# delldu/VSTNet

Hardware: AMD Instinct MI355X
Metric: stylized frames/sec at 1024x1024 (1/2/4/8 GPU) + % HBM roofline (higher is better)
Workload: dtype bf16x3

## Files before the change

include/vstnet.h:

```cpp
#ifndef VSTNET_H
#define VSTNET_H

#include <stddef.h>
#include <stdint.h>

#ifdef __cplusplus
extern "C" {
#endif
#pragma GCC visibility push(default)

#define VST_OK 0
#define VST_E_ARG (-1)
#define VST_E_SHAPE (-2)
#define VST_E_MODE (-3)
#define VST_E_WORKSPACE (-4)

#define VST_PREC_BF16X3 0
#define VST_PREC_FP32 1
#define VST_PREC_F16X2 2

#define VST_PREC_F16X2H 3

#define VST_NUM_BLOCKS 32

int vst_version(void);
const char* vst_error_string(int code);

#define VST_MAX_FRAME_PIXELS ((int64_t)1 << 26)
int64_t vst_max_frame_pixels(void);

size_t vst_conv_packed_bytes(int cout, int cin);
int vst_pack_conv(const float* w_oihw, int cout, int cin, void* packed, void* stream);

int vst_normalize_block(float* w1, float* b1, float* w4, float* b4, float* w7, int c_in1, int c_mid, int c_out,
                        float* scales, void* stream);

#define VST_RANGE_SATURATED 1u
#define VST_RANGE_WEIGHT 2u
int vst_range_flags(unsigned* flags_host, int reset);
int vst_range_flags_async(unsigned* flags4_dev, void* stream);

typedef struct vst_conv_weights {
    const void* packed;
    const float* bias;
} vst_conv_weights;

typedef struct vst_block_weights {
    vst_conv_weights conv[3];
} vst_block_weights;

typedef struct vst_net_weights {
    vst_block_weights blocks[VST_NUM_BLOCKS];
} vst_net_weights;

int vst_pack_input(const float* x, float* s1, float* s2, int B, int C, int H, int W, void* stream);
int vst_unpack_output(const float* s1, float* x, int B, int C, int H, int W, void* stream);
int vst_pack_input_u8(const uint8_t* frames_hwc, float* s1, float* s2, int B, int H, int W, void* stream);
int vst_unpack_output_u8(const float* s1, uint8_t* frames_hwc, int B, int H, int W, void* stream);
int vst_lab_luminance(const float* content, const float* stylized, float* out, int B, int H, int W, void* stream);
int vst_lab_luminance_u8(const uint8_t* content_hwc, const float* stylized, uint8_t* out_hwc, int B, int H, int W, void* stream);
int vst_lab_luminance_u8_f32(const uint8_t* content_hwc, const float* stylized, float* out, int B, int H, int W, void* stream);
int vst_spread(const float* s1, const float* s2, float* z, int B, int H, int W, int sp_steps, void* stream);
int vst_gather(const float* z, float* s1, float* s2, int B, int H, int W, int sp_steps, void* stream);

size_t vst_block_tmp_bytes(int B, int H, int W);
int vst_block_apply(const vst_block_weights* w, int channel, int stride, int direction, int precision,
                    float* dst, const float* src, void* tmp, int B, int H, int W, void* stream);

size_t vst_pass_workspace_bytes(int B, int H, int W);
int vst_pass_sub_batch(int B, int H, int W);
int vst_revnet_forward(const vst_net_weights* w, const float* x, float* z, void* workspace,
                       int B, int C_in, int H, int W, int sp_steps, int precision, void* stream);
int vst_revnet_inverse(const vst_net_weights* w, const float* z, float* x, void* workspace,
                       int B, int C_out, int H, int W, int sp_steps, int precision, void* stream);

int vst_revnet_forward_u8(const vst_net_weights* w, const uint8_t* frames_hwc, float* z, void* workspace,
                          int B, int H, int W, int sp_steps, int precision, void* stream);
int vst_revnet_inverse_u8(const vst_net_weights* w, const float* z, uint8_t* frames_hwc, void* workspace,
                          int B, int H, int W, int sp_steps, int precision, void* stream);

int vst_revnet_encode(const vst_net_weights* w, const float* x, float* code, void* workspace,
                      int B, int C_in, int H, int W, int precision, void* stream);
int vst_revnet_encode_u8(const vst_net_weights* w, const uint8_t* frames_hwc, float* code, void* workspace,
                         int B, int H, int W, int precision, void* stream);
int vst_revnet_decode(const vst_net_weights* w, const float* code, const float* affines, float* x, void* workspace,
                      int B, int C_out, int H, int W, int sp_steps, int precision, void* stream);
int vst_revnet_decode_u8(const vst_net_weights* w, const float* code, const float* affines, uint8_t* frames_hwc,
                         void* workspace, int B, int H, int W, int sp_steps, int precision, void* stream);
int vst_code_to_z(const float* code, float* z, int B, int H, int W, int sp_steps, void* stream);
int vst_z_to_code(const float* z, float* code, int B, int H, int W, int sp_steps, void* stream);
size_t vst_cwct_stats_code_workspace_bytes(int H, int W, int sp_steps);
int vst_cwct_stats_code(const float* code, int H, int W, int sp_steps, double* stats, void* workspace, void* stream);
int vst_cwct_apply_code(const float* code, float* out, int H, int W, int sp_steps, const float* affine, void* stream);
int vst_mask_to_code(const uint8_t* mask, uint8_t* mask_rows, int H, int W, void* stream);
size_t vst_cwct_stats_labels_code_workspace_bytes(int H, int W);
int vst_cwct_stats_labels_code(const float* code, int H, int W, const uint8_t* mask_rows, const void* plan, int max_slots,
                               double* stats, void* workspace, void* stream);
int vst_cwct_apply_labels_code(const float* code, float* out, int H, int W, const float* affines, const uint8_t* mask_rows,
                               const void* plan, int max_slots, void* stream);
int vst_cwct_stats_code_rect(const float* code, int H, int W, int sp_steps, int y0, int x0, int h, int w, double* stats,
                             void* workspace, void* stream);
int vst_cwct_stats_labels_code_rect(const float* code, int H, int W, int y0, int x0, int h, int w, const uint8_t* mask_rows,
                                    const void* plan, int max_slots, double* stats, void* workspace, void* stream);
int vst_revnet_decode_labels(const vst_net_weights* w, const float* code, const float* affines, const uint8_t* mask_rows,
                             const void* plan, int max_slots, float* x, void* workspace, int C_out, int H, int W,
                             int precision, void* stream);
int vst_revnet_decode_labels_u8(const vst_net_weights* w, const float* code, const float* affines, const uint8_t* mask_rows,
                                const void* plan, int max_slots, uint8_t* frame_hwc, void* workspace, int H, int W,
                                int precision, void* stream);
int vst_map_to_code(const float* map, float* rows, int H, int W, int sp_steps, void* stream);
int vst_cwct_apply_code_blend(const float* code, float* out, int H, int W, int sp_steps, const float* affine,
                              const float* strength_rows, void* stream);
int vst_cwct_apply_labels_code_blend(const float* code, float* out, int H, int W, const float* affines, const uint8_t* mask_rows,
                                     const void* plan, int max_slots, const float* strength_rows, void* stream);
int vst_revnet_decode_blend(const vst_net_weights* w, const float* code, const float* affines, const float* strength_rows,
                            float* x, void* workspace, int B, int C_out, int H, int W, int sp_steps, int precision, void* stream);
int vst_revnet_decode_blend_u8(const vst_net_weights* w, const float* code, const float* affines, const float* strength_rows,
                               uint8_t* frames_hwc, void* workspace, int B, int H, int W, int sp_steps, int precision,
                               void* stream);
int vst_revnet_decode_labels_blend(const vst_net_weights* w, const float* code, const float* affines, const uint8_t* mask_rows,
                                   const void* plan, int max_slots, const float* strength_rows, float* x, void* workspace,
                                   int C_out, int H, int W, int precision, void* stream);
int vst_revnet_decode_labels_blend_u8(const vst_net_weights* w, const float* code, const float* affines, const uint8_t* mask_rows,
                                      const void* plan, int max_slots, const float* strength_rows, uint8_t* frame_hwc,
                                      void* workspace, int H, int W, int precision, void* stream);
int vst_cwct_blend(const float* x, const float* y, const float* strength, float* out, int N, long L, void* stream);
int vst_cwct_apply_code_mix(const float* code, float* out, int H, int W, int sp_steps, const float* affines, int K,
                            const float* weight_rows, const float* strength_rows, void* stream);
int vst_revnet_decode_mix(const vst_net_weights* w, const float* code, const float* affines, int K, const float* weight_rows,
                          const float* strength_rows, float* x, void* workspace, int B, int C_out, int H, int W, int sp_steps,
                          int precision, void* stream);
int vst_revnet_decode_mix_u8(const vst_net_weights* w, const float* code, const float* affines, int K, const float* weight_rows,
                             const float* strength_rows, uint8_t* frames_hwc, void* workspace, int B, int H, int W, int sp_steps,
                             int precision, void* stream);
int vst_cwct_mix_acc(const float* a, const float* w, float* out, int N, long L, int first, void* stream);
int vst_strength_frame(const uint8_t* matte, const uint8_t* labels, const float* table, float* dense, float* rows, int H, int W,
                       int sp_steps, void* stream);
#define VST_STATS_POOL_MAX 8
int vst_cwct_stats_pool(const double* const* records_host_array, const double* weights_host, int n_ages, int n_records, int N,
                        double cut, double* out, int* used, void* stream);

size_t vst_cwct_stats_workspace_bytes(int N, long L);
int vst_cwct_stats(const float* x, int N, long L, const uint8_t* mask, int label,
                   double* stats, void* workspace, void* stream);
int vst_cwct_factor(const double* content_stats, const double* const* style_stats_host_array,
                    const float* alphas_host, int n_styles, float alpha_c, float eps, int N,
                    float* affine, int* info, void* stream);
int vst_cwct_apply(const float* x, float* y, int N, long L, const float* affine,
                   const uint8_t* mask, int label, void* stream);
int vst_cwct_apply_prec(const float* x, float* y, int N, long L, const float* affine,
                        const uint8_t* mask, int label, int precision, void* stream);
#define VST_LABEL_PLAN_BYTES 2344
int vst_label_plan(const uint8_t* cmask, long Lc, const uint8_t* smask, long Ls, void* plan, void* stream);
size_t vst_cwct_labels_workspace_bytes(int N, long L);
int vst_cwct_stats_labels(const float* x, int N, long L, const uint8_t* mask, const void* plan, int max_slots,
                          double* stats, void* workspace, void* stream);
int vst_cwct_factor_labels(const double* content_stats, const double* style_stats, const void* plan, int max_slots,
                           float eps, int N, float* affines, int* info, void* stream);
int vst_cwct_apply_labels(const float* x, float* y, int N, long L, const float* affines, const uint8_t* mask,
                          const void* plan, int max_slots, int precision, void* stream);

#define VST_MASK_OVERFLOW 1u
#define VST_MASK_OUT_OF_TABLE 2u
int vst_colors_to_labels(const uint8_t* rgb, uint8_t* labels, long n, void* stream);
int vst_label_hist(const uint8_t* labels, long n, int* hist, void* stream);
int vst_mask_prepare(const uint8_t* src, int colours, int H, int W, uint8_t* mask_rows, int* hist, void* stream);
int vst_remap_lut(const int* hist, const int* style_hist, const int16_t* table, int rows, int cols, int min_count,
                  uint8_t* lut, int* hist_out, unsigned* flags, void* stream);
int vst_apply_lut(const uint8_t* in, const uint8_t* lut, uint8_t* out, long n, void* stream);
int vst_label_plan_hist(const int* hist_c, const uint8_t* remap_lut, const int* hist_s, int max_slots, void* plan,
                        unsigned* flags, void* stream);
int vst_cwct_factor_labels_keyed(const double* content_stats, const double* style_stats, const void* plan,
                                 const void* style_plan, int max_slots, float eps, int N, float* affines, int* info,
                                 void* stream);
int vst_label_plan_hists(const int* hist_c, const uint8_t* remap_lut, const int* const* hist_s_host_array, int n_styles,
                         int max_slots, void* plan, unsigned* flags, void* stream);
int vst_cwct_factor_labels_mix(const double* content_stats, const double* const* style_stats_host_array,
                               const void* const* style_plans_host_array, const float* alphas_host, int n_styles,
                               float alpha_c, const void* plan, int max_slots, float eps, int N, float* affines, int* info,
                               void* stream);
int vst_cwct_prefactor_labels(const double* stats, const void* plan, int max_slots, int N, float eps, double* out, int* info,
                              void* stream);

int vst_cwct_prefactor(const double* stats, int N, float eps, double* out, int* info, void* stream);

int vst_generic_conv(const float* x, const float* w, const float* bias, const float* old, float sign, int relu, float* out, int B,
                     int Cin, int Cout, int H, int W, int K, int stride, void* stream);
int vst_generic_squeeze(const float* x, float* y, int B, int D, int H, int W, void* stream);
int vst_generic_unsqueeze(const float* y, float* x, int B, int D, int H, int W, void* stream);
int vst_generic_copy_channels(const float* src, float* dst, int B, int C_src, int c0, int n, long HW, int C_dst, int d0,
                              void* stream);
int vst_generic_zero(float* dst, size_t n_floats, void* stream);

size_t vst_cwct_stats_f64_workspace_bytes(int N, long L);
int vst_cwct_stats_f64(const float* x, int N, long L, const uint8_t* mask, int label, double* stats, void* workspace,
                       void* stream);
size_t vst_cwct_factor_f64_workspace_bytes(int N);
int vst_cwct_factor_f64(const double* content_stats, const double* const* style_stats_host_array, const float* alphas_host,
                        int n_styles, float alpha_c, float eps, int N, double* affine, int* info, void* workspace,
                        void* stream);
int vst_cwct_apply_f64(const float* x, float* y, int N, long L, const double* affine, const uint8_t* mask, int label,
                       void* stream);

size_t vst_cwct_stats_n_workspace_bytes(int N, long L);
int vst_cwct_stats_n(const float* x, int N, long L, const uint8_t* mask, int label, double* stats, void* workspace,
                     size_t workspace_bytes, void* stream);
size_t vst_cwct_factor_n_workspace_bytes(int N);
int vst_cwct_factor_n(const double* content_stats, const double* const* style_stats_host_array, const float* alphas_host,
                      int n_styles, float alpha_c, float eps, int N, float* affine, int* info, void* workspace,
                      size_t workspace_bytes, void* stream);
int vst_cwct_prefactor_n(const double* stats, int N, float eps, double* out, int* info, void* workspace, size_t workspace_bytes,
                         void* stream);
int vst_cwct_apply_n(const float* x, float* y, int N, long L, const float* affine, const uint8_t* mask, int label, void* stream);
size_t vst_cwct_stats_n_f64_workspace_bytes(int N, long L);
int vst_cwct_stats_n_f64(const float* x, int N, long L, const uint8_t* mask, int label, double* stats, void* workspace,
                         size_t workspace_bytes, void* stream);
size_t vst_cwct_factor_n_f64_workspace_bytes(int N);
int vst_cwct_factor_n_f64(const double* content_stats, const double* const* style_stats_host_array, const float* alphas_host,
                          int n_styles, float alpha_c, float eps, int N, double* affine, int* info, void* workspace,
                          size_t workspace_bytes, void* stream);
int vst_cwct_apply_n_f64(const float* x, float* y, int N, long L, const double* affine, const uint8_t* mask, int label,
                         void* stream);

#define VST_KERNEL_ID(cin, cout, stride) (((cin) << 16) | ((cout) << 4) | (stride))
#define VST_KERNEL_ALL (-1)
#define VST_KERNEL_PACK 1
#define VST_KERNEL_UNPACK 2
#define VST_KERNEL_SPREAD 3
#define VST_KERNEL_GATHER 4
#define VST_KERNEL_CWCT_STATS 5
#define VST_KERNEL_CWCT_FACTOR 6
#define VST_KERNEL_CWCT_APPLY 7
#define VST_KERNEL_PRESPLIT 8
#define VST_KERNEL_SEG_MIX 9
#define VST_KERNEL_CWCT_POOL 10
int vst_profile_begin(int kernel_id, int max_records);
int vst_profile_end(double* total_ms, int* launches);
int vst_profile_end_table(int* ids, double* ms, int* launches, int cap, int* n_ids);

#define VST_OPT_STAGE3_LEAN 1
#define VST_OPT_STAGE3_PINGPONG 2
#define VST_OPT_STAGE3_WIDE 3
#define VST_OPT_STAGE1_FOLD 4
#define VST_OPT_OUT_RGB 5
int vst_set_option(int option, int value);
int vst_get_option(int option);

#define VST_RESIZE_MAX_SHRINK 16
int vst_resize_coeffs_u8(int in_size, int out_size, int* ksize, int* bounds, int* kk);
int vst_resize_u8(const uint8_t* src_hwc, int Hs, int Ws, uint8_t* dst_hwc, int Hd, int Wd, const int* tables_dev,
                  uint8_t* tmp, void* stream);
int vst_resize_coeffs_u8_bilinear(int in_size, int out_size, int* ksize, int* bounds, int* kk);
int vst_resize_grey_u8(const uint8_t* src, int Hs, int Ws, uint8_t* dst, int Hd, int Wd, const int* tables_dev, uint8_t* tmp,
                       void* stream);
int vst_resize_coeffs_f32(int in_size, int out_size, int* ksize, int* xmin, float* w);
int vst_resize_f32(const float* x_planar, int B, int Hs, int Ws, float* dst_planar, int Hd, int Wd, const void* tables_dev,
                   float* tmp, void* stream);
int vst_resize_f32_to_u8(const float* x_planar, int B, int Hs, int Ws, uint8_t* dst_hwc, int Hd, int Wd,
                         const void* tables_dev, float* tmp, void* stream);

#define VST_SEG_CLASSES 150
#define VST_SEG_MAX_LABEL_PIXELS (1LL << 30)
#define VST_SEG_MIX_MAX 8
typedef struct vst_seg vst_seg;
int vst_seg_create(const int* depths, int embed_dim, vst_seg** plan);
int vst_seg_tensor_count(const vst_seg* plan);
int vst_seg_tensor_info(const vst_seg* plan, int index, const char** name, size_t* count);
int vst_seg_load_tensor(vst_seg* plan, const char* name, const float* data_host, size_t count);
int vst_seg_run_u8(vst_seg* plan, const uint8_t* frame_u8, int chw, int H, int W, uint8_t* labels_u8, void* stream);
int vst_seg_run_scaled_u8(vst_seg* plan, const uint8_t* work_u8, int chw, int Hw, int Ww, int H, int W, uint8_t* labels_u8,
                          void* stream);
int vst_seg_labels_from_logits(const float* logits, int Hq, int Wq, int H, int W, int kernel, uint8_t* labels, void* stream);
int vst_seg_logits(vst_seg* plan, const uint8_t* frame_u8, int chw, int H, int W, float* logits, float* x1, float* x2,
                   float* x3, float* x4, void* stream);
int vst_seg_shape(int H, int W, int* hw8);
int vst_seg_mix_logits(const float* const* logits_host_array, const float* weights_host, int n, size_t count, float* out,
                       void* stream);
int vst_seg_destroy(vst_seg* plan);
int vst_seg_gemm(const float* A, const float* W, const float* bias, const float* res, float* out, int M, int N, int K,
                 void* stream);
int vst_seg_layernorm(const float* x, const float* g, const float* b, float* out, int T, int C, float eps, void* stream);
int vst_seg_attention(const float* q, const float* kv, float* out, int N, int Nk, int C, float scale, void* stream);
int vst_seg_dwconv_gelu(const float* in, const float* w, const float* b, float* out, int H, int W, int C, void* stream);
int vst_seg_im2col(const float* in, int Hi, int Wi, int C, int k, int stride, int pad, float* col, void* stream);
int vst_seg_gather_rgb(const uint8_t* frame_u8, int chw, int H, int W, float* col, void* stream);
int vst_seg_head_sum(const float* y0, const float* y1, const float* y2, const float* y3, const int* hw8, int E, float* out,
                     void* stream);

#pragma GCC visibility pop
#ifdef __cplusplus
}
#endif
#endif
```

vstnet_amd/_lib.py:

```python
from __future__ import annotations

import ctypes as C
import glob
import os
import subprocess

PKG_DIR = os.path.dirname(os.path.abspath(__file__))
REPO_DIR = os.path.dirname(PKG_DIR)
LIB_PATH = os.environ.get("VSTNET_HIP_LIB") or os.path.join(PKG_DIR, "libvstnet_hip.so")
RESOURCES_PATH = os.path.join(PKG_DIR, "libvstnet_hip.resources.txt")
SOURCES = sorted(glob.glob(os.path.join(PKG_DIR, "csrc", "*.hip")))
HEADERS = sorted(glob.glob(os.path.join(PKG_DIR, "csrc", "*.h"))) + [os.path.join(REPO_DIR, "include", "vstnet.h")]

NUM_BLOCKS = 32
PREC_BF16X3 = 0
PREC_FP32 = 1
PREC_F16X2 = 2
PREC_F16X2H = 3

EXPORTS = [
    "vst_version", "vst_error_string", "vst_conv_packed_bytes", "vst_pack_conv", "vst_pack_input",
    "vst_unpack_output", "vst_pack_input_u8", "vst_unpack_output_u8", "vst_revnet_forward_u8", "vst_revnet_inverse_u8",
    "vst_spread", "vst_gather", "vst_block_tmp_bytes", "vst_block_apply",
    "vst_pass_workspace_bytes", "vst_revnet_forward", "vst_revnet_inverse",
    "vst_cwct_stats_workspace_bytes", "vst_cwct_stats", "vst_cwct_factor", "vst_cwct_apply", "vst_cwct_apply_prec",
    "vst_cwct_prefactor", "vst_label_plan", "vst_cwct_labels_workspace_bytes", "vst_cwct_stats_labels",
    "vst_cwct_factor_labels", "vst_cwct_apply_labels", "vst_profile_begin", "vst_profile_end", "vst_profile_end_table", "vst_lab_luminance",
    "vst_revnet_encode", "vst_revnet_encode_u8", "vst_revnet_decode", "vst_revnet_decode_u8", "vst_code_to_z", "vst_z_to_code",
    "vst_cwct_stats_code_workspace_bytes", "vst_cwct_stats_code", "vst_cwct_apply_code",
    "vst_mask_to_code", "vst_cwct_stats_labels_code_workspace_bytes", "vst_cwct_stats_labels_code", "vst_cwct_apply_labels_code",
    "vst_revnet_decode_labels", "vst_revnet_decode_labels_u8", "vst_pass_sub_batch",
    "vst_normalize_block", "vst_range_flags", "vst_range_flags_async",
    "vst_cwct_stats_f64_workspace_bytes", "vst_cwct_stats_f64", "vst_cwct_factor_f64_workspace_bytes", "vst_cwct_factor_f64",
    "vst_cwct_apply_f64",
    "vst_generic_conv", "vst_generic_squeeze", "vst_generic_unsqueeze", "vst_generic_copy_channels", "vst_generic_zero",
    "vst_set_option", "vst_get_option",
    "vst_cwct_stats_n_workspace_bytes", "vst_cwct_stats_n", "vst_cwct_factor_n_workspace_bytes", "vst_cwct_factor_n",
    "vst_cwct_prefactor_n", "vst_cwct_apply_n", "vst_cwct_stats_n_f64_workspace_bytes", "vst_cwct_stats_n_f64",
    "vst_cwct_factor_n_f64_workspace_bytes", "vst_cwct_factor_n_f64", "vst_cwct_apply_n_f64",
    "vst_max_frame_pixels", "vst_cwct_stats_code_rect", "vst_cwct_stats_labels_code_rect",
    "vst_colors_to_labels", "vst_label_hist", "vst_mask_prepare", "vst_remap_lut", "vst_apply_lut", "vst_label_plan_hist",
    "vst_cwct_factor_labels_keyed",
    "vst_label_plan_hists", "vst_cwct_factor_labels_mix", "vst_cwct_prefactor_labels",
    "vst_resize_coeffs_u8", "vst_resize_u8", "vst_resize_coeffs_f32", "vst_resize_f32", "vst_resize_f32_to_u8",
    "vst_lab_luminance_u8", "vst_lab_luminance_u8_f32",
    "vst_seg_create", "vst_seg_tensor_count", "vst_seg_tensor_info", "vst_seg_load_tensor", "vst_seg_run_u8", "vst_seg_logits",
    "vst_seg_shape", "vst_seg_destroy", "vst_seg_run_scaled_u8", "vst_seg_labels_from_logits",
    "vst_seg_mix_logits",
    "vst_seg_gemm", "vst_seg_layernorm", "vst_seg_attention", "vst_seg_dwconv_gelu", "vst_seg_im2col", "vst_seg_gather_rgb",
    "vst_seg_head_sum",
    "vst_map_to_code", "vst_cwct_apply_code_blend", "vst_cwct_apply_labels_code_blend", "vst_revnet_decode_blend",
    "vst_revnet_decode_blend_u8", "vst_revnet_decode_labels_blend", "vst_revnet_decode_labels_blend_u8", "vst_cwct_blend",
    "vst_strength_frame", "vst_resize_coeffs_u8_bilinear", "vst_resize_grey_u8",
    "vst_cwct_apply_code_mix", "vst_revnet_decode_mix", "vst_revnet_decode_mix_u8", "vst_cwct_mix_acc",
    "vst_cwct_stats_pool",
]
MAX_STYLES = 8
SEG_MIX_MAX = 8
KERNEL_SEG_MIX = 9
STATS_POOL_MAX = 8
KERNEL_CWCT_POOL = 10
MASK_OVERFLOW = 1
MASK_OUT_OF_TABLE = 2
LABEL_PLAN_BYTES = 2344
OPT_STAGE3_LEAN = 1
OPT_STAGE3_WIDE = 3
OPT_STAGE1_FOLD = 4
OPT_OUT_RGB = 5
RANGE_SATURATED = 1
RANGE_WEIGHT = 2


PRECISIONS = {"bf16x3": PREC_BF16X3, "fp32": PREC_FP32, "f16x2": PREC_F16X2, "f16x2h": PREC_F16X2H}


def default_precision() -> str:
    p = os.environ.get("VST_PRECISION", "bf16x3")
    if p not in PRECISIONS:
        raise ValueError(f"VST_PRECISION must be one of {sorted(PRECISIONS)}")
    return p


class VstError(RuntimeError):
    pass


class ConvWeights(C.Structure):
    _fields_ = [("packed", C.c_void_p), ("bias", C.c_void_p)]


class BlockWeights(C.Structure):
    _fields_ = [("conv", ConvWeights * 3)]


class NetWeights(C.Structure):
    _fields_ = [("blocks", BlockWeights * NUM_BLOCKS)]


def build(force: bool = False, verbose: bool = False) -> str:
    newest_src = max(os.path.getmtime(p) for p in SOURCES + HEADERS)
    if not force and os.path.exists(LIB_PATH) and os.path.getmtime(LIB_PATH) >= newest_src:
        return LIB_PATH
    hipcc = os.environ.get("HIPCC", "/opt/rocm/bin/hipcc")
    cmd = [hipcc, "-O3", "--offload-arch=gfx950", "-fPIC", "-shared", "-std=c++17", "-Xarch_host", "-fvisibility=hidden",
           "-I", os.path.join(REPO_DIR, "include"), "-o", LIB_PATH] + SOURCES
    cmd[1:1] = ["-Rpass-analysis=kernel-resource-usage", "-fno-caret-diagnostics"]
    if verbose:
        print(" ".join(cmd))
    p = subprocess.run(cmd, stderr=subprocess.PIPE, text=True)
    remarks = [ln.split("remark:", 1)[1].split("[-Rpass")[0].strip() for ln in p.stderr.splitlines() if "remark:" in ln]
    other = "\n".join(ln for ln in p.stderr.splitlines() if "remark:" not in ln and "kernel-resource-usage" not in ln)
    if p.returncode != 0:
        raise subprocess.CalledProcessError(p.returncode, cmd, stderr=other)
    if other.strip():
        print(other)
    table, name = [], None
    for r in remarks:
        if r.startswith("Function Name:"):
            name = r.split(":", 1)[1].strip()
        elif name and (r.startswith("VGPRs:") or r.startswith("ScratchSize") or r.startswith("LDS Size") or r.startswith("Occupancy")):
            table.append(f"{name}\t{r}")
    with open(RESOURCES_PATH, "w") as f:
        f.write("\n".join(table) + "\n")
    spills = [t for t in table if "ScratchSize" in t and not t.rstrip().endswith(": 0")]
    if spills:
        os.remove(LIB_PATH)
        raise RuntimeError("kernels with a private segment (register spills):\n" + "\n".join(spills))
    return LIB_PATH


RUNNER_SRC = os.path.join(REPO_DIR, "tools", "vst_run.cpp")
RUNNER_BIN = os.path.join(REPO_DIR, "tools", "vst_run")


def build_runner(force: bool = False) -> str:
    if not force and os.path.exists(RUNNER_BIN) and os.path.getmtime(RUNNER_BIN) >= max(os.path.getmtime(RUNNER_SRC),
                                                                                       os.path.getmtime(LIB_PATH)):
        return RUNNER_BIN
    hipcc = os.environ.get("HIPCC", "/opt/rocm/bin/hipcc")
    cmd = [hipcc, "-O2", "--offload-arch=gfx950", "-std=c++17", "-I", os.path.join(REPO_DIR, "include"), RUNNER_SRC,
           "-L", PKG_DIR, "-lvstnet_hip", "-Wl,-rpath," + PKG_DIR, "-Wl,-rpath,$ORIGIN/../vstnet_amd", "-o", RUNNER_BIN]
    subprocess.run(cmd, check=True)
    return RUNNER_BIN


_lib = None


def lib() -> C.CDLL:
    global _lib
    if _lib is not None:
        return _lib
    if not os.path.exists(LIB_PATH):
        raise VstError(f"{LIB_PATH} is missing: run `python -c 'import __graft_entry__ as g; g.build()'` "
                       "(there is no CPU fallback for the HIP path)")
    L = C.CDLL(LIB_PATH)
    vp, i, f, sz, lg = C.c_void_p, C.c_int, C.c_float, C.c_size_t, C.c_long
    sig = {
        "vst_version": (i, []),
        "vst_error_string": (C.c_char_p, [i]),
        "vst_conv_packed_bytes": (sz, [i, i]),
        "vst_pack_conv": (i, [vp, i, i, vp, vp]),
        "vst_normalize_block": (i, [vp, vp, vp, vp, vp, i, i, i, vp, vp]),
        "vst_range_flags": (i, [C.POINTER(C.c_uint), i]),
        "vst_range_flags_async": (i, [vp, vp]),
        "vst_pack_input": (i, [vp, vp, vp, i, i, i, i, vp]),
        "vst_unpack_output": (i, [vp, vp, i, i, i, i, vp]),
        "vst_pack_input_u8": (i, [vp, vp, vp, i, i, i, vp]),
        "vst_unpack_output_u8": (i, [vp, vp, i, i, i, vp]),
        "vst_lab_luminance": (i, [vp, vp, vp, i, i, i, vp]),
        "vst_lab_luminance_u8": (i, [vp, vp, vp, i, i, i, vp]),
        "vst_lab_luminance_u8_f32": (i, [vp, vp, vp, i, i, i, vp]),
        "vst_revnet_forward_u8": (i, [C.POINTER(NetWeights), vp, vp, vp, i, i, i, i, i, vp]),
        "vst_revnet_inverse_u8": (i, [C.POINTER(NetWeights), vp, vp, vp, i, i, i, i, i, vp]),
        "vst_spread": (i, [vp, vp, vp, i, i, i, i, vp]),
        "vst_gather": (i, [vp, vp, vp, i, i, i, i, vp]),
        "vst_block_tmp_bytes": (sz, [i, i, i]),
        "vst_block_apply": (i, [C.POINTER(BlockWeights), i, i, i, i, vp, vp, vp, i, i, i, vp]),
        "vst_pass_workspace_bytes": (sz, [i, i, i]),
        "vst_pass_sub_batch": (i, [i, i, i]),
        "vst_revnet_forward": (i, [C.POINTER(NetWeights), vp, vp, vp, i, i, i, i, i, i, vp]),
        "vst_revnet_inverse": (i, [C.POINTER(NetWeights), vp, vp, vp, i, i, i, i, i, i, vp]),
        "vst_cwct_stats_workspace_bytes": (sz, [i, lg]),
        "vst_cwct_stats": (i, [vp, i, lg, vp, i, vp, vp, vp]),
        "vst_cwct_factor": (i, [vp, C.POINTER(vp), C.POINTER(f), i, f, f, i, vp, vp, vp]),
        "vst_cwct_apply": (i, [vp, vp, i, lg, vp, vp, i, vp]),
        "vst_cwct_apply_prec": (i, [vp, vp, i, lg, vp, vp, i, i, vp]),
        "vst_cwct_prefactor": (i, [vp, i, f, vp, vp, vp]),
        "vst_cwct_stats_f64_workspace_bytes": (sz, [i, lg]),
        "vst_cwct_stats_f64": (i, [vp, i, lg, vp, i, vp, vp, vp]),
        "vst_cwct_factor_f64_workspace_bytes": (sz, [i]),
        "vst_cwct_factor_f64": (i, [vp, C.POINTER(vp), C.POINTER(f), i, f, f, i, vp, vp, vp, vp]),
        "vst_cwct_apply_f64": (i, [vp, vp, i, lg, vp, vp, i, vp]),
        "vst_cwct_stats_n_workspace_bytes": (sz, [i, lg]),
        "vst_cwct_stats_n": (i, [vp, i, lg, vp, i, vp, vp, sz, vp]),
        "vst_cwct_factor_n_workspace_bytes": (sz, [i]),
        "vst_cwct_factor_n": (i, [vp, C.POINTER(vp), C.POINTER(f), i, f, f, i, vp, vp, vp, sz, vp]),
        "vst_cwct_prefactor_n": (i, [vp, i, f, vp, vp, vp, sz, vp]),
        "vst_cwct_apply_n": (i, [vp, vp, i, lg, vp, vp, i, vp]),
        "vst_cwct_stats_n_f64_workspace_bytes": (sz, [i, lg]),
        "vst_cwct_stats_n_f64": (i, [vp, i, lg, vp, i, vp, vp, sz, vp]),
        "vst_cwct_factor_n_f64_workspace_bytes": (sz, [i]),
        "vst_cwct_factor_n_f64": (i, [vp, C.POINTER(vp), C.POINTER(f), i, f, f, i, vp, vp, vp, sz, vp]),
        "vst_cwct_apply_n_f64": (i, [vp, vp, i, lg, vp, vp, i, vp]),
        "vst_generic_conv": (i, [vp, vp, vp, vp, f, i, vp, i, i, i, i, i, i, i, vp]),
        "vst_generic_squeeze": (i, [vp, vp, i, i, i, i, vp]),
        "vst_generic_unsqueeze": (i, [vp, vp, i, i, i, i, vp]),
        "vst_generic_copy_channels": (i, [vp, vp, i, i, i, i, lg, i, i, vp]),
        "vst_generic_zero": (i, [vp, sz, vp]),
        "vst_label_plan": (i, [vp, lg, vp, lg, vp, vp]),
        "vst_cwct_labels_workspace_bytes": (sz, [i, lg]),
        "vst_cwct_stats_labels": (i, [vp, i, lg, vp, vp, i, vp, vp, vp]),
        "vst_cwct_factor_labels": (i, [vp, vp, vp, i, f, i, vp, vp, vp]),
        "vst_cwct_apply_labels": (i, [vp, vp, i, lg, vp, vp, vp, i, i, vp]),
        "vst_revnet_encode": (i, [C.POINTER(NetWeights), vp, vp, vp, i, i, i, i, i, vp]),
        "vst_revnet_encode_u8": (i, [C.POINTER(NetWeights), vp, vp, vp, i, i, i, i, vp]),
        "vst_revnet_decode": (i, [C.POINTER(NetWeights), vp, vp, vp, vp, i, i, i, i, i, i, vp]),
        "vst_revnet_decode_u8": (i, [C.POINTER(NetWeights), vp, vp, vp, vp, i, i, i, i, i, vp]),
        "vst_code_to_z": (i, [vp, vp, i, i, i, i, vp]),
        "vst_z_to_code": (i, [vp, vp, i, i, i, i, vp]),
        "vst_cwct_stats_code_workspace_bytes": (sz, [i, i, i]),
        "vst_cwct_stats_code": (i, [vp, i, i, i, vp, vp, vp]),
        "vst_cwct_apply_code": (i, [vp, vp, i, i, i, vp, vp]),
        "vst_mask_to_code": (i, [vp, vp, i, i, vp]),
        "vst_cwct_stats_labels_code_workspace_bytes": (sz, [i, i]),
        "vst_cwct_stats_labels_code": (i, [vp, i, i, vp, vp, i, vp, vp, vp]),
        "vst_cwct_apply_labels_code": (i, [vp, vp, i, i, vp, vp, vp, i, vp]),
        "vst_revnet_decode_labels": (i, [C.POINTER(NetWeights), vp, vp, vp, vp, i, vp, vp, i, i, i, i, vp]),
        "vst_revnet_decode_labels_u8": (i, [C.POINTER(NetWeights), vp, vp, vp, vp, i, vp, vp, i, i, i, vp]),
        "vst_map_to_code": (i, [vp, vp, i, i, i, vp]),
        "vst_cwct_apply_code_blend": (i, [vp, vp, i, i, i, vp, vp, vp]),
        "vst_cwct_apply_labels_code_blend": (i, [vp, vp, i, i, vp, vp, vp, i, vp, vp]),
        "vst_revnet_decode_blend": (i, [C.POINTER(NetWeights), vp, vp, vp, vp, vp, i, i, i, i, i, i, vp]),
        "vst_revnet_decode_blend_u8": (i, [C.POINTER(NetWeights), vp, vp, vp, vp, vp, i, i, i, i, i, vp]),
        "vst_revnet_decode_labels_blend": (i, [C.POINTER(NetWeights), vp, vp, vp, vp, i, vp, vp, vp, i, i, i, i, vp]),
        "vst_revnet_decode_labels_blend_u8": (i, [C.POINTER(NetWeights), vp, vp, vp, vp, i, vp, vp, vp, i, i, i, vp]),
        "vst_cwct_blend": (i, [vp, vp, vp, vp, i, lg, vp]),
        "vst_strength_frame": (i, [vp, vp, vp, vp, vp, i, i, i, vp]),
        "vst_cwct_apply_code_mix": (i, [vp, vp, i, i, i, vp, i, vp, vp, vp]),
        "vst_revnet_decode_mix": (i, [C.POINTER(NetWeights), vp, vp, i, vp, vp, vp, vp, i, i, i, i, i, i, vp]),
        "vst_revnet_decode_mix_u8": (i, [C.POINTER(NetWeights), vp, vp, i, vp, vp, vp, vp, i, i, i, i, i, vp]),
        "vst_cwct_mix_acc": (i, [vp, vp, vp, i, lg, i, vp]),
        "vst_resize_coeffs_u8_bilinear": (i, [i, i, C.POINTER(i), vp, vp]),
        "vst_resize_grey_u8": (i, [vp, i, i, vp, i, i, vp, vp, vp]),
        "vst_max_frame_pixels": (C.c_int64, []),
        "vst_cwct_stats_code_rect": (i, [vp, i, i, i, i, i, i, i, vp, vp, vp]),
        "vst_cwct_stats_labels_code_rect": (i, [vp, i, i, i, i, i, i, vp, vp, i, vp, vp, vp]),
        "vst_colors_to_labels": (i, [vp, vp, lg, vp]),
        "vst_label_hist": (i, [vp, lg, vp, vp]),
        "vst_mask_prepare": (i, [vp, i, i, i, vp, vp, vp]),
        "vst_remap_lut": (i, [vp, vp, vp, i, i, i, vp, vp, vp, vp]),
        "vst_apply_lut": (i, [vp, vp, vp, lg, vp]),
        "vst_label_plan_hist": (i, [vp, vp, vp, i, vp, vp, vp]),
        "vst_cwct_factor_labels_keyed": (i, [vp, vp, vp, vp, i, f, i, vp, vp, vp]),
        "vst_label_plan_hists": (i, [vp, vp, C.POINTER(vp), i, i, vp, vp, vp]),
        "vst_cwct_factor_labels_mix": (i, [vp, C.POINTER(vp), C.POINTER(vp), C.POINTER(f), i, f, vp, i, f, i, vp, vp, vp]),
        "vst_cwct_prefactor_labels": (i, [vp, vp, i, i, f, vp, vp, vp]),
        "vst_resize_coeffs_u8": (i, [i, i, C.POINTER(i), vp, vp]),
        "vst_resize_u8": (i, [vp, i, i, vp, i, i, vp, vp, vp]),
        "vst_resize_coeffs_f32": (i, [i, i, C.POINTER(i), vp, vp]),
        "vst_resize_f32": (i, [vp, i, i, i, vp, i, i, vp, vp, vp]),
        "vst_resize_f32_to_u8": (i, [vp, i, i, i, vp, i, i, vp, vp, vp]),
        "vst_seg_create": (i, [C.POINTER(i), i, C.POINTER(vp)]),
        "vst_seg_tensor_count": (i, [vp]),
        "vst_seg_tensor_info": (i, [vp, i, C.POINTER(C.c_char_p), C.POINTER(sz)]),
        "vst_seg_load_tensor": (i, [vp, C.c_char_p, vp, sz]),
        "vst_seg_run_u8": (i, [vp, vp, i, i, i, vp, vp]),
        "vst_seg_run_scaled_u8": (i, [vp, vp, i, i, i, i, i, vp, vp]),
        "vst_seg_labels_from_logits": (i, [vp, i, i, i, i, i, vp, vp]),
        "vst_seg_logits": (i, [vp, vp, i, i, i, vp, vp, vp, vp, vp, vp]),
        "vst_seg_shape": (i, [i, i, C.POINTER(i)]),
        "vst_seg_mix_logits": (i, [C.POINTER(vp), C.POINTER(f), i, sz, vp, vp]),
        "vst_cwct_stats_pool": (i, [C.POINTER(vp), C.POINTER(C.c_double), i, i, i, C.c_double, vp, vp, vp]),
        "vst_seg_destroy": (i, [vp]),
        "vst_seg_gemm": (i, [vp, vp, vp, vp, vp, i, i, i, vp]),
        "vst_seg_layernorm": (i, [vp, vp, vp, vp, i, i, f, vp]),
        "vst_seg_attention": (i, [vp, vp, vp, i, i, i, f, vp]),
        "vst_seg_dwconv_gelu": (i, [vp, vp, vp, vp, i, i, i, vp]),
        "vst_seg_im2col": (i, [vp, i, i, i, i, i, i, vp, vp]),
        "vst_seg_gather_rgb": (i, [vp, i, i, i, vp, vp]),
        "vst_seg_head_sum": (i, [vp, vp, vp, vp, C.POINTER(i), i, vp, vp]),
        "vst_set_option": (i, [i, i]),
        "vst_get_option": (i, [i]),
        "vst_profile_begin": (i, [i, i]),
        "vst_profile_end": (i, [C.POINTER(C.c_double), C.POINTER(i)]),
        "vst_profile_end_table": (i, [C.POINTER(i), C.POINTER(C.c_double), C.POINTER(i), i, C.POINTER(i)]),
    }
    for name, (res, args) in sig.items():
        fn = getattr(L, name)
        fn.restype = res
        fn.argtypes = args
    _lib = L
    return L


KERNEL_ALL = -1
MISC_KERNELS = {1: "pack_input", 2: "unpack_output", 3: "spread", 4: "gather", 5: "cwct_stats", 6: "cwct_factor",
                7: "cwct_apply", 8: "presplit", 9: "seg_mix", 10: "cwct_pool"}


def profile_table(run, max_records: int = 4096):
    L = lib()
    check(L.vst_profile_begin(KERNEL_ALL, max_records), "vst_profile_begin")
    try:
        run()
    finally:
        ids, ms, cnt, n = (C.c_int * 64)(), (C.c_double * 64)(), (C.c_int * 64)(), C.c_int(0)
        check(L.vst_profile_end_table(ids, ms, cnt, 64, C.byref(n)), "vst_profile_end_table")
    return {ids[k]: (ms[k], cnt[k]) for k in range(n.value)}


def set_option(option: int, value: int) -> None:
    check(lib().vst_set_option(option, int(value)), "vst_set_option")


def get_option(option: int) -> int:
    v = lib().vst_get_option(option)
    if v < 0:
        check(v, "vst_get_option")
    return v


def kernel_id(cin: int, cout: int, stride: int) -> int:
    return (cin << 16) | (cout << 4) | stride


def range_flags(reset: bool = False) -> int:
    v = C.c_uint(0)
    check(lib().vst_range_flags(C.byref(v), 1 if reset else 0), "vst_range_flags")
    return int(v.value)


def check(rc: int, what: str) -> None:
    if rc != 0:
        msg = lib().vst_error_string(rc).decode()
        raise VstError(f"{what} failed with status {rc}: {msg}")
```

vstnet_amd/csrc/common.h:

```cpp
#pragma once
#include <hip/hip_runtime.h>
#include <stdint.h>
#include <atomic>
#include "vstnet.h"

#define VST_RETURN_IF_LAUNCH_FAILED()                      \
    do {                                                   \
        hipError_t e__ = hipGetLastError();                \
        if (e__ != hipSuccess) return (int)e__;            \
    } while (0)

typedef __attribute__((ext_vector_type(8))) __bf16 bf16x8;
typedef __attribute__((ext_vector_type(8))) _Float16 f16x8;
typedef __attribute__((ext_vector_type(4))) unsigned u32x4;
typedef __attribute__((ext_vector_type(4))) __bf16 bf16x4;
typedef __attribute__((ext_vector_type(4))) float f32x4;
typedef __attribute__((ext_vector_type(16))) float f32x16;

__host__ __device__ __forceinline__ int vst_level_of_channels(int c) { return c == 16 ? 0 : (c == 64 ? 1 : 2); }

__device__ __forceinline__ size_t zc_offset(int level, int y, int x, int Wq) {
    if (level == 0) {
        const int cell = (y >> 2) * Wq + (x >> 2);
        const int sub = ((((y >> 1) & 1) * 2 + ((x >> 1) & 1)) << 6) + (((y & 1) * 2 + (x & 1)) << 4);
        return (size_t)cell * 256 + sub;
    } else if (level == 1) {
        const int cell = (y >> 1) * Wq + (x >> 1);
        return (size_t)cell * 256 + (((y & 1) * 2 + (x & 1)) << 6);
    }
    return (size_t)(y * Wq + x) * 256;
}

__device__ __forceinline__ int reflect_clamp(int v, int n) {
    if (v < 0) v = -v;
    if (v >= n) v = 2 * n - 2 - v;
    v = v < 0 ? 0 : v;
    return v >= n ? n - 1 : v;
}

#ifdef __HIPCC__
static __device__ unsigned vst_tu_range_flags;
__device__ __forceinline__ void vst_note_range(float amax) {
#ifndef VST_NO_RANGE_CHECK
    if (amax > 65504.f) atomicOr(&vst_tu_range_flags, VST_RANGE_SATURATED);
#endif
}
#define VST_DEFINE_TU_RANGE(name)                                                                                    \
    __attribute__((visibility("hidden"))) int name(unsigned* acc, int reset) {                                       \
        unsigned v = 0;                                                                                              \
        hipError_t e = hipMemcpyFromSymbol(&v, HIP_SYMBOL(vst_tu_range_flags), sizeof(v));                           \
        if (e != hipSuccess) return (int)e;                                                                          \
        *acc |= v;                                                                                                   \
        if (reset && v) {                                                                                            \
            const unsigned zero = 0;                                                                                 \
            e = hipMemcpyToSymbol(HIP_SYMBOL(vst_tu_range_flags), &zero, sizeof(zero));                              \
            if (e != hipSuccess) return (int)e;                                                                      \
        }                                                                                                            \
        return VST_OK;                                                                                               \
    }                                                                                                                \
    __attribute__((visibility("hidden"))) int name##_async(unsigned* dst_dev, hipStream_t st) {                      \
        return (int)hipMemcpyFromSymbolAsync(dst_dev, HIP_SYMBOL(vst_tu_range_flags), sizeof(unsigned), 0,           \
                                             hipMemcpyDeviceToDevice, st);                                           \
    }

__device__ __forceinline__ void split8_sp(const float (&f)[8], u32x4& hi, u32x4& lo, float& amax) {
    f16x8 h, l;
#ifndef VST_NO_RANGE_CHECK
    amax = fmaxf(fmaxf(fmaxf(amax, fabsf(f[0])), fmaxf(fabsf(f[1]), fabsf(f[2]))),
                 fmaxf(fmaxf(fabsf(f[3]), fabsf(f[4])), fmaxf(fmaxf(fabsf(f[5]), fabsf(f[6])), fabsf(f[7]))));
#endif
#pragma unroll
    for (int i = 0; i < 8; ++i) {
        h[i] = (_Float16)__builtin_amdgcn_fmed3f(f[i], -65504.f, 65504.f);
        l[i] = (_Float16)(f[i] - (float)h[i]);
    }
    hi = __builtin_bit_cast(u32x4, h);
    lo = __builtin_bit_cast(u32x4, l);
}
__device__ __forceinline__ void split8_sp(const float (&f)[8], u32x4& hi, u32x4& lo) {
    float amax = 0.f;
    split8_sp(f, hi, lo, amax);
    vst_note_range(amax);
}

__device__ __forceinline__ unsigned sp_offset(int cig, int plane, int y, int x, int H, int W) {
    return ((((unsigned)cig * 2 + plane) * H + y) * W + x) * 16u;
}
__device__ __forceinline__ unsigned sp_offset1(int cig, int y, int x, int H, int W) {
    return (((unsigned)cig * H + y) * W + x) * 16u;
}
#endif

static inline int vst_ensure_dynamic_lds(const void* kernel, int bytes, std::atomic<unsigned>* done_mask) {
    int dev = 0;
    hipError_t e = hipGetDevice(&dev);
    if (e != hipSuccess) return (int)e;
    if (dev < 32 && (done_mask->load(std::memory_order_acquire) >> dev) & 1u) return VST_OK;
    e = hipFuncSetAttribute(kernel, hipFuncAttributeMaxDynamicSharedMemorySize, bytes);
    if (e != hipSuccess) return (int)e;
    if (dev < 32) done_mask->fetch_or(1u << dev, std::memory_order_release);
    return VST_OK;
}

static inline bool vst_shape_ok(int B, int H, int W) {
    return B > 0 && H >= 8 && W >= 8 && (H % 4) == 0 && (W % 4) == 0 && (int64_t)H * W <= VST_MAX_FRAME_PIXELS;
}

struct PackedConvLayout {
    int ksteps;
    int coutp;
    size_t f32_bytes;
    size_t frag_bytes;
    int sp_sections;
    size_t f16_offset;
};

__host__ __device__ inline PackedConvLayout packed_conv_layout(int cout, int cin) {
    PackedConvLayout p;
    p.ksteps = cin >= 32 ? 9 * (cin / 32) : (cin == 16 ? 5 : 2);
    p.coutp = (cout + 15) / 16 * 16;
    p.f32_bytes = ((size_t)9 * cin * cout * 4 + 255) / 256 * 256;
    p.frag_bytes = (size_t)p.ksteps * 4 * p.coutp * 16;
    p.sp_sections = (cin >= 64 && cout >= 64) ? 1 : 0;
    p.f16_offset = p.f32_bytes + (size_t)(2 + p.sp_sections) * p.frag_bytes;
    return p;
}

#define CWCT_MAX_SLOTS 32
#define CWCT_MAX_STYLES 8
struct LabelPlan {
    int n_slots, overflow;
    int hist_c[256], hist_s[256];
    unsigned char lut[256];
    unsigned char slot_label[CWCT_MAX_SLOTS];
};
static_assert(sizeof(LabelPlan) == VST_LABEL_PLAN_BYTES, "vstnet.h: VST_LABEL_PLAN_BYTES");

int vst_prof_open(int kernel_id, hipStream_t st);
void vst_prof_close(int rec, hipStream_t st);
struct vst_prof_scope {
    int rec;
    hipStream_t st;
    vst_prof_scope(int kernel_id, hipStream_t s) : rec(vst_prof_open(kernel_id, s)), st(s) {}
    ~vst_prof_scope() { if (rec >= 0) vst_prof_close(rec, st); }
};
int vst_option(int option);

int vst3_block256(const vst_block_weights* w, int direction, int precision, float* dst, const float* src, void* tmp,
                  int pos, int src_planes_ready, int B, int H, int W, void* stream);
int vst3_conv_mid(const vst_conv_weights* c, const void* in_sp, void* out_sp, int out_single, int B, int H, int W, void* stream);
int vst3_conv_out(const vst_conv_weights* c, const void* in_sp, int in_single, float* state, void* out_sp, float sign, int B,
                  int H, int W, void* stream);
static inline bool vst_is_f16(int precision) { return precision == VST_PREC_F16X2 || precision == VST_PREC_F16X2H; }
int vst_block0_to_image(const vst_block_weights* w0, int precision, float* dst, const float* src, float* tmp, int B, int H,
                        int W, float* rgb, uint8_t* rgb_u8, int rgb_c, void* stream);

unsigned char* vst3_plane_buffer(void* tmp, int idx, int B, int H, int W);
extern "C" __attribute__((visibility("hidden"))) int vst3_gather_planes(const float* z, unsigned char* s1_planes, float* s2, int B, int H, int W, int sp_steps,
                                  void* stream);

int vst3_presplit(const float* state, unsigned char* planes, int B, int H, int W, void* stream);
int vst3_apply_code(const float* code, float* out0, float* out1, unsigned char* planes0, int H, int W, int sp_steps,
                    const float* affine, const float* strength_rows, void* stream);

int vst3_apply_code_mix(const float* code, float* out0, float* out1, unsigned char* planes0, int H, int W, int sp_steps,
                        const float* affines, int K, const float* weight_rows, const float* strength_rows, void* stream);

int vst3_apply_labels_code(const float* code, float* out0, float* out1, unsigned char* planes0, int H, int W,
                           const float* affines, const uint8_t* mask_rows, const void* plan, int max_slots,
                           const float* strength_rows, void* stream);

#define VST_INTERNAL __attribute__((visibility("hidden")))
int vst_range_tu_conv(unsigned* acc, int reset);
int vst_range_tu_conv3(unsigned* acc, int reset);
int vst_range_tu_layout(unsigned* acc, int reset);
int vst_range_tu_cwct(unsigned* acc, int reset);
int vst_range_tu_conv_async(unsigned* dst_dev, hipStream_t st);
int vst_range_tu_conv3_async(unsigned* dst_dev, hipStream_t st);
int vst_range_tu_layout_async(unsigned* dst_dev, hipStream_t st);
int vst_range_tu_cwct_async(unsigned* dst_dev, hipStream_t st);
extern "C" VST_INTERNAL int vst_pack_input_k(const float* x, const uint8_t* x_u8, float* s1, float* s2, int B, int C, int H, int W,
                                const float* addk, void* stream);
extern "C" VST_INTERNAL int vst_block0_const(const vst_block_weights* w0, float* k16, void* stream);
```

vstnet_amd/csrc/conv.hip:

```cpp
#include "common.h"

struct ConvArgs {
    const float* in;
    float* out;
    const unsigned char* packed;
    const float* bias;
    int Hin, Win, Hout, Wout;
    int Wq;
    size_t in_img_stride;
    size_t out_img_stride;
    float sign;
    int tiles_x, tiles_y, tiles_total;
    const unsigned char* packed1;
    const float* bias1;
    unsigned char* out_sp;
    size_t out_sp_img_bytes;
    unsigned trace_base;
    float* rgb;
    unsigned char* rgb_u8;
    int rgb_c;
};

#ifdef VST_TRACE
__device__ unsigned long long vst_trace_buf[4 * 16384];
__device__ unsigned long long* vst_trace_ptr;
__device__ unsigned vst_trace_cap;
static std::atomic<unsigned> vst_trace_host_n{0};
#define VST_TRACE_RESERVE(t_, grid_) (t_).trace_base = vst_trace_host_n.fetch_add((unsigned)(grid_));
#define VST_TRACE_BEGIN(which)                                                                                  \
    const unsigned long long trace_t0 = __builtin_amdgcn_s_memrealtime();
#define VST_TRACE_END_(which, cin_, cout_)                                                                      \
    if (VST_TRACE == (which) || VST_TRACE == 3) {                                                               \
        __builtin_amdgcn_s_waitcnt(0);                                                                          \
        asm volatile("s_waitcnt vmcnt(0)" ::: "memory");                                                       \
        if (threadIdx.x == 0 && (VST_TRACE == 3 || blockIdx.x < 16384)) {                                       \
            unsigned hw, xcc;                                                                                   \
            asm volatile("s_getreg_b32 %0, hwreg(HW_REG_HW_ID)" : "=s"(hw));                                    \
            asm volatile("s_getreg_b32 %0, hwreg(HW_REG_XCC_ID)" : "=s"(xcc));                                  \
            if (VST_TRACE == 3) {                                                                               \
                const unsigned i_ = a.trace_base + blockIdx.x;                                                  \
                if (vst_trace_ptr && i_ < vst_trace_cap) {                                                      \
                    unsigned long long* r_ = vst_trace_ptr + 4 * (size_t)i_;                                    \
                    r_[0] = trace_t0;                                                                           \
                    r_[1] = __builtin_amdgcn_s_memrealtime();                                                   \
                    r_[2] = hw | ((unsigned long long)xcc << 32);                                               \
                    r_[3] = (which) | ((cin_) << 8) | ((cout_) << 20) | ((unsigned long long)blockIdx.x << 32); \
                }                                                                                               \
            } else {                                                                                            \
                vst_trace_buf[4 * blockIdx.x + 0] = trace_t0;                                                   \
                vst_trace_buf[4 * blockIdx.x + 1] = __builtin_amdgcn_s_memrealtime();                           \
                vst_trace_buf[4 * blockIdx.x + 2] = hw;                                                         \
                vst_trace_buf[4 * blockIdx.x + 3] = xcc;                                                        \
            }                                                                                                   \
        }                                                                                                       \
    }
#define VST_TRACE_END(which) VST_TRACE_END_(which, 0, 0)
extern "C" __attribute__((visibility("default"))) int vst_trace_dump(unsigned long long* host, int n_wg) {
    return (int)hipMemcpyFromSymbol(host, HIP_SYMBOL(vst_trace_buf), sizeof(unsigned long long) * 4 * (size_t)n_wg);
}
extern "C" __attribute__((visibility("default"))) int vst_trace_set(unsigned long long* dev_buf, unsigned cap) {
    const unsigned zero = 0;
    hipError_t e = hipMemcpyToSymbol(HIP_SYMBOL(vst_trace_ptr), &dev_buf, sizeof(dev_buf));
    if (e == hipSuccess) e = hipMemcpyToSymbol(HIP_SYMBOL(vst_trace_cap), &cap, sizeof(cap));
    (void)zero;
    vst_trace_host_n.store(0);
    return (int)e;
}
extern "C" __attribute__((visibility("default"))) int vst_trace_count(unsigned* n) { *n = vst_trace_host_n.load(); return 0; }
#else
#define VST_TRACE_BEGIN(which)
#define VST_TRACE_END(which)
#define VST_TRACE_END_(which, cin_, cout_)
#define VST_TRACE_RESERVE(t_, grid_)
#endif

__device__ __forceinline__ bool xcd_tile(const ConvArgs& a, int& bx, int& by, int& bz) {
    const int g = blockIdx.x, per = gridDim.x >> 3;
    const int n = (g & 7) * per + (g >> 3);
    if (n >= a.tiles_total) return false;
    bx = n % a.tiles_x;
    const int r = n / a.tiles_x;
    by = r % a.tiles_y;
    bz = r / a.tiles_y;
    return true;
}

template <int CIN, int COUT, int STRIDE, int MRO = 0, int KSO = 0>
struct ConvCfg {
    static constexpr int NT = COUT >= 64 ? 64 : 16;
    static constexpr int NB = NT / 16;
    static constexpr int COUTP = (COUT + 15) / 16 * 16;
    static constexpr int NCOT = COUTP / NT;
    static constexpr int MR = MRO ? MRO : (STRIDE == 2 ? 2 : 4);
    static constexpr int TH = 4 * MR, TW = 16;
    static constexpr int IH = (TH - 1) * STRIDE + 3, IW = (TW - 1) * STRIDE + 3;
    static constexpr int NSLOT = (IH * IW + 15) / 16 * 16;
    static constexpr int CC = CIN >= 32 ? 32 : CIN;
    static constexpr int NCHUNK = CIN / CC;
    static constexpr int CIG = CC >= 8 ? CC / 8 : 1;
    static constexpr int KS = KSO ? KSO : (CIN >= 32 ? 9 : (CIN == 16 ? 5 : 2));
    static constexpr int A_PLANE = CIN == 4 ? NSLOT * 8 : CIG * NSLOT * 16;
    static constexpr int B_PLANE = KS * 4 * NT * 16;
    static constexpr int LDS_BYTES = 2 * A_PLANE + 2 * B_PLANE;
    static constexpr int LDS_BYTES_T2 = 2 * A_PLANE + B_PLANE;
    static_assert(LDS_BYTES <= 160 * 1024, "LDS budget");
};

__device__ __forceinline__ void split8_f16(const float4 v0, const float4 v1, uint4& hi, uint4& lo, float& amax) {
    const float f[8] = {v0.x, v0.y, v0.z, v0.w, v1.x, v1.y, v1.z, v1.w};
    u32x4 h, l;
    split8_sp(f, h, l, amax);
    hi = __builtin_bit_cast(uint4, h);
    lo = __builtin_bit_cast(uint4, l);
}

__device__ __forceinline__ void split4_f16(const float4 v, uint2& hi, uint2& lo, float& amax) {
    const float f[4] = {v.x, v.y, v.z, v.w};
    typedef __attribute__((ext_vector_type(4))) _Float16 f16x4;
    f16x4 h, l;
#ifndef VST_NO_RANGE_CHECK
    amax = fmaxf(fmaxf(amax, fabsf(f[0])), fmaxf(fmaxf(fabsf(f[1]), fabsf(f[2])), fabsf(f[3])));
#endif
#pragma unroll
    for (int i = 0; i < 4; ++i) {
        const float c = __builtin_amdgcn_fmed3f(f[i], -65504.f, 65504.f);
        h[i] = (_Float16)c;
        l[i] = (_Float16)(f[i] - (float)h[i]);
    }
    hi = __builtin_bit_cast(uint2, h);
    lo = __builtin_bit_cast(uint2, l);
}

__device__ __forceinline__ void split8(const float4 v0, const float4 v1, uint4& hi, uint4& lo) {
    const float f[8] = {v0.x, v0.y, v0.z, v0.w, v1.x, v1.y, v1.z, v1.w};
    bf16x8 h, l;
#pragma unroll
    for (int i = 0; i < 8; ++i) {
        h[i] = (__bf16)f[i];
        l[i] = (__bf16)(f[i] - (float)h[i]);
    }
    hi = __builtin_bit_cast(uint4, h);
    lo = __builtin_bit_cast(uint4, l);
}

__device__ __forceinline__ void split4(const float4 v, uint2& hi, uint2& lo) {
    const float f[4] = {v.x, v.y, v.z, v.w};
    bf16x4 h, l;
#pragma unroll
    for (int i = 0; i < 4; ++i) {
        h[i] = (__bf16)f[i];
        l[i] = (__bf16)(f[i] - (float)h[i]);
    }
    hi = __builtin_bit_cast(uint2, h);
    lo = __builtin_bit_cast(uint2, l);
}

template <int COUT, int NB>
__device__ __forceinline__ void load_bias(const ConvArgs& a, int co_lane, float4 (&bias)[NB]) {
#pragma unroll
    for (int n = 0; n < NB; ++n)
        bias[n] = co_lane + n * 16 < COUT ? *(const float4*)(a.bias + co_lane + n * 16) : make_float4(0.f, 0.f, 0.f, 0.f);
}

template <int COUT, bool OUT_STATE, bool FULL = false>
__device__ __forceinline__ float4* out_ptr(const ConvArgs& a, float* out_img, int oy, int ox, int co) {
    if (!FULL && (oy >= a.Hout || ox >= a.Wout || co >= COUT)) return nullptr;
    if (OUT_STATE) return (float4*)(out_img + zc_offset(vst_level_of_channels(COUT), oy, ox, a.Wq) + co);
    return (float4*)(out_img + ((size_t)oy * a.Wout + ox) * COUT + co);
}

template <int COUT, int MR, int NB, bool FULL = false>
__device__ __forceinline__ void load_old(const ConvArgs& a, float* out_img, int oy0, int ox, int co_lane,
                                         float4 (&old)[MR][NB]) {
#pragma unroll
    for (int m = 0; m < MR; ++m)
#pragma unroll
        for (int n = 0; n < NB; ++n) {
            const float4* p = out_ptr<COUT, true, FULL>(a, out_img, oy0 + m, ox, co_lane + n * 16);
            old[m][n] = (FULL || p) ? *p : make_float4(0.f, 0.f, 0.f, 0.f);
        }
}

template <int COUT, bool OUT_STATE, int MR, int NB, bool FULL = false>
__device__ __forceinline__ void store_tile(const ConvArgs& a, float* out_img, int oy0, int ox, int co_lane,
                                           const f32x4 (&acc)[MR][NB], const float4 (&bias)[NB],
                                           const float4 (&old)[MR][NB]) {
#pragma unroll
    for (int m = 0; m < MR; ++m)
#pragma unroll
        for (int n = 0; n < NB; ++n) {
            float4* p = out_ptr<COUT, OUT_STATE, FULL>(a, out_img, oy0 + m, ox, co_lane + n * 16);
            if (!FULL && !p) continue;
            float4 r = make_float4(acc[m][n][0] + bias[n].x, acc[m][n][1] + bias[n].y, acc[m][n][2] + bias[n].z,
                                   acc[m][n][3] + bias[n].w);
            if (OUT_STATE) {
                const float4 o = old[m][n];
                r = make_float4(o.x + a.sign * r.x, o.y + a.sign * r.y, o.z + a.sign * r.z, o.w + a.sign * r.w);
            } else {
                r.x = r.x > 0.f ? r.x : 0.f; r.y = r.y > 0.f ? r.y : 0.f;
                r.z = r.z > 0.f ? r.z : 0.f; r.w = r.w > 0.f ? r.w : 0.f;
            }
            *p = r;
        }
}

#define MFMA3(acc, wh, wl, xh, xl)                                              \
    acc = __builtin_amdgcn_mfma_f32_16x16x32_bf16(wh, xl, acc, 0, 0, 0);        \
    acc = __builtin_amdgcn_mfma_f32_16x16x32_bf16(wl, xh, acc, 0, 0, 0);        \
    acc = __builtin_amdgcn_mfma_f32_16x16x32_bf16(wh, xh, acc, 0, 0, 0)

#define MFMA_T(acc, wh, wl, xh, xl)                                                                                          \
    if constexpr (TERMS == 3) {                                                                                               \
        MFMA3(acc, wh, wl, xh, xl);                                                                                           \
    } else {                                                                                                                  \
        acc = __builtin_amdgcn_mfma_f32_16x16x32_f16(__builtin_bit_cast(f16x8, wh), __builtin_bit_cast(f16x8, xl), acc, 0, 0, 0); \
        acc = __builtin_amdgcn_mfma_f32_16x16x32_f16(__builtin_bit_cast(f16x8, wh), __builtin_bit_cast(f16x8, xh), acc, 0, 0, 0); \
    }
#define SPLIT8_T(v0_, v1_, h_, l_) { if constexpr (TERMS == 3) split8(v0_, v1_, h_, l_); else split8_f16(v0_, v1_, h_, l_, range_amax); }
#define SPLIT4_T(v_, h_, l_) { if constexpr (TERMS == 3) split4(v_, h_, l_); else split4_f16(v_, h_, l_, range_amax); }

template <int CIN, int COUT, int STRIDE, bool IN_STATE, bool OUT_STATE, bool OUT_SP = false, int TERMS = 3, bool OUT_H16 = false,
          bool FOLD = false>
__global__ __launch_bounds__(256) void conv_mfma_kernel(const ConvArgs a) {
    static_assert(!FOLD || (CIN == 16 && COUT == 4 && STRIDE == 1 && TERMS == 3 && !OUT_STATE && !OUT_SP && !OUT_H16),
                  "tap-folded form: conv.1 of the 16-channel blocks, bf16x3");
    using C = ConvCfg<CIN, COUT, STRIDE, 0, FOLD ? 2 : 0>;
    extern __shared__ __attribute__((aligned(16))) unsigned char smem[];
    unsigned char* const a_hi = smem;
    unsigned char* const a_lo = smem + C::A_PLANE;
    unsigned char* const b_hi = smem + 2 * C::A_PLANE;
    unsigned char* const b_lo = TERMS == 3 ? b_hi + C::B_PLANE : b_hi;

    const int tid = threadIdx.x, lane = tid & 63, wave = tid >> 6;
    const int lrow = lane & 15, kg = lane >> 4;
    int bx, by, bz;
    if (!xcd_tile(a, bx, by, bz)) return;
    float range_amax = 0.f;
    VST_TRACE_BEGIN(2)
    const int tx0 = bx * C::TW, ty0 = by * C::TH;
    const int b = bz / C::NCOT, co0 = (bz % C::NCOT) * C::NT;

    const float* const in_img = a.in + (size_t)b * a.in_img_stride;
    const PackedConvLayout PL = packed_conv_layout(COUT, CIN);
    const unsigned char* const w_hi = a.packed + (TERMS == 3 ? PL.f32_bytes : PL.f16_offset);
    const unsigned char* const w_lo = w_hi + PL.frag_bytes;

    f32x4 acc[C::MR][C::NB];
#pragma unroll
    for (int m = 0; m < C::MR; ++m)
#pragma unroll
        for (int n = 0; n < C::NB; ++n) acc[m][n] = f32x4{0.f, 0.f, 0.f, 0.f};

    const int slot_base = (wave * C::MR * STRIDE) * C::IW + lrow * STRIDE;

    constexpr int A_ITEMS_T = CIN == 4 ? C::IH * C::IW : C::IH * C::IW * C::CIG;
    constexpr int AIT = (A_ITEMS_T + 255) / 256, NV = CIN == 4 ? 1 : 2;
    constexpr int W_ITEMS_T = C::KS * 4 * C::NT, WIT = (W_ITEMS_T + 255) / 256;
    typedef __attribute__((ext_vector_type(4))) unsigned u32x4;
    f32x4 areg[AIT][NV];
    u32x4 wreg[WIT][2];
#define F4(v_) make_float4((v_)[0], (v_)[1], (v_)[2], (v_)[3])
#define GEN_FETCH(chunk_)                                                                           \
    _Pragma("unroll") for (int it = 0; it < WIT; ++it) {                                           \
        int idx = it * 256 + tid;                                                                  \
        idx = idx < W_ITEMS_T ? idx : W_ITEMS_T - 1;                                               \
        const int co = idx % C::NT, r = idx / C::NT;                                               \
        if constexpr (FOLD) {                                                                      \
            const int ty = 2 * (r >> 2) + ((r >> 1) & 1), tx = co >> 2;           \
            const bool live = ty < 3 && tx < 3;                                                    \
            const int tap = live ? 3 * ty + tx : 0;                                                \
            const size_t src = ((size_t)((tap >> 1) * 4 + (tap & 1) * 2 + (r & 1)) * 16 + (co & 3)) * 16; \
            const u32x4 h_ = *(const u32x4*)(w_hi + src), l_ = *(const u32x4*)(w_lo + src);        \
            wreg[it][0] = live ? h_ : u32x4{0u, 0u, 0u, 0u};                                       \
            wreg[it][1] = live ? l_ : u32x4{0u, 0u, 0u, 0u};                                       \
        } else {                                                                                   \
            const size_t src = ((size_t)((chunk_) * C::KS * 4 + r) * C::COUTP + co0 + co) * 16;    \
            wreg[it][0] = *(const u32x4*)(w_hi + src);                                             \
            if (TERMS == 3) wreg[it][1] = *(const u32x4*)(w_lo + src);                             \
        }                                                                                          \
    }                                                                                              \
    _Pragma("unroll") for (int it = 0; it < AIT; ++it) {                                           \
        int idx = it * 256 + tid;                                                                  \
        idx = idx < A_ITEMS_T ? idx : A_ITEMS_T - 1;                                               \
        const int cig = CIN == 4 ? 0 : idx % C::CIG, slot = CIN == 4 ? idx : idx / C::CIG;         \
        const int iy = slot / C::IW, ix = slot - iy * C::IW;                                       \
        const int gy = reflect_clamp(ty0 * STRIDE - 1 + iy, a.Hin);                                \
        const int gx = reflect_clamp(tx0 * STRIDE - 1 + ix, a.Win);                                \
        const size_t off = IN_STATE ? zc_offset(vst_level_of_channels(CIN), gy, gx, a.Wq)          \
                                    : ((size_t)gy * a.Win + gx) * CIN;                             \
        const float* p = in_img + off + (chunk_) * C::CC + cig * 8;                                \
        areg[it][0] = *(const f32x4*)p;                                                            \
        if (NV == 2) areg[it][NV - 1] = *(const f32x4*)(p + 4);                                    \
    }
#define GEN_LAND()                                                                                 \
    _Pragma("unroll") for (int it = 0; it < AIT; ++it) {                                           \
        int idx = it * 256 + tid;                                                                  \
        idx = idx < A_ITEMS_T ? idx : A_ITEMS_T - 1;                                               \
        if (CIN == 4) {                                                                            \
            uint2 h, l;                                                                            \
            SPLIT4_T(F4(areg[it][0]), h, l);                                                       \
            *(uint2*)(a_hi + idx * 8) = h;                                                         \
            *(uint2*)(a_lo + idx * 8) = l;                                                         \
        } else {                                                                                   \
            const int cig = idx % C::CIG, slot = idx / C::CIG;                                     \
            uint4 h, l;                                                                            \
            SPLIT8_T(F4(areg[it][0]), F4(areg[it][NV - 1]), h, l);                                 \
            *(uint4*)(a_hi + (cig * C::NSLOT + slot) * 16) = h;                                    \
            *(uint4*)(a_lo + (cig * C::NSLOT + slot) * 16) = l;                                    \
        }                                                                                          \
    }                                                                                              \
    _Pragma("unroll") for (int it = 0; it < WIT; ++it) {                                           \
        int idx = it * 256 + tid;                                                                  \
        idx = idx < W_ITEMS_T ? idx : W_ITEMS_T - 1;                                               \
        *(u32x4*)(b_hi + idx * 16) = wreg[it][0];                                                  \
        if (TERMS == 3) *(u32x4*)(b_lo + idx * 16) = wreg[it][1];                                  \
    }

    float* const out_img = a.out + (size_t)b * a.out_img_stride;
    float4 bias[C::NB], old[C::MR][C::NB];
    const bool interior = COUT % 16 == 0 && ty0 + C::TH <= a.Hout && tx0 + C::TW <= a.Wout;
    constexpr bool EARLY_OLD = OUT_STATE && C::MR * C::NB >= 16;
    auto fetch_old = [&]() __attribute__((always_inline)) {
        if (interior) load_old<COUT, C::MR, C::NB, true>(a, out_img, ty0 + wave * C::MR, tx0 + lrow, co0 + 4 * kg, old);
        else load_old<COUT, C::MR, C::NB>(a, out_img, ty0 + wave * C::MR, tx0 + lrow, co0 + 4 * kg, old);
    };

    GEN_FETCH(0);
    GEN_LAND();
    if constexpr (FOLD) {
        constexpr int NPX = C::MR * C::IW, NBLK = (NPX + 15) / 16;
        static_assert(4 * NBLK * 16 * 12 * 4 <= 2 * C::A_PLANE, "the transposed accumulators fit the image region");
        __syncthreads();
        f32x4 facc[NBLK];
#pragma unroll
        for (int j = 0; j < NBLK; ++j) facc[j] = f32x4{0.f, 0.f, 0.f, 0.f};
#pragma unroll
        for (int ks = 0; ks < C::KS; ++ks) {
            const int boff = ((ks * 4 + kg) * 16 + lrow) * 16;
            const bf16x8 wh = __builtin_bit_cast(bf16x8, *(const uint4*)(b_hi + boff));
            const bf16x8 wl = __builtin_bit_cast(bf16x8, *(const uint4*)(b_lo + boff));
            int ty = 2 * ks + (kg >> 1);
            ty = ty > 2 ? 2 : ty;
#pragma unroll
            for (int j = 0; j < NBLK; ++j) {
                int q = j * 16 + lrow;
                q = q < NPX ? q : NPX - 1;
                const int aoff = ((kg & 1) * C::NSLOT + (wave * C::MR + ty) * C::IW + q) * 16;
                const bf16x8 xh = __builtin_bit_cast(bf16x8, *(const uint4*)(a_hi + aoff));
                const bf16x8 xl = __builtin_bit_cast(bf16x8, *(const uint4*)(a_lo + aoff));
                MFMA3(facc[j], wh, wl, xh, xl);
            }
        }
        __syncthreads();
        float* const sc = (float*)smem + wave * (NBLK * 16 * 12);
        if (kg < 3) {
#pragma unroll
            for (int j = 0; j < NBLK; ++j) *(f32x4*)(sc + ((j * 16 + lrow) * 3 + kg) * 4) = facc[j];
        }
        __syncthreads();
        const int q0 = kg * C::IW + lrow;
        const f32x4 d0 = *(const f32x4*)(sc + ((q0 + 0) * 3 + 0) * 4);
        const f32x4 d1 = *(const f32x4*)(sc + ((q0 + 1) * 3 + 1) * 4);
        const f32x4 d2 = *(const f32x4*)(sc + ((q0 + 2) * 3 + 2) * 4);
        const float4 bs = *(const float4*)a.bias;
        const int oy = ty0 + wave * C::MR + kg, ox = tx0 + lrow;
        if (oy < a.Hout && ox < a.Wout) {
            float4 r = make_float4((d0[0] + d1[0]) + d2[0] + bs.x, (d0[1] + d1[1]) + d2[1] + bs.y,
                                   (d0[2] + d1[2]) + d2[2] + bs.z, (d0[3] + d1[3]) + d2[3] + bs.w);
            r.x = r.x > 0.f ? r.x : 0.f; r.y = r.y > 0.f ? r.y : 0.f;
            r.z = r.z > 0.f ? r.z : 0.f; r.w = r.w > 0.f ? r.w : 0.f;
            *(float4*)(a.out + (size_t)b * a.out_img_stride + ((size_t)oy * a.Wout + ox) * COUT) = r;
        }
        VST_TRACE_END_(2, CIN, COUT)
        return;
    }
#pragma unroll
    for (int chunk = 0; chunk < C::NCHUNK; ++chunk) {
        __syncthreads();
        if (chunk + 1 < C::NCHUNK) { GEN_FETCH(chunk + 1); }
        if (EARLY_OLD && chunk == C::NCHUNK - 1) fetch_old();

#pragma unroll
        for (int ks = 0; ks < C::KS; ++ks) {
            bf16x8 wh[C::NB], wl[C::NB];
#pragma unroll
            for (int n = 0; n < C::NB; ++n) {
                const int boff = ((ks * 4 + kg) * C::NT + n * 16 + lrow) * 16;
                wh[n] = __builtin_bit_cast(bf16x8, *(const uint4*)(b_hi + boff));
                if (TERMS == 3) wl[n] = __builtin_bit_cast(bf16x8, *(const uint4*)(b_lo + boff)); else wl[n] = wh[n];
            }
#pragma unroll
            for (int m = 0; m < C::MR; ++m) {
                bf16x8 xh, xl;
                if (CIN >= 32) {
                    const int dy = ks / 3, dx = ks - dy * 3;
                    const int slot = slot_base + (m * STRIDE + dy) * C::IW + dx;
                    const int aoff = (kg * C::NSLOT + slot) * 16;
                    xh = __builtin_bit_cast(bf16x8, *(const uint4*)(a_hi + aoff));
                    xl = __builtin_bit_cast(bf16x8, *(const uint4*)(a_lo + aoff));
                } else if (CIN == 16) {
                    int tap = 2 * ks + (kg >> 1);
                    tap = tap > 8 ? 8 : tap;
                    const int dy = tap / 3, dx = tap - dy * 3;
                    const int slot = slot_base + (m * STRIDE + dy) * C::IW + dx;
                    const int aoff = ((kg & 1) * C::NSLOT + slot) * 16;
                    xh = __builtin_bit_cast(bf16x8, *(const uint4*)(a_hi + aoff));
                    xl = __builtin_bit_cast(bf16x8, *(const uint4*)(a_lo + aoff));
                } else {
                    int t0 = 8 * ks + 2 * kg;
                    t0 = t0 > 8 ? 8 : t0;
                    const int t1 = t0 + 1 > 8 ? 8 : t0 + 1;
                    const int s0 = slot_base + (m * STRIDE + t0 / 3) * C::IW + t0 % 3;
                    const int s1 = slot_base + (m * STRIDE + t1 / 3) * C::IW + t1 % 3;
                    const uint2 h0 = *(const uint2*)(a_hi + s0 * 8), h1 = *(const uint2*)(a_hi + s1 * 8);
                    const uint2 l0 = *(const uint2*)(a_lo + s0 * 8), l1 = *(const uint2*)(a_lo + s1 * 8);
                    xh = __builtin_bit_cast(bf16x8, make_uint4(h0.x, h0.y, h1.x, h1.y));
                    xl = __builtin_bit_cast(bf16x8, make_uint4(l0.x, l0.y, l1.x, l1.y));
                }
#pragma unroll
                for (int n = 0; n < C::NB; ++n) { MFMA_T(acc[m][n], wh[n], wl[n], xh, xl); }
            }
        }
        if (chunk + 1 < C::NCHUNK) {
            __syncthreads();
            GEN_LAND();
        }
    }
#undef GEN_FETCH
#undef GEN_LAND
#undef F4

    load_bias<COUT, C::NB>(a, co0 + 4 * kg, bias);
    if constexpr (OUT_SP) {
        static_assert(COUT == 64 && C::NB == 4 && !OUT_STATE, "plane output: the 64-channel intermediates only");
        unsigned char* const sp_img = a.out_sp + (size_t)b * a.out_sp_img_bytes;
#pragma unroll
        for (int m = 0; m < C::MR; ++m) {
            const int oy = ty0 + wave * C::MR + m, ox = tx0 + lrow;
            if (oy >= a.Hout || ox >= a.Wout) continue;
#pragma unroll
            for (int j = 0; j < 2; ++j) {
                float f8[8];
#pragma unroll
                for (int e = 0; e < 8; ++e) {
                    const int n = 2 * j + (e >> 2);
                    const float bb = e & 2 ? (e & 1 ? bias[n].w : bias[n].z) : (e & 1 ? bias[n].y : bias[n].x);
                    const float v = acc[m][n][e & 3] + bb;
                    f8[e] = v > 0.f ? v : 0.f;
                }
                u32x4 hi, lo;
                split8_sp(f8, hi, lo, range_amax);
                *(u32x4*)(sp_img + sp_offset(j * 4 + kg, 0, oy, ox, a.Hout, a.Wout)) = hi;
                *(u32x4*)(sp_img + sp_offset(j * 4 + kg, 1, oy, ox, a.Hout, a.Wout)) = lo;
            }
        }
        vst_note_range(range_amax);
        return;
    }
    if constexpr (OUT_H16) {
        static_assert(!OUT_STATE && !OUT_SP, "fp16 output: the h1 intermediates only");
        _Float16* const o16 = (_Float16*)a.out + (size_t)b * a.out_img_stride;
#pragma unroll
        for (int m = 0; m < C::MR; ++m)
#pragma unroll
            for (int n = 0; n < C::NB; ++n) {
                const int oy = ty0 + wave * C::MR + m, ox = tx0 + lrow, co = co0 + 4 * kg + n * 16;
                if (oy >= a.Hout || ox >= a.Wout || co >= COUT) continue;
                const float r[4] = {acc[m][n][0] + bias[n].x, acc[m][n][1] + bias[n].y, acc[m][n][2] + bias[n].z, acc[m][n][3] + bias[n].w};
                typedef __attribute__((ext_vector_type(4))) _Float16 f16x4;
                f16x4 h;
                range_amax = fmaxf(fmaxf(range_amax, r[0]), fmaxf(fmaxf(r[1], r[2]), r[3]));
#pragma unroll
                for (int e = 0; e < 4; ++e) h[e] = (_Float16)__builtin_amdgcn_fmed3f(r[e], 0.f, 65504.f);
                *(f16x4*)(o16 + ((size_t)oy * a.Wout + ox) * COUT + co) = h;
            }
        vst_note_range(range_amax);
        VST_TRACE_END_(2, CIN, COUT)
        return;
    }
    if constexpr (TERMS == 2) vst_note_range(range_amax);
    if (OUT_STATE && !EARLY_OLD) fetch_old();
    if (interior) store_tile<COUT, OUT_STATE, C::MR, C::NB, true>(a, out_img, ty0 + wave * C::MR, tx0 + lrow, co0 + 4 * kg, acc, bias, old);
    else store_tile<COUT, OUT_STATE, C::MR, C::NB>(a, out_img, ty0 + wave * C::MR, tx0 + lrow, co0 + 4 * kg, acc, bias, old);
    VST_TRACE_END_(2, CIN, COUT)
}

template <int CIN, bool NO_LO = false>
__device__ __forceinline__ void read_x_small(const unsigned char* img_hi, const unsigned char* img_lo, int nslot,
                                             int slot00, int iw, int ks, int kg, bf16x8& xh, bf16x8& xl) {
    if (CIN == 16) {
        int tap = 2 * ks + (kg >> 1);
        tap = tap > 8 ? 8 : tap;
        const int slot = slot00 + (tap / 3) * iw + tap % 3;
        const int aoff = ((kg & 1) * nslot + slot) * 16;
        xh = __builtin_bit_cast(bf16x8, *(const uint4*)(img_hi + aoff));
        if (!NO_LO) xl = __builtin_bit_cast(bf16x8, *(const uint4*)(img_lo + aoff)); else xl = xh;
    } else {
        int t0 = 8 * ks + 2 * kg;
        t0 = t0 > 8 ? 8 : t0;
        const int t1 = t0 + 1 > 8 ? 8 : t0 + 1;
        const int s0 = slot00 + (t0 / 3) * iw + t0 % 3, s1 = slot00 + (t1 / 3) * iw + t1 % 3;
        const uint2 h0 = *(const uint2*)(img_hi + s0 * 8), h1 = *(const uint2*)(img_hi + s1 * 8);
        xh = __builtin_bit_cast(bf16x8, make_uint4(h0.x, h0.y, h1.x, h1.y));
        if (!NO_LO) {
            const uint2 l0 = *(const uint2*)(img_lo + s0 * 8), l1 = *(const uint2*)(img_lo + s1 * 8);
            xl = __builtin_bit_cast(bf16x8, make_uint4(l0.x, l0.y, l1.x, l1.y));
        } else {
            xl = xh;
        }
    }
}

template <int MID, int CH, int TERMS = 3, int MR = 4, bool H16 = false>
struct PairCfg {
    using C7 = ConvCfg<MID, CH, 1, MR>;
    static constexpr int R1 = 20, N1SLOT = (4 * MR + 4) * R1, RW = 18, RH = 4 * MR + 2, NPX = RH * RW, NBLK = (NPX + 15) / 16;
    static constexpr int H1_PLANE = MID == 4 ? N1SLOT * 8 : C7::CIG * N1SLOT * 16;
    static constexpr int W4_PLANE = C7::KS * 4 * 16 * 16;
    static constexpr bool ALIAS = MID == 16;
    static constexpr int WPL = TERMS == 3 ? 2 : 1;
    static constexpr int H1W4 = (H16 ? 1 : 2) * H1_PLANE + WPL * W4_PLANE;
    static constexpr int U_BYTES = ALIAS ? (H1W4 > WPL * C7::B_PLANE ? H1W4 : WPL * C7::B_PLANE) : H1W4 + WPL * C7::B_PLANE;
    static constexpr int LDS_BYTES = 2 * C7::A_PLANE + U_BYTES;
};

template <int MID, int CH, int TERMS = 3, int MR = 4, bool H16 = false, bool OUT_RGB = false>
__global__ __launch_bounds__(256, (MID == 16 && TERMS == 2) ? 3 : 1) void conv_pair_kernel(const ConvArgs a) {
    static_assert(!H16 || TERMS == 2, "fp16 h1: the 2-term kernels only");
    static_assert(!OUT_RGB || (MID == 4 && CH == 16), "image output: the 16-channel blocks only");
    using P = PairCfg<MID, CH, TERMS, MR, H16>;
    using C = typename P::C7;
    static_assert(C::NCHUNK == 1 && C::NCOT == 1, "single-chunk shapes");
    extern __shared__ __attribute__((aligned(16))) unsigned char smem[];
    unsigned char* const a_hi = smem;
    unsigned char* const a_lo = smem + C::A_PLANE;
    unsigned char* const u0 = smem + 2 * C::A_PLANE;
    unsigned char* const b_hi = P::ALIAS ? u0 : u0 + P::H1W4;
    unsigned char* const b_lo = TERMS == 3 ? b_hi + C::B_PLANE : b_hi;
    unsigned char* const h1_hi = u0;
    unsigned char* const h1_lo = H16 ? u0 : u0 + P::H1_PLANE;
    unsigned char* const w4s_hi = u0 + (H16 ? 1 : 2) * P::H1_PLANE;
    unsigned char* const w4s_lo = TERMS == 3 ? w4s_hi + P::W4_PLANE : w4s_hi;

    const int tid = threadIdx.x, lane = tid & 63, wave = tid >> 6;
    const int lrow = lane & 15, kg = lane >> 4;
    int bx, by, b;
    if (!xcd_tile(a, bx, by, b)) return;
    float range_amax = 0.f;
    VST_TRACE_BEGIN(1)
    const int tx0 = bx * C::TW, ty0 = by * C::TH;
    const int H = a.Hout, W = a.Wout;
    const float* const in_img = a.in + (size_t)b * a.in_img_stride;
    float* const out_img = a.out + (size_t)b * a.out_img_stride;
    const PackedConvLayout PL7 = packed_conv_layout(CH, MID), PL4 = packed_conv_layout(MID, MID);
    const unsigned char* const w7_hi = a.packed + (TERMS == 3 ? PL7.f32_bytes : PL7.f16_offset);
    const unsigned char* const w7_lo = w7_hi + PL7.frag_bytes;
    const unsigned char* const w4_hi = a.packed1 + (TERMS == 3 ? PL4.f32_bytes : PL4.f16_offset);
    const unsigned char* const w4_lo = w4_hi + PL4.frag_bytes;

    typedef __attribute__((ext_vector_type(4))) unsigned u32x4;
    constexpr int H1_ITEMS = MID == 4 ? P::N1SLOT : P::N1SLOT * C::CIG, H1IT = (H1_ITEMS + 255) / 256, NV = MID == 4 ? 1 : 2;
    constexpr int W4_ITEMS = C::KS * 4 * 16, W4IT = (W4_ITEMS + 255) / 256;
    constexpr int W7_ITEMS = C::KS * 4 * C::NT, W7IT = (W7_ITEMS + 255) / 256;
    f32x4 hreg[H1IT][NV];
    u32x4 h16reg[H16 ? H1IT : 1];
    u32x4 w4reg[W4IT][2], w7reg[W7IT][2];
#pragma unroll
    for (int it = 0; it < W4IT; ++it) {
        int idx = it * 256 + tid;
        idx = idx < W4_ITEMS ? idx : W4_ITEMS - 1;
        w4reg[it][0] = *(const u32x4*)(w4_hi + (size_t)idx * 16);
        if (TERMS == 3) w4reg[it][1] = *(const u32x4*)(w4_lo + (size_t)idx * 16);
    }
#pragma unroll
    for (int it = 0; it < H1IT; ++it) {
        int idx = it * 256 + tid;
        idx = idx < H1_ITEMS ? idx : H1_ITEMS - 1;
        const int cig = MID == 4 ? 0 : idx % C::CIG, slot = MID == 4 ? idx : idx / C::CIG;
        const int iy = slot / P::R1, ix = slot - iy * P::R1;
        const int gy = reflect_clamp(ty0 - 2 + iy, H), gx = reflect_clamp(tx0 - 2 + ix, W);
        if constexpr (H16) {
            const _Float16* p16 = (const _Float16*)a.in + (size_t)b * a.in_img_stride + ((size_t)gy * W + gx) * MID + cig * 8;
            if (MID == 4) { const uint2 v = *(const uint2*)p16; h16reg[it] = u32x4{v.x, v.y, 0u, 0u}; }
            else h16reg[it] = *(const u32x4*)p16;
        } else {
            const float* p = in_img + ((size_t)gy * W + gx) * MID + cig * 8;
            hreg[it][0] = *(const f32x4*)p;
            if (NV == 2) hreg[it][NV - 1] = *(const f32x4*)(p + 4);
        }
    }
#pragma unroll
    for (int it = 0; it < W7IT; ++it) {
        int idx = it * 256 + tid;
        idx = idx < W7_ITEMS ? idx : W7_ITEMS - 1;
        const int co = idx % C::NT, r = idx / C::NT;
        const size_t src = ((size_t)r * C::COUTP + co) * 16;
        w7reg[it][0] = *(const u32x4*)(w7_hi + src);
        if (TERMS == 3) w7reg[it][1] = *(const u32x4*)(w7_lo + src);
    }
    float4 bias[C::NB], old[C::MR][C::NB];
    const bool interior = ty0 + C::TH <= H && tx0 + C::TW <= W;
    constexpr bool EARLY_OLD = C::MR * C::NB >= 16 && TERMS == 3 && !OUT_RGB;
#define PAIR_FETCH_OLD()                                                                                         \
    if (interior) load_old<CH, C::MR, C::NB, true>(a, out_img, ty0 + wave * C::MR, tx0 + lrow, 4 * kg, old);   \
    else load_old<CH, C::MR, C::NB>(a, out_img, ty0 + wave * C::MR, tx0 + lrow, 4 * kg, old);
    if (EARLY_OLD) { PAIR_FETCH_OLD(); }

#define F4(v_) make_float4((v_)[0], (v_)[1], (v_)[2], (v_)[3])
#pragma unroll
    for (int it = 0; it < H1IT; ++it) {
        int idx = it * 256 + tid;
        idx = idx < H1_ITEMS ? idx : H1_ITEMS - 1;
        if constexpr (H16) {
            if (MID == 4) {
                *(uint2*)(h1_hi + idx * 8) = make_uint2(h16reg[it][0], h16reg[it][1]);
            } else {
                const int cig = idx % C::CIG, slot = idx / C::CIG;
                *(u32x4*)(h1_hi + (cig * P::N1SLOT + slot) * 16) = h16reg[it];
            }
        } else if (MID == 4) {
            uint2 h, l;
            SPLIT4_T(F4(hreg[it][0]), h, l);
            *(uint2*)(h1_hi + idx * 8) = h;
            *(uint2*)(h1_lo + idx * 8) = l;
        } else {
            const int cig = idx % C::CIG, slot = idx / C::CIG;
            uint4 h, l;
            SPLIT8_T(F4(hreg[it][0]), F4(hreg[it][NV - 1]), h, l);
            *(uint4*)(h1_hi + (cig * P::N1SLOT + slot) * 16) = h;
            *(uint4*)(h1_lo + (cig * P::N1SLOT + slot) * 16) = l;
        }
    }
#undef F4
#pragma unroll
    for (int it = 0; it < W4IT; ++it) {
        int idx = it * 256 + tid;
        idx = idx < W4_ITEMS ? idx : W4_ITEMS - 1;
        *(u32x4*)(w4s_hi + idx * 16) = w4reg[it][0];
        if (TERMS == 3) *(u32x4*)(w4s_lo + idx * 16) = w4reg[it][1];
    }
#define LAND_W7()                                                                                  \
    _Pragma("unroll") for (int it = 0; it < W7IT; ++it) {                                          \
        int idx = it * 256 + tid;                                                                  \
        idx = idx < W7_ITEMS ? idx : W7_ITEMS - 1;                                                 \
        *(u32x4*)(b_hi + idx * 16) = w7reg[it][0];                                                 \
        if (TERMS == 3) *(u32x4*)(b_lo + idx * 16) = w7reg[it][1];                                 \
    }
    if (!P::ALIAS) { LAND_W7(); }
    __syncthreads();

    {
        float4 b4 = make_float4(0.f, 0.f, 0.f, 0.f);
        if (4 * kg < MID) b4 = *(const float4*)(a.bias1 + 4 * kg);
        const bool ring_inside = ty0 >= 1 && tx0 >= 1 && ty0 + C::TH + 1 <= H && tx0 + 17 <= W;
        constexpr bool HOIST = MID == 4;
        bf16x8 w4h[HOIST ? C::KS : 1], w4l[HOIST ? C::KS : 1];
        if (HOIST) {
#pragma unroll
            for (int ks = 0; ks < C::KS; ++ks) {
                const int boff = ((ks * 4 + kg) * 16 + lrow) * 16;
                w4h[HOIST ? ks : 0] = __builtin_bit_cast(bf16x8, *(const uint4*)(w4s_hi + boff));
                w4l[HOIST ? ks : 0] = __builtin_bit_cast(bf16x8, *(const uint4*)(w4s_lo + boff));
            }
        }
        for (int blk0 = wave; blk0 < P::NBLK; blk0 += 8) {
            f32x4 acc4[2];
            int ryv[2], rxv[2];
            bool okv[2];
#pragma unroll
            for (int u = 0; u < 2; ++u) {
                int p = (blk0 + 4 * u) * 16 + lrow;
                okv[u] = p < P::NPX;
                p = okv[u] ? p : P::NPX - 1;
                ryv[u] = p / P::RW; rxv[u] = p - ryv[u] * P::RW;
                acc4[u] = f32x4{0.f, 0.f, 0.f, 0.f};
            }
#pragma unroll
            for (int ks = 0; ks < C::KS; ++ks) {
                bf16x8 wh, wl;
                if (HOIST) {
                    wh = w4h[HOIST ? ks : 0]; wl = w4l[HOIST ? ks : 0];
                } else {
                    const int boff = ((ks * 4 + kg) * 16 + lrow) * 16;
                    wh = __builtin_bit_cast(bf16x8, *(const uint4*)(w4s_hi + boff));
                    wl = __builtin_bit_cast(bf16x8, *(const uint4*)(w4s_lo + boff));
                }
#pragma unroll
                for (int u = 0; u < 2; ++u) {
                    bf16x8 xh, xl;
                    read_x_small<MID, H16>(h1_hi, h1_lo, P::N1SLOT, ryv[u] * P::R1 + rxv[u], P::R1, ks, kg, xh, xl);
                    if constexpr (H16) {
                        acc4[u] = __builtin_amdgcn_mfma_f32_16x16x32_f16(__builtin_bit_cast(f16x8, wh), __builtin_bit_cast(f16x8, xh), acc4[u], 0, 0, 0);
                    } else {
                        MFMA_T(acc4[u], wh, wl, xh, xl);
                    }
                }
            }
#pragma unroll
            for (int u = 0; u < 2; ++u) {
                const int ry = ryv[u], rx = rxv[u];
                float4 v = make_float4(acc4[u][0] + b4.x, acc4[u][1] + b4.y, acc4[u][2] + b4.z, acc4[u][3] + b4.w);
                v.x = v.x > 0.f ? v.x : 0.f; v.y = v.y > 0.f ? v.y : 0.f;
                v.z = v.z > 0.f ? v.z : 0.f; v.w = v.w > 0.f ? v.w : 0.f;
                uint2 h, l;
                SPLIT4_T(v, h, l);
#define PAIR_PUT(slot_)                                                                            \
                if (MID == 4) {                                                                    \
                    *(uint2*)(a_hi + (slot_) * 8) = h;                                             \
                    *(uint2*)(a_lo + (slot_) * 8) = l;                                             \
                } else {                                                                           \
                    const int off_ = ((kg >> 1) * C::NSLOT + (slot_)) * 16 + (kg & 1) * 8;         \
                    *(uint2*)(a_hi + off_) = h;                                                    \
                    *(uint2*)(a_lo + off_) = l;                                                    \
                }
                if (ring_inside) {
                    if (okv[u] && 4 * kg < MID) { PAIR_PUT(ry * C::IW + rx); }
                } else {
                    const int gy = ty0 - 1 + ry, gx = tx0 - 1 + rx;
                    if (okv[u] && 4 * kg < MID && gy >= 0 && gy < H && gx >= 0 && gx < W) {
                        const int my = gy == 1 ? -2 : (gy == H - 2 ? 2 : 0), mx = gx == 1 ? -2 : (gx == W - 2 ? 2 : 0);
                        int sy = ry + my, sx = rx + mx;
                        sy = (sy < 0 || sy >= P::RH) ? ry : sy;
                        sx = (sx < 0 || sx >= P::RW) ? rx : sx;
                        PAIR_PUT(ry * C::IW + rx);
                        PAIR_PUT(sy * C::IW + rx);
                        PAIR_PUT(ry * C::IW + sx);
                        PAIR_PUT(sy * C::IW + sx);
                    }
                }
#undef PAIR_PUT
            }
        }
    }
    __syncthreads();
    if (P::ALIAS) {
        LAND_W7();
        __syncthreads();
    }
#undef LAND_W7

    f32x4 acc[C::MR][C::NB];
#pragma unroll
    for (int m = 0; m < C::MR; ++m)
#pragma unroll
        for (int n = 0; n < C::NB; ++n) acc[m][n] = f32x4{0.f, 0.f, 0.f, 0.f};
    const int slot_base = (wave * C::MR) * C::IW + lrow;
#pragma unroll
    for (int ks = 0; ks < C::KS; ++ks) {
        bf16x8 wh[C::NB], wl[C::NB];
#pragma unroll
        for (int n = 0; n < C::NB; ++n) {
            const int boff = ((ks * 4 + kg) * C::NT + n * 16 + lrow) * 16;
            wh[n] = __builtin_bit_cast(bf16x8, *(const uint4*)(b_hi + boff));
            wl[n] = __builtin_bit_cast(bf16x8, *(const uint4*)(b_lo + boff));
        }
#pragma unroll
        for (int m = 0; m < C::MR; ++m) {
            bf16x8 xh, xl;
            read_x_small<MID>(a_hi, a_lo, C::NSLOT, slot_base + m * C::IW, C::IW, ks, kg, xh, xl);
#pragma unroll
            for (int n = 0; n < C::NB; ++n) { MFMA_T(acc[m][n], wh[n], wl[n], xh, xl); }
        }
    }
    load_bias<CH, C::NB>(a, 4 * kg, bias);
    if constexpr (TERMS == 2) vst_note_range(range_amax);
    if constexpr (OUT_RGB) {
        const int ox = tx0 + lrow, nc = a.rgb_u8 ? 3 : a.rgb_c;
        const size_t plane = (size_t)H * W;
#pragma unroll
        for (int m = 0; m < C::MR; ++m) {
            const int oy = ty0 + wave * C::MR + m;
            if (oy >= H || ox >= W || 4 * kg >= nc) continue;
            const float4 o = *(const float4*)(out_img + zc_offset(0, oy, ox, a.Wq) + 4 * kg);
            float4 r = make_float4(acc[m][0][0] + bias[0].x, acc[m][0][1] + bias[0].y, acc[m][0][2] + bias[0].z,
                                   acc[m][0][3] + bias[0].w);
            r = make_float4(o.x + a.sign * r.x, o.y + a.sign * r.y, o.z + a.sign * r.z, o.w + a.sign * r.w);
            const float c[4] = {r.x, r.y, r.z, r.w};
            if (a.rgb_u8) {
                unsigned char* dst = a.rgb_u8 + ((size_t)b * plane + (size_t)oy * W + ox) * 3;
#pragma unroll
                for (int k = 0; k < 3; ++k) {
                    float t = c[k] * 255.f;
                    t = t < 0.f ? 0.f : (t > 255.f ? 255.f : t);
                    dst[k] = (unsigned char)t;
                }
            } else {
                float* dst = a.rgb + ((size_t)b * a.rgb_c + 4 * kg) * plane + (size_t)oy * W + ox;
#pragma unroll
                for (int k = 0; k < 4; ++k)
                    if (4 * kg + k < nc) dst[k * plane] = c[k];
            }
        }
        VST_TRACE_END_(1, MID, CH)
        return;
    }
    if (!EARLY_OLD) { PAIR_FETCH_OLD(); }
#undef PAIR_FETCH_OLD
    if (interior) store_tile<CH, true, C::MR, C::NB, true>(a, out_img, ty0 + wave * C::MR, tx0 + lrow, 4 * kg, acc, bias, old);
    else store_tile<CH, true, C::MR, C::NB>(a, out_img, ty0 + wave * C::MR, tx0 + lrow, 4 * kg, acc, bias, old);
    VST_TRACE_END_(1, MID, CH)
}

template <int CIN, int COUT, int NW_ = 8, int MR_ = 2>
struct PipeCfg {
    static constexpr int NW = NW_, NTHR = 64 * NW, MR = MR_;
    static constexpr int NT = 64, NB = 4, TH = MR * NW, IW = 18, NPIX = (TH + 2) * IW, NSLOT = (NPIX + 15) / 16 * 16;
    static constexpr int NCHUNK = CIN / 32, NCOT = COUT / 64;
    static constexpr int A_PLANE = 4 * NSLOT * 16, A_BUF = 2 * A_PLANE;
    static constexpr int B_PLANE = 3 * 4 * 64 * 16, B_BUF = 2 * B_PLANE;
    static constexpr int LDS_BYTES = 2 * A_BUF + 2 * B_BUF;
    static constexpr int A_PART = NPIX * 4 / 3;
    static constexpr int A_ITEMS = ((A_PART / 4 + 15) / 16 * 64 + NTHR - 1) / NTHR;
    static constexpr int B_ITEMS = 2 * 768 / NTHR;
    static_assert(NPIX % 3 == 0, "three equal parts");
    static_assert(LDS_BYTES <= 160 * 1024, "LDS budget");
};

template <int NDSR, int NVM, int NDW>
__device__ __forceinline__ void wide_interleave() {
#pragma unroll
    for (int i = 0; i < 48; ++i) {
        __builtin_amdgcn_sched_group_barrier(0x008, 1, 0);
        if (i % 2 == 0 && i / 2 < NDSR) __builtin_amdgcn_sched_group_barrier(0x100, 1, 0);
        if (i % 2 == 1 && i / 2 < NVM) __builtin_amdgcn_sched_group_barrier(0x020, 1, 0);
        if (i % 2 == 1 && i / 2 < NDW) __builtin_amdgcn_sched_group_barrier(0x200, 1, 0);
    }
}

template <int CIN, int COUT, bool IN_STATE, bool OUT_STATE, int NW = 8, int MR = 2>
__global__ __launch_bounds__(64 * NW, (NW == 4 && MR == 2) ? 2 : 1) void conv_pipe_kernel(const ConvArgs a) {
    using C = PipeCfg<CIN, COUT, NW, MR>;
    constexpr bool WIDE = NW == 4 && MR == 4;
    constexpr bool PEEL = WIDE && COUT == 64;
    extern __shared__ __attribute__((aligned(16))) unsigned char smem[];
    unsigned char* const Abuf = smem;
    unsigned char* const Bbuf = smem + 2 * C::A_BUF;

    const int tid = threadIdx.x, lane = tid & 63, wave = tid >> 6;
    const int lrow = lane & 15, kg = lane >> 4;
    int bx, by, b;
    if (!xcd_tile(a, bx, by, b)) return;
    VST_TRACE_BEGIN(4)
    const int tx0 = bx * 16, ty0 = by * C::TH;
    const float* const in_img = a.in + (size_t)b * a.in_img_stride;
    float* const out_img = a.out + (size_t)b * a.out_img_stride;
    const PackedConvLayout PL = packed_conv_layout(COUT, CIN);
    const unsigned char* const w_plane0 = a.packed + PL.f32_bytes;

    unsigned a_src[3][C::A_ITEMS], a_dst[3][C::A_ITEMS];
#define A_TABLE(part)                                                                   \
    _Pragma("unroll") for (int it = 0; it < C::A_ITEMS; ++it) {                         \
         \
            \
        const int j = it * C::NTHR + tid;                                               \
        int sl = (j >> 6) * 16 + (j & 15);                            \
        sl = sl < C::A_PART / 4 ? sl : C::A_PART / 4 - 1;                               \
        const int cig = (j >> 4) & 3, slot = (part) * (C::A_PART / 4) + sl;             \
        const int iy = slot / C::IW, ix = slot - iy * C::IW;                            \
        const int gy = reflect_clamp(ty0 - 1 + iy, a.Hin), gx = reflect_clamp(tx0 - 1 + ix, a.Win); \
        const size_t off = IN_STATE ? zc_offset(vst_level_of_channels(CIN), gy, gx, a.Wq) \
                                    : ((size_t)gy * a.Win + gx) * CIN;                  \
        a_src[part][it] = (unsigned)(off + cig * 8);                                    \
        a_dst[part][it] = (cig * C::NSLOT + slot) * 16;                                 \
    }
    if constexpr (!PEEL) {
#pragma unroll
        for (int part = 0; part < 3; ++part) { A_TABLE(part); }
    }
    typedef f32x4 APart[C::A_ITEMS][2];
    typedef u32x4 BStage[C::B_ITEMS];
#define LOAD_A(r, chunk, part)                                                          \
    _Pragma("unroll") for (int it_ = 0; it_ < C::A_ITEMS; ++it_) {                      \
        const float* p_ = in_img + a_src[part][it_] + (chunk) * 32;                     \
        r[it_][0] = *(const f32x4*)p_; r[it_][1] = *(const f32x4*)(p_ + 4);             \
    }
#define F4_(v_) make_float4((v_)[0], (v_)[1], (v_)[2], (v_)[3])
#define STORE_A(buf, part, r)                                                           \
    _Pragma("unroll") for (int it_ = 0; it_ < C::A_ITEMS; ++it_) {                      \
        unsigned char* base_ = Abuf + (buf) * C::A_BUF;                                 \
        uint4 h_, l_;                                                                   \
        split8(F4_(r[it_][0]), F4_(r[it_][1]), h_, l_);                                 \
        *(uint4*)(base_ + a_dst[part][it_]) = h_;                                       \
        *(uint4*)(base_ + C::A_PLANE + a_dst[part][it_]) = l_;                          \
    }
    int b_off[C::B_ITEMS], b_dst[C::B_ITEMS];
#pragma unroll
    for (int it = 0; it < C::B_ITEMS; ++it) {
        if constexpr (NW == 4) {
            const int plane = it / 3, k3 = it % 3, kgi = tid >> 6, co = tid & 63;
            b_off[it] = ((kgi * COUT + co) * 16) + (int)(plane * PL.frag_bytes) + k3 * 4 * COUT * 16;
            b_dst[it] = tid * 16 + plane * C::B_PLANE + k3 * 256 * 16;
        } else {
            const int idx = it * C::NTHR + tid;
            const int plane = idx >= 768, r = idx - plane * 768;
            const int k3 = r >> 8, kgi = (r >> 6) & 3, co = r & 63;
            b_off[it] = (int)(plane * PL.frag_bytes) + ((k3 * 4 + kgi) * COUT + co) * 16;
            b_dst[it] = plane * C::B_PLANE + r * 16;
        }
    }
#define LOAD_B(r, q_, dy_)                                                              \
    {                                                                                   \
        const int cot_ = (q_) / C::NCHUNK, chunk_ = (q_) - cot_ * C::NCHUNK;            \
        const unsigned char* src_ = w_plane0 + ((size_t)(chunk_ * 9 + (dy_) * 3) * 4 * COUT + cot_ * 64) * 16;   \
        _Pragma("unroll") for (int it_ = 0; it_ < C::B_ITEMS; ++it_) r[it_] = *(const u32x4*)(src_ + b_off[it_]); \
    }
#define STORE_B(buf, r)                                                                 \
    { _Pragma("unroll") for (int it_ = 0; it_ < C::B_ITEMS; ++it_) *(u32x4*)(Bbuf + (buf) * C::B_BUF + b_dst[it_]) = r[it_]; }
    struct Frags { bf16x8 wh[4], wl[4], xh[C::MR], xl[C::MR]; };
    auto read_frags = [&](Frags& f, const unsigned char* Ab, const unsigned char* Bb, int k3) {
#pragma unroll
        for (int n = 0; n < 4; ++n) {
            f.wh[n] = __builtin_bit_cast(bf16x8, *(const uint4*)(Bb + (k3 * 256 + n * 16) * 16));
            f.wl[n] = __builtin_bit_cast(bf16x8, *(const uint4*)(Bb + C::B_PLANE + (k3 * 256 + n * 16) * 16));
        }
#pragma unroll
        for (int m = 0; m < C::MR; ++m) {
            f.xh[m] = __builtin_bit_cast(bf16x8, *(const uint4*)(Ab + (m * C::IW + k3) * 16));
            f.xl[m] = __builtin_bit_cast(bf16x8, *(const uint4*)(Ab + C::A_PLANE + (m * C::IW + k3) * 16));
        }
    };

    constexpr int Q = C::NCOT * C::NCHUNK;
    static_assert(Q % 2 == 0, "stage parity is static only for an even number of (slice, chunk) pairs");
    constexpr bool ONE_SET = NW == 4 && !WIDE;
#define RS(i_) (ONE_SET ? 0 : (i_))
    BStage rb[ONE_SET ? 1 : 2];
    APart ra[ONE_SET ? 1 : 2];
    if constexpr (PEEL) {
        BStage rb0;
        LOAD_B(rb0, 0, 0);
        APart r0, r1, r2;
        A_TABLE(0); LOAD_A(r0, 0, 0);
        __builtin_amdgcn_sched_barrier(0);
        A_TABLE(1); LOAD_A(r1, 0, 1);
        __builtin_amdgcn_sched_barrier(0);
        A_TABLE(2); LOAD_A(r2, 0, 2);
        __builtin_amdgcn_sched_barrier(0);
        LOAD_B(rb[1], 0, 1);
        if (C::NCHUNK > 1) LOAD_A(ra[1], 1, 0);
        STORE_B(0, rb0);
        STORE_A(0, 0, r0); STORE_A(0, 1, r1); STORE_A(0, 2, r2);
    } else {
        BStage rb0;
        LOAD_B(rb0, 0, 0);
        APart r0, r1, r2;
        LOAD_A(r0, 0, 0); LOAD_A(r1, 0, 1); LOAD_A(r2, 0, 2);
        LOAD_B(rb[RS(1)], 0, 1);
        if (C::NCHUNK > 1) LOAD_A(ra[RS(1)], 1, 0);
        STORE_A(0, 0, r0); STORE_A(0, 1, r1); STORE_A(0, 2, r2);
        STORE_B(0, rb0);
    }
    __syncthreads();

    f32x4 acc[C::MR][4];
#pragma unroll
    for (int m = 0; m < C::MR; ++m)
#pragma unroll
        for (int n = 0; n < 4; ++n) acc[m][n] = f32x4{0.f, 0.f, 0.f, 0.f};
    const int slot_base = (wave * C::MR) * C::IW + lrow;
    const int oy0 = ty0 + wave * C::MR;
    float4 bias[4], old[C::MR][4];
    const bool full_tile = ty0 + C::TH <= a.Hout && tx0 + 16 <= a.Wout;
    constexpr bool DEFER = OUT_STATE && C::NCOT > 1 && C::NCHUNK == 2;
    bool pending = false;
    int pend_cot = 0;
#define DEFER_UNIT(unit_)                                                                                                             \
    {                                                                                                                                 \
        const int m_ = (unit_) >> 2, n_ = (unit_) & 3;                                                                                \
        if (pending) {                                                             \
            float4* p_ = full_tile ? out_ptr<COUT, OUT_STATE, true>(a, out_img, oy0 + m_, tx0 + lrow, pend_cot * 64 + 4 * kg + n_ * 16) \
                                   : out_ptr<COUT, OUT_STATE, false>(a, out_img, oy0 + m_, tx0 + lrow, pend_cot * 64 + 4 * kg + n_ * 16); \
            if (full_tile || p_) *p_ = old[m_][n_];                                                                                   \
        }                                                                                                                             \
        {                                                                      \
            const float4* q_ = full_tile ? out_ptr<COUT, OUT_STATE, true>(a, out_img, oy0 + m_, tx0 + lrow, cot * 64 + 4 * kg + n_ * 16) \
                                         : out_ptr<COUT, OUT_STATE, false>(a, out_img, oy0 + m_, tx0 + lrow, cot * 64 + 4 * kg + n_ * 16); \
            old[m_][n_] = (full_tile || q_) ? *q_ : make_float4(0.f, 0.f, 0.f, 0.f);                                                  \
        }                                                                                                                             \
    }

    constexpr int NPASS = PEEL ? 2 : 1;
#pragma unroll
    for (int pass = 0; pass < NPASS; ++pass) {
    const bool tail = PEEL && pass == 1;
    const int q0_begin = tail ? Q - 2 : 0, q0_end = (PEEL && !tail) ? Q - 2 : Q;
#pragma unroll 1
    for (int q0v = q0_begin; q0v < q0_end; q0v += 2) {
      const int q0 = tail ? Q - 2 : q0v;
#pragma unroll
      for (int qq = 0; qq < 2; ++qq) {
        const int q = q0 + qq;
        const int cot = q / C::NCHUNK, chunk = q - cot * C::NCHUNK;
        const bool last_chunk = (!PEEL || tail) && chunk == C::NCHUNK - 1;
        const bool first_chunk = PEEL ? tail && qq == 0 : chunk == 0;
#pragma unroll
        for (int dy = 0; dy < 3; ++dy) {
            const int s = q * 3 + dy;
            const int cur = (qq * 3 + dy) & 1;
            if constexpr (WIDE) {
                constexpr bool A_ALWAYS = C::NCOT == 1;
                const int q2 = dy == 0 ? q : q + 1, dy2 = (dy + 2) % 3;
                const int qn = dy == 2 ? q + 1 : q, dyn = (dy + 1) % 3;
                const bool ld_b = !tail || q2 < Q, st_b = !tail || s + 1 < 3 * Q;
                const bool ld_a = A_ALWAYS && (!tail || qn + 1 < C::NCHUNK), st_a = A_ALWAYS && (!tail || q + 1 < C::NCHUNK);
                if (DEFER ? (dy == 2 && last_chunk) : (dy == 0 && first_chunk)) load_bias<COUT, 4>(a, cot * 64 + 4 * kg, bias);
                if (!A_ALWAYS && q < C::NCHUNK - 1) STORE_A((chunk + 1) & 1, dy, ra[cur ^ 1]);
                if (!A_ALWAYS && qn < C::NCHUNK - 1) LOAD_A(ra[cur], qn + 1, dyn);
                if (OUT_STATE && !DEFER && dy == 2 && last_chunk) {
                    if (full_tile) load_old<COUT, C::MR, 4, true>(a, out_img, oy0, tx0 + lrow, cot * 64 + 4 * kg, old);
                    else load_old<COUT, C::MR, 4, false>(a, out_img, oy0, tx0 + lrow, cot * 64 + 4 * kg, old);
                }
                const unsigned char* Ab = Abuf + (chunk & 1) * C::A_BUF + (kg * C::NSLOT + slot_base + dy * C::IW) * 16;
                const unsigned char* Bb = Bbuf + (s & 1) * C::B_BUF + (kg * 64 + lrow) * 16;
                Frags fr[2];
#pragma unroll
                for (int k3 = 0; k3 < 3; ++k3) {
                    if constexpr (DEFER) {
                        if (qq == 0 && dy * 3 + k3 < C::MR * 2) { DEFER_UNIT(2 * (dy * 3 + k3)); DEFER_UNIT(2 * (dy * 3 + k3) + 1); }
                    }
                    if (k3 == 0) read_frags(fr[0], Ab, Bb, 0);
                    __builtin_amdgcn_sched_barrier(0);
                    if (k3 == 0) {
                        if (ld_b) LOAD_B(rb[cur], (PEEL || q2 < Q) ? q2 : Q - 1, dy2);
                        if (ld_a) LOAD_A(ra[cur], qn + 1, dyn);
                    }
                    if (k3 < 2) read_frags(fr[(k3 + 1) & 1], Ab, Bb, k3 + 1);
                    if (k3 == 2) {
                        if (st_b) STORE_B((s + 1) & 1, rb[cur ^ 1]);
                        if (st_a) STORE_A((chunk + 1) & 1, dy, ra[cur ^ 1]);
                    }
                    const Frags& f = fr[k3 & 1];
#pragma unroll
                    for (int m = 0; m < C::MR; ++m)
#pragma unroll
                        for (int n = 0; n < 4; ++n) { MFMA3(acc[m][n], f.wh[n], f.wl[n], f.xh[m], f.xl[m]); }
                    constexpr int NSTB = C::B_ITEMS, NSTG = C::B_ITEMS + 2 * C::A_ITEMS;
                    if (k3 == 0) {
                        if (ld_a) wide_interleave<16, NSTG, 0>();
                        else if (ld_b) wide_interleave<16, NSTB, 0>();
                        else wide_interleave<16, 0, 0>();
                    } else if (k3 == 1) {
                        wide_interleave<16, 0, 0>();
                    } else {
                        if (st_a) wide_interleave<0, 0, NSTG>();
                        else if (st_b) wide_interleave<0, 0, NSTB>();
                        else wide_interleave<0, 0, 0>();
                    }
                    __builtin_amdgcn_sched_barrier(0);
                }
            } else {
#define PIPE_LAND()                                                                                 \
            {                                                                                       \
                if (s + 1 < 3 * Q) STORE_B((s + 1) & 1, rb[RS(cur ^ 1)]);                            \
                if (q < C::NCHUNK - 1) STORE_A((chunk + 1) & 1, dy, ra[RS(cur ^ 1)]);                \
            }
            if constexpr (ONE_SET) { PIPE_LAND(); }
            {
                const int q2 = dy == 0 ? q : q + 1, dy2 = (dy + 2) % 3;
                if (q2 < Q) LOAD_B(rb[RS(cur)], q2, dy2);
                const int qn = dy == 2 ? q + 1 : q, dyn = (dy + 1) % 3;
                if (qn < C::NCHUNK - 1) LOAD_A(ra[RS(cur)], qn + 1, dyn);
            }
            if (DEFER ? (dy == 2 && last_chunk) : (dy == 0 && chunk == 0)) load_bias<COUT, 4>(a, cot * 64 + 4 * kg, bias);
            if (OUT_STATE && !DEFER && dy == 2 && last_chunk) {
                if (full_tile) load_old<COUT, C::MR, 4, true>(a, out_img, oy0, tx0 + lrow, cot * 64 + 4 * kg, old);
                else load_old<COUT, C::MR, 4, false>(a, out_img, oy0, tx0 + lrow, cot * 64 + 4 * kg, old);
            }

            if constexpr (!ONE_SET) { PIPE_LAND(); }
#undef PIPE_LAND

            const unsigned char* Ab = Abuf + (chunk & 1) * C::A_BUF + (kg * C::NSLOT + slot_base + dy * C::IW) * 16;
            const unsigned char* Bb = Bbuf + (s & 1) * C::B_BUF + (kg * 64 + lrow) * 16;
            Frags fr[2];
            read_frags(fr[0], Ab, Bb, 0);
#pragma unroll
            for (int k3 = 0; k3 < 3; ++k3) {
                __builtin_amdgcn_sched_barrier(0);
                if (k3 < 2) read_frags(fr[(k3 + 1) & 1], Ab, Bb, k3 + 1);
                if constexpr (DEFER) {
                    if (qq == 0 && dy * 3 + k3 < C::MR * 4) DEFER_UNIT(dy * 3 + k3);
                }
                __builtin_amdgcn_sched_barrier(0);
                const Frags& f = fr[k3 & 1];
#pragma unroll
                for (int m = 0; m < C::MR; ++m)
#pragma unroll
                    for (int n = 0; n < 4; ++n) { MFMA3(acc[m][n], f.wh[n], f.wl[n], f.xh[m], f.xl[m]); }
            }
            }

            if (DEFER && dy == 2 && last_chunk && cot != C::NCOT - 1) {
#pragma unroll
                for (int m = 0; m < C::MR; ++m)
#pragma unroll
                    for (int n = 0; n < 4; ++n) {
                        const float4 o = old[m][n];
                        old[m][n] = make_float4(o.x + a.sign * (acc[m][n][0] + bias[n].x), o.y + a.sign * (acc[m][n][1] + bias[n].y),
                                                o.z + a.sign * (acc[m][n][2] + bias[n].z), o.w + a.sign * (acc[m][n][3] + bias[n].w));
                        acc[m][n] = f32x4{0.f, 0.f, 0.f, 0.f};
                    }
                pending = true;
                pend_cot = cot;
            } else if (dy == 2 && last_chunk) {
                if (full_tile) store_tile<COUT, OUT_STATE, C::MR, 4, true>(a, out_img, oy0, tx0 + lrow, cot * 64 + 4 * kg, acc, bias, old);
                else store_tile<COUT, OUT_STATE, C::MR, 4, false>(a, out_img, oy0, tx0 + lrow, cot * 64 + 4 * kg, acc, bias, old);
#pragma unroll
                for (int m = 0; m < C::MR; ++m)
#pragma unroll
                    for (int n = 0; n < 4; ++n) acc[m][n] = f32x4{0.f, 0.f, 0.f, 0.f};
            }
            if (DEFER && qq == 0 && dy == 2) pending = false;
            __syncthreads();
        }
      }
    }
    }
#undef A_TABLE
#undef LOAD_A
#undef STORE_A
#undef LOAD_B
#undef STORE_B
#undef F4_
#undef RS
#undef DEFER_UNIT
    VST_TRACE_END_(4, CIN, COUT)
}

template <bool IN_STATE, bool OUT_STATE>
__global__ __launch_bounds__(256) void conv_fp32_kernel(const ConvArgs a, int CIN, int COUT, int STRIDE, int B) {
    const size_t total = (size_t)B * a.Hout * a.Wout * COUT;
    const float* wf = (const float*)a.packed;
    for (size_t idx = (size_t)blockIdx.x * blockDim.x + threadIdx.x; idx < total; idx += (size_t)gridDim.x * blockDim.x) {
        const int co = idx % COUT;
        size_t rest = idx / COUT;
        const int ox = rest % a.Wout; rest /= a.Wout;
        const int oy = rest % a.Hout;
        const int b = rest / a.Hout;
        const float* in_img = a.in + (size_t)b * a.in_img_stride;
        float acc = a.bias[co];
        for (int tap = 0; tap < 9; ++tap) {
            const int gy = reflect_clamp(oy * STRIDE - 1 + tap / 3, a.Hin);
            const int gx = reflect_clamp(ox * STRIDE - 1 + tap % 3, a.Win);
            const float* p = in_img + (IN_STATE ? zc_offset(vst_level_of_channels(CIN), gy, gx, a.Wq)
                                                : ((size_t)gy * a.Win + gx) * CIN);
            const float* w = wf + (size_t)tap * CIN * COUT + co;
            for (int ci = 0; ci < CIN; ++ci) acc = fmaf(p[ci], w[(size_t)ci * COUT], acc);
        }
        float* out_img = a.out + (size_t)b * a.out_img_stride;
        if (OUT_STATE) {
            float* p = out_img + zc_offset(vst_level_of_channels(COUT), oy, ox, a.Wq) + co;
            *p = *p + a.sign * acc;
        } else {
            out_img[((size_t)oy * a.Wout + ox) * COUT + co] = acc > 0.f ? acc : 0.f;
        }
    }
}
template <void (*KERN)(const ConvArgs)>
static int launch_tiles(int threads, int lds_bytes, int tw, int th, int ncot, int B, const ConvArgs& a, hipStream_t st) {
    static std::atomic<unsigned> attr_done{0};
    if (int rc = vst_ensure_dynamic_lds((const void*)KERN, lds_bytes, &attr_done)) return rc;
    ConvArgs t = a;
    t.tiles_x = (a.Wout + tw - 1) / tw; t.tiles_y = (a.Hout + th - 1) / th;
    t.tiles_total = t.tiles_x * t.tiles_y * B * ncot;
    const int grid = (t.tiles_total + 7) / 8 * 8;
    VST_TRACE_RESERVE(t, grid)
    KERN<<<dim3(grid), threads, lds_bytes, st>>>(t);
    VST_RETURN_IF_LAUNCH_FAILED();
    return VST_OK;
}

template <int CIN, int COUT, bool IN_STATE, bool OUT_STATE, int NW, int MR>
static int launch_pipe(const ConvArgs& a, int B, hipStream_t st) {
    using C = PipeCfg<CIN, COUT, NW, MR>;
    return launch_tiles<conv_pipe_kernel<CIN, COUT, IN_STATE, OUT_STATE, NW, MR>>(C::NTHR, C::LDS_BYTES, 16, C::TH, 1, B, a, st);
}

template <int CIN, int COUT, int STRIDE, bool IN_STATE, bool OUT_STATE>
static int launch_conv(const ConvArgs& a, int B, int precision, hipStream_t st, bool out_h16 = false) {
    if (precision == VST_PREC_FP32) {
        const size_t total = (size_t)B * a.Hout * a.Wout * COUT;
        size_t blocks = (total + 255) / 256;
        if (blocks > 65536) blocks = 65536;
        conv_fp32_kernel<IN_STATE, OUT_STATE><<<dim3((unsigned)blocks), 256, 0, st>>>(a, CIN, COUT, STRIDE, B);
        VST_RETURN_IF_LAUNCH_FAILED();
        return VST_OK;
    }
    if (precision != VST_PREC_BF16X3 && !vst_is_f16(precision)) return VST_E_MODE;
    vst_prof_scope prof(VST_KERNEL_ID(CIN, COUT, STRIDE), st);
    if constexpr (CIN >= 64 && COUT >= 64 && STRIDE == 1) {
        if (vst_option(VST_OPT_STAGE3_LEAN)) return launch_pipe<CIN, COUT, IN_STATE, OUT_STATE, 4, 2>(a, B, st);
        if (vst_option(VST_OPT_STAGE3_WIDE)) return launch_pipe<CIN, COUT, IN_STATE, OUT_STATE, 4, 4>(a, B, st);
        return launch_pipe<CIN, COUT, IN_STATE, OUT_STATE, 8, 2>(a, B, st);
    } else {
        using C = ConvCfg<CIN, COUT, STRIDE>;
        constexpr bool T2_SHAPE = (CIN == 64 && COUT == 16) || (CIN == 16 && COUT == 16 && STRIDE == 2) || (CIN == 16 && COUT == 4);
        if constexpr (T2_SHAPE) {
            if (vst_is_f16(precision)) {
                if constexpr (!OUT_STATE) {
                    if (out_h16)
                        return launch_tiles<conv_mfma_kernel<CIN, COUT, STRIDE, IN_STATE, OUT_STATE, false, 2, true>>(
                            256, C::LDS_BYTES_T2, C::TW, C::TH, C::NCOT, B, a, st);
                }
                return launch_tiles<conv_mfma_kernel<CIN, COUT, STRIDE, IN_STATE, OUT_STATE, false, 2>>(
                    256, C::LDS_BYTES_T2, C::TW, C::TH, C::NCOT, B, a, st);
            }
        }
        if constexpr (CIN == 16 && COUT == 4 && STRIDE == 1 && !OUT_STATE) {
            if (vst_option(VST_OPT_STAGE1_FOLD))
                return launch_tiles<conv_mfma_kernel<CIN, COUT, STRIDE, IN_STATE, OUT_STATE, false, 3, false, true>>(
                    256, ConvCfg<CIN, COUT, STRIDE, 0, 2>::LDS_BYTES, C::TW, C::TH, C::NCOT, B, a, st);
        }
        return launch_tiles<conv_mfma_kernel<CIN, COUT, STRIDE, IN_STATE, OUT_STATE, false, 3>>(
            256, C::LDS_BYTES, C::TW, C::TH, C::NCOT, B, a, st);
    }
}

static int launch_conv_s2_planes(const ConvArgs& a, int B, hipStream_t st) {
    using C = ConvCfg<64, 64, 2>;
    vst_prof_scope prof(VST_KERNEL_ID(64, 64, 2), st);
    return launch_tiles<conv_mfma_kernel<64, 64, 2, true, false, true, 2>>(256, C::LDS_BYTES_T2, C::TW, C::TH, C::NCOT, B, a, st);
}

template <int MID, int CH>
static int launch_pair(const ConvArgs& a, int B, int precision, hipStream_t st) {
    const bool t2 = vst_is_f16(precision), h16 = precision == VST_PREC_F16X2H;
    vst_prof_scope prof(VST_KERNEL_ID(MID, CH, 1), st);
    if constexpr (MID == 4) {
        if (a.rgb || a.rgb_u8) {
            constexpr int LDS = PairCfg<MID, CH, 3>::LDS_BYTES;
            static_assert(LDS >= PairCfg<MID, CH, 2>::LDS_BYTES && LDS >= PairCfg<MID, CH, 2, 4, true>::LDS_BYTES, "");
            if (h16) return launch_tiles<conv_pair_kernel<MID, CH, 2, 4, true, true>>(256, LDS, 16, 16, 1, B, a, st);
            if (t2) return launch_tiles<conv_pair_kernel<MID, CH, 2, 4, false, true>>(256, LDS, 16, 16, 1, B, a, st);
            return launch_tiles<conv_pair_kernel<MID, CH, 3, 4, false, true>>(256, LDS, 16, 16, 1, B, a, st);
        }
    }
    if (h16) return launch_tiles<conv_pair_kernel<MID, CH, 2, 4, true>>(256, PairCfg<MID, CH, 2, 4, true>::LDS_BYTES, 16, 16, 1, B, a, st);
    if (t2) return launch_tiles<conv_pair_kernel<MID, CH, 2>>(256, PairCfg<MID, CH, 2>::LDS_BYTES, 16, 16, 1, B, a, st);
    return launch_tiles<conv_pair_kernel<MID, CH, 3>>(256, PairCfg<MID, CH, 3>::LDS_BYTES, 16, 16, 1, B, a, st);
}

template <int CH, int STRIDE>
static int run_block(const vst_block_weights* w, int direction, int precision, float* dst, const float* src,
                     float* tmp, int B, int H, int W, hipStream_t st, float* rgb = nullptr, uint8_t* rgb_u8 = nullptr,
                     int rgb_c = 0) {
    constexpr int LV = CH == 16 ? 0 : (CH == 64 ? 1 : 2);
    constexpr int MID = CH / 4;
    constexpr int IN_CH = STRIDE == 1 ? CH : CH / 4;
    const int Ho = H >> LV, Wo = W >> LV;
    const size_t state_img = (size_t)H * W * 16;
    const size_t mid_img = (size_t)Ho * Wo * MID;
    float* h1 = tmp;
    float* h2 = tmp + (size_t)B * mid_img;
    ConvArgs a{};
    a.Wq = W >> 2;
    a.in = src; a.out = h1; a.packed = (const unsigned char*)w->conv[0].packed; a.bias = w->conv[0].bias;
    a.Hin = Ho * STRIDE; a.Win = Wo * STRIDE; a.Hout = Ho; a.Wout = Wo;
    a.in_img_stride = state_img; a.out_img_stride = mid_img; a.sign = 0.f;
    if constexpr (CH == 256 && STRIDE == 2) {
        if (vst_is_f16(precision)) {
            const size_t mid_bytes = (size_t)Ho * Wo * 64 * 4;
            unsigned char* const h1p = (unsigned char*)tmp;
            unsigned char* const h2p = h1p + (size_t)B * mid_bytes;
            unsigned char* const planes_a = h2p + (size_t)B * mid_bytes;
            a.out_sp = h1p; a.out_sp_img_bytes = mid_bytes;
            int rc2 = launch_conv_s2_planes(a, B, st);
            if (rc2) return rc2;
            const int h2_single = precision == VST_PREC_F16X2H;
            rc2 = vst3_conv_mid(&w->conv[1], h1p, h2p, h2_single, B, H, W, st);
            if (rc2) return rc2;
            return vst3_conv_out(&w->conv[2], h2p, h2_single, dst, direction > 0 ? planes_a : nullptr, direction > 0 ? 1.f : -1.f,
                                 B, H, W, st);
        }
    }
    const bool h16 = CH <= 64 && precision == VST_PREC_F16X2H;
    int rc = launch_conv<IN_CH, MID, STRIDE, true, false>(a, B, precision, st, h16);
    if (rc) return rc;
    if constexpr (CH <= 64) {
        if (precision != VST_PREC_FP32) {
            a.in = h1; a.out = dst; a.Hin = Ho; a.Win = Wo; a.in_img_stride = mid_img; a.out_img_stride = state_img;
            a.packed = (const unsigned char*)w->conv[2].packed; a.bias = w->conv[2].bias;
            a.packed1 = (const unsigned char*)w->conv[1].packed; a.bias1 = w->conv[1].bias;
            a.sign = direction > 0 ? 1.f : -1.f;
            a.rgb = rgb; a.rgb_u8 = rgb_u8; a.rgb_c = rgb_c;
            return launch_pair<MID, CH>(a, B, precision, st);
        }
    }
    a.in = h1; a.out = h2; a.packed = (const unsigned char*)w->conv[1].packed; a.bias = w->conv[1].bias;
    a.Hin = Ho; a.Win = Wo; a.in_img_stride = mid_img;
    rc = launch_conv<MID, MID, 1, false, false>(a, B, precision, st);
    if (rc) return rc;
    a.in = h2; a.out = dst; a.packed = (const unsigned char*)w->conv[2].packed; a.bias = w->conv[2].bias;
    a.out_img_stride = state_img; a.sign = direction > 0 ? 1.f : -1.f;
    return launch_conv<MID, CH, 1, false, true>(a, B, precision, st);
}

VST_DEFINE_TU_RANGE(vst_range_tu_conv)

int vst_block0_to_image(const vst_block_weights* w0, int precision, float* dst, const float* src, float* tmp, int B, int H,
                        int W, float* rgb, uint8_t* rgb_u8, int rgb_c, void* stream) {
    return run_block<16, 1>(w0, -1, precision, dst, src, tmp, B, H, W, (hipStream_t)stream, rgb, rgb_u8, rgb_c);
}

extern "C" {

size_t vst_block_tmp_bytes(int B, int H, int W) { return (size_t)B * H * W * 40 * sizeof(float); }

int vst_block_apply(const vst_block_weights* w, int channel, int stride, int direction, int precision,
                    float* dst, const float* src, void* tmp, int B, int H, int W, void* stream) {
    if (!w || !dst || !src || !tmp) return VST_E_ARG;
    if (!vst_shape_ok(B, H, W)) return VST_E_SHAPE;
    if (direction != 1 && direction != -1) return VST_E_MODE;
    for (int i = 0; i < 3; ++i)
        if (!w->conv[i].packed || !w->conv[i].bias) return VST_E_ARG;
    hipStream_t st = (hipStream_t)stream;
    float* t = (float*)tmp;
    if (channel == 16 && stride == 1) return run_block<16, 1>(w, direction, precision, dst, src, t, B, H, W, st);
    if (channel == 64 && stride == 1) return run_block<64, 1>(w, direction, precision, dst, src, t, B, H, W, st);
    if (channel == 64 && stride == 2) return run_block<64, 2>(w, direction, precision, dst, src, t, B, H, W, st);
    if (channel == 256 && stride == 1) {
        if (vst_is_f16(precision)) return vst3_block256(w, direction, precision, dst, src, tmp, -1, 0, B, H, W, stream);
        return run_block<256, 1>(w, direction, precision, dst, src, t, B, H, W, st);
    }
    if (channel == 256 && stride == 2) return run_block<256, 2>(w, direction, precision, dst, src, t, B, H, W, st);
    return VST_E_SHAPE;
}

}
```

vstnet_amd/csrc/layout.hip:

```cpp
#include "common.h"

__global__ __launch_bounds__(256) void pack_input_kernel(const float* __restrict__ x, float* __restrict__ s1,
                                                         int C, int H, int W, const float* __restrict__ addk) {
    const int xg = blockIdx.x * 64 + (threadIdx.x & 63);
    const int yg = blockIdx.y * 4 + (threadIdx.x >> 6);
    const int b = blockIdx.z;
    if (xg >= W || yg >= H) return;
    const size_t plane = (size_t)H * W;
    const float* src = x + (size_t)b * C * plane + (size_t)yg * W + xg;
    float v[16];
#pragma unroll
    for (int c = 0; c < 16; ++c) v[c] = (c < C ? src[c * plane] : 0.f) + (addk ? addk[c] : 0.f);
    float* dst = s1 + (size_t)b * plane * 16 + zc_offset(0, yg, xg, W >> 2);
#pragma unroll
    for (int c = 0; c < 16; c += 4) *(float4*)(dst + c) = make_float4(v[c], v[c + 1], v[c + 2], v[c + 3]);
}

__global__ __launch_bounds__(256) void unpack_output_kernel(const float* __restrict__ s1, float* __restrict__ x,
                                                            int C, int H, int W) {
    const int xg = blockIdx.x * 64 + (threadIdx.x & 63);
    const int yg = blockIdx.y * 4 + (threadIdx.x >> 6);
    const int b = blockIdx.z;
    if (xg >= W || yg >= H) return;
    const size_t plane = (size_t)H * W;
    const float* src = s1 + (size_t)b * plane * 16 + zc_offset(0, yg, xg, W >> 2);
    float* dst = x + (size_t)b * C * plane + (size_t)yg * W + xg;
    for (int c = 0; c < C; ++c) dst[c * plane] = src[c];
}

__global__ __launch_bounds__(256) void pack_input_u8_kernel(const uint8_t* __restrict__ img, float* __restrict__ s1,
                                                            int H, int W, const float* __restrict__ addk) {
    const int xg = blockIdx.x * 64 + (threadIdx.x & 63);
    const int yg = blockIdx.y * 4 + (threadIdx.x >> 6);
    const int b = blockIdx.z;
    if (xg >= W || yg >= H) return;
    const uint8_t* src = img + ((size_t)b * H * W + (size_t)yg * W + xg) * 3;
    float* dst = s1 + (size_t)b * H * W * 16 + zc_offset(0, yg, xg, W >> 2);
    float k[16];
#pragma unroll
    for (int c = 0; c < 16; ++c) k[c] = addk ? addk[c] : 0.f;
    *(float4*)(dst) = make_float4((float)src[0] / 255.f + k[0], (float)src[1] / 255.f + k[1], (float)src[2] / 255.f + k[2], k[3]);
    *(float4*)(dst + 4) = make_float4(k[4], k[5], k[6], k[7]);
    *(float4*)(dst + 8) = make_float4(k[8], k[9], k[10], k[11]);
    *(float4*)(dst + 12) = make_float4(k[12], k[13], k[14], k[15]);
}

__global__ __launch_bounds__(256) void unpack_output_u8_kernel(const float* __restrict__ s1, uint8_t* __restrict__ img,
                                                               int H, int W) {
    const int xg = blockIdx.x * 64 + (threadIdx.x & 63);
    const int yg = blockIdx.y * 4 + (threadIdx.x >> 6);
    const int b = blockIdx.z;
    if (xg >= W || yg >= H) return;
    const float4 v = *(const float4*)(s1 + (size_t)b * H * W * 16 + zc_offset(0, yg, xg, W >> 2));
    uint8_t* dst = img + ((size_t)b * H * W + (size_t)yg * W + xg) * 3;
    const float c[3] = {v.x, v.y, v.z};
#pragma unroll
    for (int k = 0; k < 3; ++k) {
        float t = c[k] * 255.f;
        t = t < 0.f ? 0.f : (t > 255.f ? 255.f : t);
        dst[k] = (uint8_t)t;
    }
}

__global__ void block0_const_kernel(const float* __restrict__ w2, const float* __restrict__ w3,
                                    const float* __restrict__ b1, const float* __restrict__ b2,
                                    const float* __restrict__ b3, float* __restrict__ k) {
    __shared__ float h1[4], h2[4];
    const int t = threadIdx.x;
    if (t < 4) h1[t] = b1[t] > 0.f ? b1[t] : 0.f;
    __syncthreads();
    if (t < 4) {
        float acc = b2[t];
        for (int tap = 0; tap < 9; ++tap)
            for (int ci = 0; ci < 4; ++ci) acc = fmaf(w2[(tap * 4 + ci) * 4 + t], h1[ci], acc);
        h2[t] = acc > 0.f ? acc : 0.f;
    }
    __syncthreads();
    if (t < 16) {
        float acc = b3[t];
        for (int tap = 0; tap < 9; ++tap)
            for (int ci = 0; ci < 4; ++ci) acc = fmaf(w3[(tap * 4 + ci) * 16 + t], h2[ci], acc);
        k[t] = acc;
    }
}

template <int SP>
struct SpreadGeom {
    static constexpr int CELL_STRIDE = SP == 2 ? 324 : 258;
    __device__ static __forceinline__ int lds_index(int slot, int c) {
        if (SP == 2) {
            const int g = c >> 5, d = c & 31;
            return slot * 324 + (g >> 2) * 162 + ((g >> 1) & 1) * 66 + (g & 1) * 33 + d;
        } else {
            return slot * 258 + (c >> 7) * 129 + (c & 127);
        }
    }
};

template <int SP, bool TO_Z, bool PLANES = false>
__global__ __launch_bounds__(256) void spread_gather_kernel(float* __restrict__ s1, float* __restrict__ s2,
                                                            float* __restrict__ z, int H, int W,
                                                            unsigned char* __restrict__ sp1 = nullptr) {
    __shared__ float lds[32 * SpreadGeom<SP>::CELL_STRIDE];
    const int Hq = H >> 2, Wq = W >> 2;
    const int w0 = blockIdx.x * 16, h = blockIdx.y, b = blockIdx.z;
    const int t = threadIdx.x;
    const size_t img = (size_t)Hq * Wq * 256;
    float* half[2] = {s1 + (size_t)b * img, s2 + (size_t)b * img};

    auto state_phase = [&]() {
        if (PLANES) {
            unsigned char* const sp_img = sp1 + (size_t)b * img * 4;
#pragma unroll
            for (int it = 0; it < 2; ++it) {
                const int idx = it * 256 + t;
                const int cell = idx & 15, cig = idx >> 4;
                const int w = w0 + cell;
                if (w >= Wq) continue;
                const int cot = cig >> 3, j = (cig >> 2) & 1, kg = cig & 3;
                const int li = SpreadGeom<SP>::lds_index(cell, cot * 64 + j * 32 + kg * 4);
                const float f8[8] = {lds[li], lds[li + 1], lds[li + 2], lds[li + 3], lds[li + 16], lds[li + 17], lds[li + 18], lds[li + 19]};
                u32x4 hi, lo;
                split8_sp(f8, hi, lo);
                *(u32x4*)(sp_img + sp_offset(cig, 0, h, w, Hq, Wq)) = hi;
                *(u32x4*)(sp_img + sp_offset(cig, 1, h, w, Hq, Wq)) = lo;
            }
        }
#pragma unroll
        for (int it = PLANES ? 4 : 0; it < 8; ++it) {
            const int idx = it * 256 + t;
            const int slot = idx >> 6, q = idx & 63;
            const int w = w0 + (slot & 15);
            if (w >= Wq) continue;
            float* p = half[slot >> 4] + ((size_t)h * Wq + w) * 256 + q * 4;
            const int li = SpreadGeom<SP>::lds_index(slot, q * 4);
            if (TO_Z) {
                const float4 v = *(const float4*)p;
                lds[li] = v.x; lds[li + 1] = v.y; lds[li + 2] = v.z; lds[li + 3] = v.w;
            } else {
                *(float4*)p = make_float4(lds[li], lds[li + 1], lds[li + 2], lds[li + 3]);
            }
        }
    };
    auto z_phase = [&]() {
        if (SP == 2) {
            const int X = t & 63, wave = t >> 6;
            const int wl = X >> 2, j = (X >> 1) & 1, jp = X & 1;
            const int xg = w0 * 4 + X;
#pragma unroll 8
            for (int it = 0; it < 32; ++it) {
                const int combo = it * 4 + wave;
                const int d = combo >> 2, Yl = combo & 3;
                const int i = Yl >> 1, ip = Yl & 1;
                if (xg >= W) continue;
                float* p = z + (((size_t)b * 32 + d) * H + (4 * h + Yl)) * W + xg;
                const int li = (i * 16 + wl) * 324 + j * 162 + ip * 66 + jp * 33 + d;
                if (TO_Z) *p = lds[li]; else lds[li] = *p;
            }
        } else {
            const int H2 = H >> 1, W2 = W >> 1;
            const int X = t & 31, dsel = (t >> 5) & 1, wave = t >> 6;
            const int wl = X >> 1, j = X & 1;
            const int xg = w0 * 2 + X;
#pragma unroll 8
            for (int it = 0; it < 32; ++it) {
                const int combo = (it * 4 + wave) * 2 + dsel;
                const int d = combo >> 1, i = combo & 1;
                if (xg >= W2) continue;
                float* p = z + (((size_t)b * 128 + d) * H2 + (2 * h + i)) * W2 + xg;
                const int li = (i * 16 + wl) * 258 + j * 129 + d;
                if (TO_Z) *p = lds[li]; else lds[li] = *p;
            }
        }
    };
    if (TO_Z) { state_phase(); __syncthreads(); z_phase(); }
    else      { z_phase(); __syncthreads(); state_phase(); }
}

__global__ void pack_conv_kernel(const float* __restrict__ w, int cout, int cin, unsigned char* __restrict__ packed) {
    const PackedConvLayout L = packed_conv_layout(cout, cin);
    const size_t n_f32 = (size_t)9 * cin * cout;
    const size_t n_frag = (size_t)L.ksteps * 4 * L.coutp * 8;
    const size_t idx = (size_t)blockIdx.x * blockDim.x + threadIdx.x;
    if (idx < n_f32) {
        const int co = idx % cout;
        const int ci = (idx / cout) % cin;
        const int tap = idx / ((size_t)cout * cin);
        ((float*)packed)[idx] = w[((size_t)co * cin + ci) * 9 + tap];
    }
    if (idx < n_frag) {
        const int j = idx & 7;
        const int co = (idx >> 3) % L.coutp;
        const int kg = (idx >> 3) / L.coutp % 4;
        const int ks = (idx >> 3) / L.coutp / 4;
        int tap, ci;
        if (cin >= 32) { tap = ks % 9; ci = (ks / 9) * 32 + kg * 8 + j; }
        else if (cin == 16) { tap = 2 * ks + (kg >> 1); ci = (kg & 1) * 8 + j; }
        else { tap = 8 * ks + 2 * kg + (j >> 2); ci = j & 3; }
        float v = 0.f;
        if (tap < 9 && co < cout && ci < cin) v = w[((size_t)co * cin + ci) * 9 + tap];
        const __bf16 hi = (__bf16)v;
        const __bf16 lo = (__bf16)(v - (float)hi);
        ((__bf16*)(packed + L.f32_bytes))[idx] = hi;
        ((__bf16*)(packed + L.f32_bytes + L.frag_bytes))[idx] = lo;
        ((_Float16*)(packed + L.f16_offset))[idx] = (_Float16)v;
        if (fabsf(v) > 65504.f) atomicOr(&vst_tu_range_flags, VST_RANGE_WEIGHT);
        if (L.sp_sections) {
            const int cip = (ks / 9) * 32 + (j >> 2) * 16 + kg * 4 + (j & 3);
            const float vp = co < cout ? w[((size_t)co * cin + cip) * 9 + tap] : 0.f;
            unsigned char* sp = packed + L.f32_bytes + 2 * L.frag_bytes;
            ((_Float16*)sp)[idx] = (_Float16)vp;
        }
    }
}

__device__ __forceinline__ float pow2_scale_of_norm(float sumsq) {
    const float nrm = sqrtf(sumsq);
    if (!(nrm > 0.f) || !(nrm < 3.0e38f)) return 1.f;
    int e;
    const float m = frexpf(nrm, &e);
    int r = m >= 0.70710678f ? e : e - 1;
    r = r > 40 ? 40 : (r < -40 ? -40 : r);
    return ldexpf(1.f, -r);
}

__global__ __launch_bounds__(256) void normalize_block_kernel(float* __restrict__ w1, float* __restrict__ b1, float* __restrict__ w4,
                                                              float* __restrict__ b4, float* __restrict__ w7, int cin1, int mid,
                                                              int cout, float* __restrict__ scales) {
    __shared__ float sc[64];
    const int tid = threadIdx.x, lane = tid & 63, wave = tid >> 6;
    auto row_scales = [&](const float* w, int K) {
        for (int r = wave; r < mid; r += 4) {
            float acc = 0.f;
            for (int k = lane; k < K; k += 64) { const float v = w[(size_t)r * K + k]; acc += v * v; }
#pragma unroll
            for (int o = 32; o >= 1; o >>= 1) acc += __shfl_xor(acc, o, 64);
            if (lane == 0) sc[r] = pow2_scale_of_norm(acc);
        }
        __syncthreads();
    };
    const int K1 = cin1 * 9, K4 = mid * 9;
    row_scales(w1, K1);
    for (int i = tid; i < mid * K1; i += 256) w1[i] *= sc[i / K1];
    for (int i = tid; i < mid; i += 256) { b1[i] *= sc[i]; if (scales) scales[i] = sc[i]; }
    for (int i = tid; i < mid * K4; i += 256) w4[i] /= sc[(i / 9) % mid];
    __syncthreads();
    row_scales(w4, K4);
    for (int i = tid; i < mid * K4; i += 256) w4[i] *= sc[i / K4];
    for (int i = tid; i < mid; i += 256) { b4[i] *= sc[i]; if (scales) scales[mid + i] = sc[i]; }
    for (int i = tid; i < cout * K4; i += 256) w7[i] /= sc[(i / 9) % mid];
}

VST_DEFINE_TU_RANGE(vst_range_tu_layout)

extern "C" {

int vst_version(void) { return 113; }
int64_t vst_max_frame_pixels(void) { return VST_MAX_FRAME_PIXELS; }

int vst_normalize_block(float* w1, float* b1, float* w4, float* b4, float* w7, int c_in1, int c_mid, int c_out, float* scales,
                        void* stream) {
    if (!w1 || !b1 || !w4 || !b4 || !w7) return VST_E_ARG;
    if (c_in1 <= 0 || c_mid <= 0 || c_mid > 64 || c_out <= 0) return VST_E_SHAPE;
    normalize_block_kernel<<<dim3(1), 256, 0, (hipStream_t)stream>>>(w1, b1, w4, b4, w7, c_in1, c_mid, c_out, scales);
    VST_RETURN_IF_LAUNCH_FAILED();
    return VST_OK;
}

const char* vst_error_string(int code) {
    switch (code) {
        case VST_OK: return "ok";
        case VST_E_ARG: return "invalid argument (null pointer or non-positive size)";
        case VST_E_SHAPE: return "unsupported shape (H, W must be multiples of 4 and >= 8, H * W <= VST_MAX_FRAME_PIXELS; channels in the documented sets)";
        case VST_E_MODE: return "unknown mode (precision / sp_steps / direction)";
        case VST_E_WORKSPACE: return "workspace too small or null";
        default: return code > 0 ? hipGetErrorString((hipError_t)code) : "unknown vstnet error";
    }
}

size_t vst_conv_packed_bytes(int cout, int cin) {
    const PackedConvLayout L = packed_conv_layout(cout, cin);
    return L.f16_offset + L.frag_bytes;
}

int vst_pack_conv(const float* w, int cout, int cin, void* packed, void* stream) {
    if (!w || !packed || cout <= 0) return VST_E_ARG;
    if (!(cin == 4 || cin == 16 || (cin >= 32 && cin % 32 == 0))) return VST_E_SHAPE;
    const PackedConvLayout L = packed_conv_layout(cout, cin);
    size_t n = (size_t)9 * cin * cout;
    const size_t n_frag = (size_t)L.ksteps * 4 * L.coutp * 8;
    if (n_frag > n) n = n_frag;
    pack_conv_kernel<<<dim3((unsigned)((n + 255) / 256)), 256, 0, (hipStream_t)stream>>>(w, cout, cin, (unsigned char*)packed);
    VST_RETURN_IF_LAUNCH_FAILED();
    return VST_OK;
}

int vst_pack_input_k(const float* x, const uint8_t* x_u8, float* s1, float* s2, int B, int C, int H, int W,
                     const float* addk, void* stream) {
    if ((!x && !x_u8) || !s1 || !s2) return VST_E_ARG;
    if (!vst_shape_ok(B, H, W) || C < 1 || C > 16) return VST_E_SHAPE;
    hipStream_t st = (hipStream_t)stream;
    hipError_t e = hipMemsetAsync(s2, 0, (size_t)B * H * W * 16 * sizeof(float), st);
    if (e != hipSuccess) return (int)e;
    const dim3 grid((W + 63) / 64, (H + 3) / 4, B);
    vst_prof_scope prof(VST_KERNEL_PACK, st);
    if (x_u8) pack_input_u8_kernel<<<grid, 256, 0, st>>>(x_u8, s1, H, W, addk);
    else pack_input_kernel<<<grid, 256, 0, st>>>(x, s1, C, H, W, addk);
    VST_RETURN_IF_LAUNCH_FAILED();
    return VST_OK;
}

int vst_block0_const(const vst_block_weights* w0, float* k16, void* stream) {
    if (!w0 || !k16) return VST_E_ARG;
    block0_const_kernel<<<1, 64, 0, (hipStream_t)stream>>>((const float*)w0->conv[1].packed, (const float*)w0->conv[2].packed,
                                                           w0->conv[0].bias, w0->conv[1].bias, w0->conv[2].bias, k16);
    VST_RETURN_IF_LAUNCH_FAILED();
    return VST_OK;
}

int vst_pack_input(const float* x, float* s1, float* s2, int B, int C, int H, int W, void* stream) {
    if (!x) return VST_E_ARG;
    return vst_pack_input_k(x, nullptr, s1, s2, B, C, H, W, nullptr, stream);
}

int vst_unpack_output(const float* s1, float* x, int B, int C, int H, int W, void* stream) {
    if (!x || !s1) return VST_E_ARG;
    if (!vst_shape_ok(B, H, W) || C < 1 || C > 16) return VST_E_SHAPE;
    vst_prof_scope prof(VST_KERNEL_UNPACK, (hipStream_t)stream);
    unpack_output_kernel<<<dim3((W + 63) / 64, (H + 3) / 4, B), 256, 0, (hipStream_t)stream>>>(s1, x, C, H, W);
    VST_RETURN_IF_LAUNCH_FAILED();
    return VST_OK;
}

int vst_pack_input_u8(const uint8_t* frames_hwc, float* s1, float* s2, int B, int H, int W, void* stream) {
    if (!frames_hwc) return VST_E_ARG;
    return vst_pack_input_k(nullptr, frames_hwc, s1, s2, B, 3, H, W, nullptr, stream);
}

int vst_unpack_output_u8(const float* s1, uint8_t* frames_hwc, int B, int H, int W, void* stream) {
    if (!frames_hwc || !s1) return VST_E_ARG;
    if (!vst_shape_ok(B, H, W)) return VST_E_SHAPE;
    vst_prof_scope prof(VST_KERNEL_UNPACK, (hipStream_t)stream);
    unpack_output_u8_kernel<<<dim3((W + 63) / 64, (H + 3) / 4, B), 256, 0, (hipStream_t)stream>>>(s1, frames_hwc, H, W);
    VST_RETURN_IF_LAUNCH_FAILED();
    return VST_OK;
}

int vst_spread(const float* s1, const float* s2, float* z, int B, int H, int W, int sp_steps, void* stream) {
    if (!s1 || !s2 || !z) return VST_E_ARG;
    if (!vst_shape_ok(B, H, W)) return VST_E_SHAPE;
    const dim3 grid((W / 4 + 15) / 16, H / 4, B);
    hipStream_t st = (hipStream_t)stream;
    vst_prof_scope prof(VST_KERNEL_SPREAD, st);
    if (sp_steps == 2) spread_gather_kernel<2, true><<<grid, 256, 0, st>>>((float*)s1, (float*)s2, z, H, W);
    else if (sp_steps == 1) spread_gather_kernel<1, true><<<grid, 256, 0, st>>>((float*)s1, (float*)s2, z, H, W);
    else return VST_E_MODE;
    VST_RETURN_IF_LAUNCH_FAILED();
    return VST_OK;
}

int vst3_gather_planes(const float* z, unsigned char* s1_planes, float* s2, int B, int H, int W, int sp_steps, void* stream) {
    if (!s1_planes || !s2 || !z) return VST_E_ARG;
    if (!vst_shape_ok(B, H, W)) return VST_E_SHAPE;
    const dim3 grid((W / 4 + 15) / 16, H / 4, B);
    hipStream_t st = (hipStream_t)stream;
    vst_prof_scope prof(VST_KERNEL_GATHER, st);
    if (sp_steps == 2) spread_gather_kernel<2, false, true><<<grid, 256, 0, st>>>(nullptr, s2, (float*)z, H, W, s1_planes);
    else if (sp_steps == 1) spread_gather_kernel<1, false, true><<<grid, 256, 0, st>>>(nullptr, s2, (float*)z, H, W, s1_planes);
    else return VST_E_MODE;
    VST_RETURN_IF_LAUNCH_FAILED();
    return VST_OK;
}

int vst_gather(const float* z, float* s1, float* s2, int B, int H, int W, int sp_steps, void* stream) {
    if (!s1 || !s2 || !z) return VST_E_ARG;
    if (!vst_shape_ok(B, H, W)) return VST_E_SHAPE;
    const dim3 grid((W / 4 + 15) / 16, H / 4, B);
    hipStream_t st = (hipStream_t)stream;
    vst_prof_scope prof(VST_KERNEL_GATHER, st);
    if (sp_steps == 2) spread_gather_kernel<2, false><<<grid, 256, 0, st>>>(s1, s2, (float*)z, H, W);
    else if (sp_steps == 1) spread_gather_kernel<1, false><<<grid, 256, 0, st>>>(s1, s2, (float*)z, H, W);
    else return VST_E_MODE;
    VST_RETURN_IF_LAUNCH_FAILED();
    return VST_OK;
}

}
```

vstnet_amd/csrc/revnet.hip:

```cpp
#include "common.h"

static const int kBlockChannel[VST_NUM_BLOCKS] = {16, 16, 16, 16, 16, 16, 16, 16, 16, 16, 64, 64, 64, 64, 64, 64,
                                                  64, 64, 64, 64, 256, 256, 256, 256, 256, 256, 256, 256, 256, 256,
                                                  256, 256};
static const int kBlockStride[VST_NUM_BLOCKS] = {1, 1, 1, 1, 1, 1, 1, 1, 1, 1, 2, 1, 1, 1, 1, 1,
                                                 1, 1, 1, 1, 2, 1, 1, 1, 1, 1, 1, 1, 1, 1, 1, 1};

static int pass_sub_batch(int B, int H, int W) {
    const size_t per_img = (size_t)H * W * 288;
    size_t nb = ((size_t)192 << 20) / per_img;
    if (nb < 1) nb = 1;
    return nb > (size_t)B ? B : (int)nb;
}

static int forward_blocks(const vst_net_weights* w, const float* x, const uint8_t* x_u8, float* const s[2], float* tmp, int B,
                          int C_in, int H, int W, int precision, void* stream) {
    const bool fold0 = precision != VST_PREC_FP32;
    float* k16 = tmp;
    int rc = fold0 ? vst_block0_const(&w->blocks[0], k16, stream) : VST_OK;
    if (rc) return rc;
    rc = vst_pack_input_k(x, x_u8, s[0], s[1], B, x_u8 ? 3 : C_in, H, W, fold0 ? k16 : nullptr, stream);
    if (rc) return rc;
    const bool sp = vst_is_f16(precision);
    for (int k = fold0 ? 1 : 0; k < VST_NUM_BLOCKS; ++k) {
        if (sp && k >= 21)
            rc = vst3_block256(&w->blocks[k], +1, precision, s[k & 1], s[1 - (k & 1)], tmp, k - 21, 1, B, H, W, stream);
        else
            rc = vst_block_apply(&w->blocks[k], kBlockChannel[k], kBlockStride[k], +1, precision, s[k & 1], s[1 - (k & 1)],
                                 tmp, B, H, W, stream);
        if (rc) return rc;
    }
    return VST_OK;
}

static int inverse_blocks(const vst_net_weights* w, float* x, uint8_t* x_u8, float* const s[2], float* tmp, int B, int C_out,
                          int H, int W, int precision, void* stream) {
    const bool sp = vst_is_f16(precision);
    int rc = VST_OK;
    const bool rgb0 = precision != VST_PREC_FP32 && vst_option(VST_OPT_OUT_RGB);
    if (rgb0) {
        if ((!x && !x_u8) || !vst_shape_ok(B, H, W) || (!x_u8 && (C_out < 1 || C_out > 16))) return VST_E_ARG;
        for (int i = 0; i < 3; ++i)
            if (!w->blocks[0].conv[i].packed || !w->blocks[0].conv[i].bias) return VST_E_ARG;
    }
    for (int k = VST_NUM_BLOCKS - 1; k >= 0; --k) {
        if (sp && k >= 21)
            rc = vst3_block256(&w->blocks[k], -1, precision, s[k & 1], s[1 - (k & 1)], tmp, VST_NUM_BLOCKS - 1 - k, 1, B, H, W,
                               stream);
        else if (k == 0 && rgb0)
            return vst_block0_to_image(&w->blocks[0], precision, s[0], s[1], tmp, B, H, W, x_u8 ? nullptr : x, x_u8, C_out, stream);
        else
            rc = vst_block_apply(&w->blocks[k], kBlockChannel[k], kBlockStride[k], -1, precision, s[k & 1], s[1 - (k & 1)],
                                 tmp, B, H, W, stream);
        if (rc) return rc;
    }
    return x_u8 ? vst_unpack_output_u8(s[0], x_u8, B, H, W, stream) : vst_unpack_output(s[0], x, B, C_out, H, W, stream);
}

static int revnet_forward_any(const vst_net_weights* w, const float* x, const uint8_t* x_u8, float* z, void* workspace,
                              int B, int C_in, int H, int W, int sp_steps, int precision, void* stream) {
    if (!w || (!x && !x_u8) || !z) return VST_E_ARG;
    if (!workspace) return VST_E_WORKSPACE;
    if (!vst_shape_ok(B, H, W) || C_in < 1 || C_in > 16) return VST_E_SHAPE;
    if (sp_steps != 1 && sp_steps != 2) return VST_E_MODE;
    const int nb = pass_sub_batch(B, H, W);
    const size_t zimg = (size_t)32 * H * W;
    for (int b0 = 0; b0 < B; b0 += nb) {
        const int n = B - b0 < nb ? B - b0 : nb;
        float* s[2] = {(float*)workspace, (float*)workspace + n * (zimg / 2)};
        float* tmp = s[1] + n * (zimg / 2);
        int rc = forward_blocks(w, x ? x + (size_t)b0 * C_in * H * W : nullptr, x_u8 ? x_u8 + (size_t)b0 * H * W * 3 : nullptr, s,
                                tmp, n, C_in, H, W, precision, stream);
        if (!rc) rc = vst_spread(s[0], s[1], z + b0 * zimg, n, H, W, sp_steps, stream);
        if (rc) return rc;
    }
    return VST_OK;
}

static int revnet_inverse_any(const vst_net_weights* w, const float* z, float* x, uint8_t* x_u8, void* workspace, int B,
                              int C_out, int H, int W, int sp_steps, int precision, void* stream) {
    if (!w || (!x && !x_u8) || !z) return VST_E_ARG;
    if (!workspace) return VST_E_WORKSPACE;
    if (!vst_shape_ok(B, H, W) || C_out < 1 || C_out > 16) return VST_E_SHAPE;
    if (sp_steps != 1 && sp_steps != 2) return VST_E_MODE;
    const int nb = pass_sub_batch(B, H, W);
    const size_t zimg = (size_t)32 * H * W;
    for (int b0 = 0; b0 < B; b0 += nb) {
        const int n = B - b0 < nb ? B - b0 : nb;
        float* s[2] = {(float*)workspace, (float*)workspace + n * (zimg / 2)};
        float* tmp = s[1] + n * (zimg / 2);
        int rc = vst_is_f16(precision)
                     ? vst3_gather_planes(z + b0 * zimg, vst3_plane_buffer(tmp, 0, n, H, W), s[1], n, H, W, sp_steps, stream)
                     : vst_gather(z + b0 * zimg, s[0], s[1], n, H, W, sp_steps, stream);
        if (!rc) rc = inverse_blocks(w, x ? x + (size_t)b0 * C_out * H * W : nullptr, x_u8 ? x_u8 + (size_t)b0 * H * W * 3 : nullptr,
                                     s, tmp, n, C_out, H, W, precision, stream);
        if (rc) return rc;
    }
    return VST_OK;
}

static int revnet_encode_any(const vst_net_weights* w, const float* x, const uint8_t* x_u8, float* code, void* workspace, int B,
                             int C_in, int H, int W, int precision, void* stream) {
    if (!w || (!x && !x_u8) || !code) return VST_E_ARG;
    if (!workspace) return VST_E_WORKSPACE;
    if (!vst_shape_ok(B, H, W) || C_in < 1 || C_in > 16) return VST_E_SHAPE;
    const size_t img = (size_t)32 * H * W;
    float* tmp = (float*)workspace + img;
    for (int b = 0; b < B; ++b) {
        float* s[2] = {code + b * img, code + b * img + img / 2};
        const int rc = forward_blocks(w, x ? x + (size_t)b * C_in * H * W : nullptr, x_u8 ? x_u8 + (size_t)b * H * W * 3 : nullptr,
                                      s, tmp, 1, C_in, H, W, precision, stream);
        if (rc) return rc;
    }
    return VST_OK;
}

static int revnet_decode_labels_any(const vst_net_weights* w, const float* code, const float* affines, const uint8_t* mask_rows,
                                    const void* plan, int max_slots, const float* strength_rows, float* x, uint8_t* x_u8,
                                    void* workspace, int C_out, int H, int W, int precision, void* stream) {
    if (!w || (!x && !x_u8) || !code || !affines || !mask_rows || !plan) return VST_E_ARG;
    if (!workspace) return VST_E_WORKSPACE;
    if (!vst_shape_ok(1, H, W) || C_out < 1 || C_out > 16 || max_slots < 1 || max_slots > 8) return VST_E_SHAPE;
    const size_t img = (size_t)32 * H * W;
    float* s[2] = {(float*)workspace, (float*)workspace + img / 2};
    float* tmp = (float*)workspace + img;
    unsigned char* planes0 = vst_is_f16(precision) ? vst3_plane_buffer(tmp, 0, 1, H, W) : nullptr;
    int rc = vst3_apply_labels_code(code, s[0], s[1], planes0, H, W, affines, mask_rows, plan, max_slots, strength_rows, stream);
    if (rc) return rc;
    return inverse_blocks(w, x, x_u8, s, tmp, 1, C_out, H, W, precision, stream);
}

static int revnet_decode_any(const vst_net_weights* w, const float* code, const float* affines, const float* strength_rows,
                             float* x, uint8_t* x_u8, void* workspace, int B, int C_out, int H, int W, int sp_steps, int precision,
                             void* stream, int K = 0, const float* weight_rows = nullptr) {
    if (!w || (!x && !x_u8) || !code) return VST_E_ARG;
    if (K != 0 && (K < 2 || K > CWCT_MAX_STYLES || !affines || !weight_rows)) return VST_E_ARG;
    if (!workspace) return VST_E_WORKSPACE;
    if (!vst_shape_ok(B, H, W) || C_out < 1 || C_out > 16) return VST_E_SHAPE;
    if (sp_steps != 1 && sp_steps != 2) return VST_E_MODE;
    if (K != 0 && sp_steps == 1 && K != 2) return VST_E_MODE;
    const int N = sp_steps == 2 ? 32 : 128;
    const size_t img = (size_t)32 * H * W, rows = img / N;
    float* s[2] = {(float*)workspace, (float*)workspace + img / 2};
    float* tmp = (float*)workspace + img;
    const bool sp = vst_is_f16(precision);
    unsigned char* planes0 = sp ? vst3_plane_buffer(tmp, 0, 1, H, W) : nullptr;
    hipStream_t st = (hipStream_t)stream;
    for (int b = 0; b < B; ++b) {
        const float* c = code + b * img;
        int rc;
        if (K) {
            rc = vst3_apply_code_mix(c, s[0], s[1], planes0, H, W, sp_steps, affines + (size_t)b * K * ((size_t)N * N + N), K,
                                     weight_rows + (size_t)b * K * rows, strength_rows ? strength_rows + (size_t)b * rows : nullptr,
                                     stream);
        } else if (affines) {
            rc = vst3_apply_code(c, s[0], s[1], planes0, H, W, sp_steps, affines + (size_t)b * ((size_t)N * N + N),
                                 strength_rows ? strength_rows + (size_t)b * rows : nullptr, stream);
        } else {
            rc = sp ? vst3_presplit(c, planes0, 1, H, W, stream)
                    : (int)hipMemcpyAsync(s[0], c, img / 2 * sizeof(float), hipMemcpyDeviceToDevice, st);
            if (!rc) rc = (int)hipMemcpyAsync(s[1], c + img / 2, img / 2 * sizeof(float), hipMemcpyDeviceToDevice, st);
        }
        if (rc) return rc;
        rc = inverse_blocks(w, x ? x + (size_t)b * C_out * H * W : nullptr, x_u8 ? x_u8 + (size_t)b * H * W * 3 : nullptr, s, tmp,
                            1, C_out, H, W, precision, stream);
        if (rc) return rc;
    }
    return VST_OK;
}

extern "C" {

size_t vst_pass_workspace_bytes(int B, int H, int W) { return (size_t)B * H * W * (16 + 16 + 40) * sizeof(float); }

int vst_pass_sub_batch(int B, int H, int W) {
    if (!vst_shape_ok(B, H, W)) return VST_E_SHAPE;
    return pass_sub_batch(B, H, W);
}

int vst_revnet_forward(const vst_net_weights* w, const float* x, float* z, void* workspace, int B, int C_in, int H,
                       int W, int sp_steps, int precision, void* stream) {
    if (!x) return VST_E_ARG;
    return revnet_forward_any(w, x, nullptr, z, workspace, B, C_in, H, W, sp_steps, precision, stream);
}

int vst_revnet_inverse(const vst_net_weights* w, const float* z, float* x, void* workspace, int B, int C_out, int H,
                       int W, int sp_steps, int precision, void* stream) {
    if (!x) return VST_E_ARG;
    return revnet_inverse_any(w, z, x, nullptr, workspace, B, C_out, H, W, sp_steps, precision, stream);
}

int vst_revnet_forward_u8(const vst_net_weights* w, const uint8_t* frames_hwc, float* z, void* workspace, int B, int H,
                          int W, int sp_steps, int precision, void* stream) {
    if (!frames_hwc) return VST_E_ARG;
    return revnet_forward_any(w, nullptr, frames_hwc, z, workspace, B, 3, H, W, sp_steps, precision, stream);
}

int vst_revnet_inverse_u8(const vst_net_weights* w, const float* z, uint8_t* frames_hwc, void* workspace, int B, int H,
                          int W, int sp_steps, int precision, void* stream) {
    if (!frames_hwc) return VST_E_ARG;
    return revnet_inverse_any(w, z, nullptr, frames_hwc, workspace, B, 3, H, W, sp_steps, precision, stream);
}

int vst_revnet_encode(const vst_net_weights* w, const float* x, float* code, void* workspace, int B, int C_in, int H, int W,
                      int precision, void* stream) {
    if (!x) return VST_E_ARG;
    return revnet_encode_any(w, x, nullptr, code, workspace, B, C_in, H, W, precision, stream);
}

int vst_revnet_encode_u8(const vst_net_weights* w, const uint8_t* frames_hwc, float* code, void* workspace, int B, int H, int W,
                         int precision, void* stream) {
    if (!frames_hwc) return VST_E_ARG;
    return revnet_encode_any(w, nullptr, frames_hwc, code, workspace, B, 3, H, W, precision, stream);
}

int vst_revnet_decode_blend(const vst_net_weights* w, const float* code, const float* affines, const float* strength_rows,
                            float* x, void* workspace, int B, int C_out, int H, int W, int sp_steps, int precision, void* stream) {
    if (!x) return VST_E_ARG;
    return revnet_decode_any(w, code, affines, strength_rows, x, nullptr, workspace, B, C_out, H, W, sp_steps, precision, stream);
}

int vst_revnet_decode_blend_u8(const vst_net_weights* w, const float* code, const float* affines, const float* strength_rows,
                               uint8_t* frames_hwc, void* workspace, int B, int H, int W, int sp_steps, int precision,
                               void* stream) {
    if (!frames_hwc) return VST_E_ARG;
    return revnet_decode_any(w, code, affines, strength_rows, nullptr, frames_hwc, workspace, B, 3, H, W, sp_steps, precision,
                             stream);
}

int vst_revnet_decode_mix(const vst_net_weights* w, const float* code, const float* affines, int K, const float* weight_rows,
                          const float* strength_rows, float* x, void* workspace, int B, int C_out, int H, int W, int sp_steps,
                          int precision, void* stream) {
    if (!x || !affines || !weight_rows || K < 2 || K > CWCT_MAX_STYLES) return VST_E_ARG;
    return revnet_decode_any(w, code, affines, strength_rows, x, nullptr, workspace, B, C_out, H, W, sp_steps, precision, stream, K,
                             weight_rows);
}

int vst_revnet_decode_mix_u8(const vst_net_weights* w, const float* code, const float* affines, int K, const float* weight_rows,
                             const float* strength_rows, uint8_t* frames_hwc, void* workspace, int B, int H, int W, int sp_steps,
                             int precision, void* stream) {
    if (!frames_hwc || !affines || !weight_rows || K < 2 || K > CWCT_MAX_STYLES) return VST_E_ARG;
    return revnet_decode_any(w, code, affines, strength_rows, nullptr, frames_hwc, workspace, B, 3, H, W, sp_steps, precision,
                             stream, K, weight_rows);
}

int vst_revnet_decode(const vst_net_weights* w, const float* code, const float* affines, float* x, void* workspace, int B,
                      int C_out, int H, int W, int sp_steps, int precision, void* stream) {
    return vst_revnet_decode_blend(w, code, affines, nullptr, x, workspace, B, C_out, H, W, sp_steps, precision, stream);
}

int vst_revnet_decode_u8(const vst_net_weights* w, const float* code, const float* affines, uint8_t* frames_hwc, void* workspace,
                         int B, int H, int W, int sp_steps, int precision, void* stream) {
    return vst_revnet_decode_blend_u8(w, code, affines, nullptr, frames_hwc, workspace, B, H, W, sp_steps, precision, stream);
}

int vst_revnet_decode_labels_blend(const vst_net_weights* w, const float* code, const float* affines, const uint8_t* mask_rows,
                                   const void* plan, int max_slots, const float* strength_rows, float* x, void* workspace,
                                   int C_out, int H, int W, int precision, void* stream) {
    if (!x) return VST_E_ARG;
    return revnet_decode_labels_any(w, code, affines, mask_rows, plan, max_slots, strength_rows, x, nullptr, workspace, C_out, H,
                                    W, precision, stream);
}

int vst_revnet_decode_labels_blend_u8(const vst_net_weights* w, const float* code, const float* affines, const uint8_t* mask_rows,
                                      const void* plan, int max_slots, const float* strength_rows, uint8_t* frame_hwc,
                                      void* workspace, int H, int W, int precision, void* stream) {
    if (!frame_hwc) return VST_E_ARG;
    return revnet_decode_labels_any(w, code, affines, mask_rows, plan, max_slots, strength_rows, nullptr, frame_hwc, workspace, 3,
                                    H, W, precision, stream);
}

int vst_revnet_decode_labels(const vst_net_weights* w, const float* code, const float* affines, const uint8_t* mask_rows,
                             const void* plan, int max_slots, float* x, void* workspace, int C_out, int H, int W, int precision,
                             void* stream) {
    return vst_revnet_decode_labels_blend(w, code, affines, mask_rows, plan, max_slots, nullptr, x, workspace, C_out, H, W,
                                          precision, stream);
}

int vst_revnet_decode_labels_u8(const vst_net_weights* w, const float* code, const float* affines, const uint8_t* mask_rows,
                                const void* plan, int max_slots, uint8_t* frame_hwc, void* workspace, int H, int W, int precision,
                                void* stream) {
    return vst_revnet_decode_labels_blend_u8(w, code, affines, mask_rows, plan, max_slots, nullptr, frame_hwc, workspace, H, W,
                                             precision, stream);
}

int vst_code_to_z(const float* code, float* z, int B, int H, int W, int sp_steps, void* stream) {
    if (!code || !z) return VST_E_ARG;
    const size_t img = (size_t)32 * H * W;
    for (int b = 0; b < B; ++b) {
        const int rc = vst_spread(code + b * img, code + b * img + img / 2, z + b * img, 1, H, W, sp_steps, stream);
        if (rc) return rc;
    }
    return VST_OK;
}

int vst_z_to_code(const float* z, float* code, int B, int H, int W, int sp_steps, void* stream) {
    if (!code || !z) return VST_E_ARG;
    const size_t img = (size_t)32 * H * W;
    for (int b = 0; b < B; ++b) {
        const int rc = vst_gather(z + b * img, code + b * img, code + b * img + img / 2, 1, H, W, sp_steps, stream);
        if (rc) return rc;
    }
    return VST_OK;
}

}
```

vstnet_amd/csrc/runtime.hip:

```cpp
#include <mutex>
#include <stdlib.h>
#include "common.h"

static const struct { const char* env; int def; } kOptions[] = {
    {nullptr, 0},
    {"VST_LEAN", 0},
    {nullptr, 0},
    {"VST_WIDE", 1},
    {"VST_FOLD16", 1},
    {"VST_OUT_RGB", 1},
};
constexpr int kNumOptions = sizeof(kOptions) / sizeof(kOptions[0]);
static std::atomic<int> g_options[kNumOptions];
static const bool g_options_ready = [] {
    for (int i = 0; i < kNumOptions; ++i) {
        const char* e = kOptions[i].env ? getenv(kOptions[i].env) : nullptr;
        g_options[i].store(e && (e[0] == '0' || e[0] == '1') ? e[0] - '0' : kOptions[i].def, std::memory_order_relaxed);
    }
    return true;
}();
static bool option_ok(int option) { return option > 0 && option < kNumOptions && kOptions[option].env; }

int vst_option(int option) { return g_options[option].load(std::memory_order_relaxed); }

#define VST_PROFILE_MAX_RECORDS 4096
static std::mutex g_prof_mu;
static std::atomic<int> g_prof_kernel{0};
static int g_prof_count = 0, g_prof_cap = 0;
static int g_prof_id[VST_PROFILE_MAX_RECORDS];
static hipEvent_t g_prof_ev[2 * VST_PROFILE_MAX_RECORDS];
static bool g_prof_ev_created = false;

int vst_prof_open(int kernel_id, hipStream_t st) {
    const int sel = g_prof_kernel.load(std::memory_order_relaxed);
    if (sel != kernel_id && sel != VST_KERNEL_ALL) return -1;
    std::lock_guard<std::mutex> lk(g_prof_mu);
    if ((g_prof_kernel.load() != kernel_id && g_prof_kernel.load() != VST_KERNEL_ALL) || g_prof_count >= g_prof_cap) return -1;
    const int rec = g_prof_count++;
    g_prof_id[rec] = kernel_id;
    (void)hipEventRecord(g_prof_ev[2 * rec], st);
    return rec;
}

void vst_prof_close(int rec, hipStream_t st) {
    std::lock_guard<std::mutex> lk(g_prof_mu);
    if (rec < g_prof_count) (void)hipEventRecord(g_prof_ev[2 * rec + 1], st);
}

extern "C" {

int vst_set_option(int option, int value) {
    if (!option_ok(option)) return VST_E_ARG;
    g_options[option].store(value != 0, std::memory_order_relaxed);
    return VST_OK;
}

int vst_get_option(int option) { return option_ok(option) ? vst_option(option) : VST_E_ARG; }

int vst_range_flags(unsigned* flags_host, int reset) {
    if (!flags_host) return VST_E_ARG;
    hipError_t e = hipDeviceSynchronize();
    if (e != hipSuccess) return (int)e;
    unsigned v = 0;
    if (int rc = vst_range_tu_conv(&v, reset)) return rc;
    if (int rc = vst_range_tu_conv3(&v, reset)) return rc;
    if (int rc = vst_range_tu_layout(&v, reset)) return rc;
    if (int rc = vst_range_tu_cwct(&v, reset)) return rc;
    *flags_host = v;
    return VST_OK;
}

int vst_range_flags_async(unsigned* flags4_dev, void* stream) {
    if (!flags4_dev) return VST_E_ARG;
    hipStream_t st = (hipStream_t)stream;
    if (int rc = vst_range_tu_conv_async(flags4_dev + 0, st)) return rc;
    if (int rc = vst_range_tu_conv3_async(flags4_dev + 1, st)) return rc;
    if (int rc = vst_range_tu_layout_async(flags4_dev + 2, st)) return rc;
    return vst_range_tu_cwct_async(flags4_dev + 3, st);
}

int vst_profile_begin(int kernel_id, int max_records) {
    if ((kernel_id <= 0 && kernel_id != VST_KERNEL_ALL) || max_records <= 0) return VST_E_ARG;
    if (max_records > VST_PROFILE_MAX_RECORDS) max_records = VST_PROFILE_MAX_RECORDS;
    std::lock_guard<std::mutex> lk(g_prof_mu);
    if (!g_prof_ev_created) {
        for (int i = 0; i < 2 * VST_PROFILE_MAX_RECORDS; ++i) {
            hipError_t e = hipEventCreate(&g_prof_ev[i]);
            if (e != hipSuccess) return (int)e;
        }
        g_prof_ev_created = true;
    }
    g_prof_count = 0; g_prof_cap = max_records;
    g_prof_kernel.store(kernel_id);
    return VST_OK;
}

int vst_profile_end(double* total_ms, int* launches) {
    if (!total_ms || !launches) return VST_E_ARG;
    std::lock_guard<std::mutex> lk(g_prof_mu);
    g_prof_kernel.store(0);
    double tot = 0.0;
    for (int i = 0; i < g_prof_count; ++i) {
        hipError_t e = hipEventSynchronize(g_prof_ev[2 * i + 1]);
        if (e != hipSuccess) return (int)e;
        float ms = 0.f;
        e = hipEventElapsedTime(&ms, g_prof_ev[2 * i], g_prof_ev[2 * i + 1]);
        if (e != hipSuccess) return (int)e;
        tot += ms;
    }
    *total_ms = tot; *launches = g_prof_count;
    g_prof_count = 0; g_prof_cap = 0;
    return VST_OK;
}

int vst_profile_end_table(int* ids, double* ms, int* launches, int cap, int* n_ids) {
    if (!ids || !ms || !launches || !n_ids || cap <= 0) return VST_E_ARG;
    std::lock_guard<std::mutex> lk(g_prof_mu);
    g_prof_kernel.store(0);
    int n = 0;
    for (int i = 0; i < g_prof_count; ++i) {
        hipError_t e = hipEventSynchronize(g_prof_ev[2 * i + 1]);
        if (e != hipSuccess) return (int)e;
        float t = 0.f;
        e = hipEventElapsedTime(&t, g_prof_ev[2 * i], g_prof_ev[2 * i + 1]);
        if (e != hipSuccess) return (int)e;
        int k = 0;
        while (k < n && ids[k] != g_prof_id[i]) ++k;
        if (k == n) {
            if (n == cap) continue;
            ids[n] = g_prof_id[i]; ms[n] = 0.0; launches[n] = 0; ++n;
        }
        ms[k] += t; launches[k] += 1;
    }
    *n_ids = n;
    g_prof_count = 0; g_prof_cap = 0;
    return VST_OK;
}

}
```

Measured before the change: 221.1.

## Add row-band scheduling for stage 1/2 revnet block chains

```diff
diff --git a/include/vstnet.h b/include/vstnet.h
--- a/include/vstnet.h
+++ b/include/vstnet.h
@@ -243,8 +243,11 @@
 #define VST_OPT_STAGE3_WIDE 3
 #define VST_OPT_STAGE1_FOLD 4
 #define VST_OPT_OUT_RGB 5
+#define VST_OPT_BANDS 7
 int vst_set_option(int option, int value);
 int vst_get_option(int option);
+
+int vst_band_schedule(int stage, int direction, int H, int W, int bands, int* out, int cap);
 
 #define VST_RESIZE_MAX_SHRINK 16
 int vst_resize_coeffs_u8(int in_size, int out_size, int* ksize, int* bounds, int* kk);
diff --git a/vstnet_amd/_lib.py b/vstnet_amd/_lib.py
--- a/vstnet_amd/_lib.py
+++ b/vstnet_amd/_lib.py
@@ -54,6 +54,7 @@
     "vst_strength_frame", "vst_resize_coeffs_u8_bilinear", "vst_resize_grey_u8",
     "vst_cwct_apply_code_mix", "vst_revnet_decode_mix", "vst_revnet_decode_mix_u8", "vst_cwct_mix_acc",
     "vst_cwct_stats_pool",
+    "vst_band_schedule",
 ]
 MAX_STYLES = 8
 SEG_MIX_MAX = 8
@@ -67,6 +68,7 @@
 OPT_STAGE3_WIDE = 3
 OPT_STAGE1_FOLD = 4
 OPT_OUT_RGB = 5
+OPT_BANDS = 7
 RANGE_SATURATED = 1
 RANGE_WEIGHT = 2
 
@@ -282,6 +284,7 @@
         "vst_seg_head_sum": (i, [vp, vp, vp, vp, C.POINTER(i), i, vp, vp]),
         "vst_set_option": (i, [i, i]),
         "vst_get_option": (i, [i]),
+        "vst_band_schedule": (i, [i, i, i, i, i, C.POINTER(i), i]),
         "vst_profile_begin": (i, [i, i]),
         "vst_profile_end": (i, [C.POINTER(C.c_double), C.POINTER(i)]),
         "vst_profile_end_table": (i, [C.POINTER(i), C.POINTER(C.c_double), C.POINTER(i), i, C.POINTER(i)]),
@@ -321,6 +324,14 @@
     return v
 
 
+def band_schedule(stage: int, direction: int, H: int, W: int, bands: int):
+    out = (C.c_int * (3 * 64))()
+    n = lib().vst_band_schedule(stage, direction, H, W, bands, out, 64)
+    if n < 0:
+        check(n, "vst_band_schedule")
+    return [(out[3 * e], out[3 * e + 1], out[3 * e + 2]) for e in range(n)]
+
+
 def kernel_id(cin: int, cout: int, stride: int) -> int:
     return (cin << 16) | (cout << 4) | stride
 
diff --git a/vstnet_amd/csrc/common.h b/vstnet_amd/csrc/common.h
--- a/vstnet_amd/csrc/common.h
+++ b/vstnet_amd/csrc/common.h
@@ -136,12 +136,12 @@
 };
 static_assert(sizeof(LabelPlan) == VST_LABEL_PLAN_BYTES, "vstnet.h: VST_LABEL_PLAN_BYTES");
 
-int vst_prof_open(int kernel_id, hipStream_t st);
+int vst_prof_open(int kernel_id, hipStream_t st, bool counted = true);
 void vst_prof_close(int rec, hipStream_t st);
 struct vst_prof_scope {
     int rec;
     hipStream_t st;
-    vst_prof_scope(int kernel_id, hipStream_t s) : rec(vst_prof_open(kernel_id, s)), st(s) {}
+    vst_prof_scope(int kernel_id, hipStream_t s, bool counted = true) : rec(vst_prof_open(kernel_id, s, counted)), st(s) {}
     ~vst_prof_scope() { if (rec >= 0) vst_prof_close(rec, st); }
 };
 int vst_option(int option);
@@ -153,7 +153,9 @@
                   int H, int W, void* stream);
 static inline bool vst_is_f16(int precision) { return precision == VST_PREC_F16X2 || precision == VST_PREC_F16X2H; }
 int vst_block0_to_image(const vst_block_weights* w0, int precision, float* dst, const float* src, float* tmp, int B, int H,
-                        int W, float* rgb, uint8_t* rgb_u8, int rgb_c, void* stream);
+                        int W, float* rgb, uint8_t* rgb_u8, int rgb_c, void* stream, int y0 = 0, int y1 = 0, bool counted = true);
+int vst_block_band(const vst_block_weights* w, int channel, int direction, int precision, float* dst, const float* src, float* tmp,
+                   int B, int H, int W, int y0, int y1, bool counted, void* stream);
 
 unsigned char* vst3_plane_buffer(void* tmp, int idx, int B, int H, int W);
 extern "C" __attribute__((visibility("hidden"))) int vst3_gather_planes(const float* z, unsigned char* s1_planes, float* s2, int B, int H, int W, int sp_steps,
diff --git a/vstnet_amd/csrc/conv.hip b/vstnet_amd/csrc/conv.hip
--- a/vstnet_amd/csrc/conv.hip
+++ b/vstnet_amd/csrc/conv.hip
@@ -19,6 +19,7 @@
     float* rgb;
     unsigned char* rgb_u8;
     int rgb_c;
+    int y_begin, y_end;
 };
 
 #ifdef VST_TRACE
@@ -164,7 +165,7 @@
 
 template <int COUT, bool OUT_STATE, bool FULL = false>
 __device__ __forceinline__ float4* out_ptr(const ConvArgs& a, float* out_img, int oy, int ox, int co) {
-    if (!FULL && (oy >= a.Hout || ox >= a.Wout || co >= COUT)) return nullptr;
+    if (!FULL && (oy >= a.y_end || ox >= a.Wout || co >= COUT)) return nullptr;
     if (OUT_STATE) return (float4*)(out_img + zc_offset(vst_level_of_channels(COUT), oy, ox, a.Wq) + co);
     return (float4*)(out_img + ((size_t)oy * a.Wout + ox) * COUT + co);
 }
@@ -237,7 +238,7 @@
     if (!xcd_tile(a, bx, by, bz)) return;
     float range_amax = 0.f;
     VST_TRACE_BEGIN(2)
-    const int tx0 = bx * C::TW, ty0 = by * C::TH;
+    const int tx0 = bx * C::TW, ty0 = a.y_begin + by * C::TH;
     const int b = bz / C::NCOT, co0 = (bz % C::NCOT) * C::NT;
 
     const float* const in_img = a.in + (size_t)b * a.in_img_stride;
@@ -284,7 +285,8 @@
         idx = idx < A_ITEMS_T ? idx : A_ITEMS_T - 1;                                               \
         const int cig = CIN == 4 ? 0 : idx % C::CIG, slot = CIN == 4 ? idx : idx / C::CIG;         \
         const int iy = slot / C::IW, ix = slot - iy * C::IW;                                       \
-        const int gy = reflect_clamp(ty0 * STRIDE - 1 + iy, a.Hin);                                \
+        int gy = reflect_clamp(ty0 * STRIDE - 1 + iy, a.Hin);                                      \
+        if (STRIDE == 1) gy = min(max(gy, a.y_begin - 1), a.y_end);    \
         const int gx = reflect_clamp(tx0 * STRIDE - 1 + ix, a.Win);                                \
         const size_t off = IN_STATE ? zc_offset(vst_level_of_channels(CIN), gy, gx, a.Wq)          \
                                     : ((size_t)gy * a.Win + gx) * CIN;                             \
@@ -318,7 +320,7 @@
 
     float* const out_img = a.out + (size_t)b * a.out_img_stride;
     float4 bias[C::NB], old[C::MR][C::NB];
-    const bool interior = COUT % 16 == 0 && ty0 + C::TH <= a.Hout && tx0 + C::TW <= a.Wout;
+    const bool interior = COUT % 16 == 0 && ty0 + C::TH <= a.y_end && tx0 + C::TW <= a.Wout;
     constexpr bool EARLY_OLD = OUT_STATE && C::MR * C::NB >= 16;
     auto fetch_old = [&]() __attribute__((always_inline)) {
         if (interior) load_old<COUT, C::MR, C::NB, true>(a, out_img, ty0 + wave * C::MR, tx0 + lrow, co0 + 4 * kg, old);
@@ -364,7 +366,7 @@
         const f32x4 d2 = *(const f32x4*)(sc + ((q0 + 2) * 3 + 2) * 4);
         const float4 bs = *(const float4*)a.bias;
         const int oy = ty0 + wave * C::MR + kg, ox = tx0 + lrow;
-        if (oy < a.Hout && ox < a.Wout) {
+        if (oy < a.y_end && ox < a.Wout) {
             float4 r = make_float4((d0[0] + d1[0]) + d2[0] + bs.x, (d0[1] + d1[1]) + d2[1] + bs.y,
                                    (d0[2] + d1[2]) + d2[2] + bs.z, (d0[3] + d1[3]) + d2[3] + bs.w);
             r.x = r.x > 0.f ? r.x : 0.f; r.y = r.y > 0.f ? r.y : 0.f;
@@ -437,7 +439,7 @@
 #pragma unroll
         for (int m = 0; m < C::MR; ++m) {
             const int oy = ty0 + wave * C::MR + m, ox = tx0 + lrow;
-            if (oy >= a.Hout || ox >= a.Wout) continue;
+            if (oy >= a.y_end || ox >= a.Wout) continue;
 #pragma unroll
             for (int j = 0; j < 2; ++j) {
                 float f8[8];
@@ -465,7 +467,7 @@
 #pragma unroll
             for (int n = 0; n < C::NB; ++n) {
                 const int oy = ty0 + wave * C::MR + m, ox = tx0 + lrow, co = co0 + 4 * kg + n * 16;
-                if (oy >= a.Hout || ox >= a.Wout || co >= COUT) continue;
+                if (oy >= a.y_end || ox >= a.Wout || co >= COUT) continue;
                 const float r[4] = {acc[m][n][0] + bias[n].x, acc[m][n][1] + bias[n].y, acc[m][n][2] + bias[n].z, acc[m][n][3] + bias[n].w};
                 typedef __attribute__((ext_vector_type(4))) _Float16 f16x4;
                 f16x4 h;
@@ -548,7 +550,8 @@
     if (!xcd_tile(a, bx, by, b)) return;
     float range_amax = 0.f;
     VST_TRACE_BEGIN(1)
-    const int tx0 = bx * C::TW, ty0 = by * C::TH;
+    __builtin_assume((a.y_begin & 3) == 0);
+    const int tx0 = bx * C::TW, ty0 = a.y_begin + by * C::TH;
     const int H = a.Hout, W = a.Wout;
     const float* const in_img = a.in + (size_t)b * a.in_img_stride;
     float* const out_img = a.out + (size_t)b * a.out_img_stride;
@@ -578,7 +581,7 @@
         idx = idx < H1_ITEMS ? idx : H1_ITEMS - 1;
         const int cig = MID == 4 ? 0 : idx % C::CIG, slot = MID == 4 ? idx : idx / C::CIG;
         const int iy = slot / P::R1, ix = slot - iy * P::R1;
-        const int gy = reflect_clamp(ty0 - 2 + iy, H), gx = reflect_clamp(tx0 - 2 + ix, W);
+        const int gy = min(max(reflect_clamp(ty0 - 2 + iy, H), a.y_begin - 2), a.y_end + 1), gx = reflect_clamp(tx0 - 2 + ix, W);
         if constexpr (H16) {
             const _Float16* p16 = (const _Float16*)a.in + (size_t)b * a.in_img_stride + ((size_t)gy * W + gx) * MID + cig * 8;
             if (MID == 4) { const uint2 v = *(const uint2*)p16; h16reg[it] = u32x4{v.x, v.y, 0u, 0u}; }
@@ -599,7 +602,7 @@
         if (TERMS == 3) w7reg[it][1] = *(const u32x4*)(w7_lo + src);
     }
     float4 bias[C::NB], old[C::MR][C::NB];
-    const bool interior = ty0 + C::TH <= H && tx0 + C::TW <= W;
+    const bool interior = ty0 + C::TH <= a.y_end && tx0 + C::TW <= W;
     constexpr bool EARLY_OLD = C::MR * C::NB >= 16 && TERMS == 3 && !OUT_RGB;
 #define PAIR_FETCH_OLD()                                                                                         \
     if (interior) load_old<CH, C::MR, C::NB, true>(a, out_img, ty0 + wave * C::MR, tx0 + lrow, 4 * kg, old);   \
@@ -652,7 +655,7 @@
     {
         float4 b4 = make_float4(0.f, 0.f, 0.f, 0.f);
         if (4 * kg < MID) b4 = *(const float4*)(a.bias1 + 4 * kg);
-        const bool ring_inside = ty0 >= 1 && tx0 >= 1 && ty0 + C::TH + 1 <= H && tx0 + 17 <= W;
+        const bool ring_inside = ty0 >= 1 && tx0 >= 1 && ty0 + C::TH + 1 <= H && tx0 + 17 <= W && ty0 + C::TH <= a.y_end;
         constexpr bool HOIST = MID == 4;
         bf16x8 w4h[HOIST ? C::KS : 1], w4l[HOIST ? C::KS : 1];
         if (HOIST) {
@@ -770,7 +773,7 @@
 #pragma unroll
         for (int m = 0; m < C::MR; ++m) {
             const int oy = ty0 + wave * C::MR + m;
-            if (oy >= H || ox >= W || 4 * kg >= nc) continue;
+            if (oy >= a.y_end || ox >= W || 4 * kg >= nc) continue;
             const float4 o = *(const float4*)(out_img + zc_offset(0, oy, ox, a.Wq) + 4 * kg);
             float4 r = make_float4(acc[m][0][0] + bias[0].x, acc[m][0][1] + bias[0].y, acc[m][0][2] + bias[0].z,
                                    acc[m][0][3] + bias[0].w);
@@ -1161,7 +1164,9 @@
     static std::atomic<unsigned> attr_done{0};
     if (int rc = vst_ensure_dynamic_lds((const void*)KERN, lds_bytes, &attr_done)) return rc;
     ConvArgs t = a;
-    t.tiles_x = (a.Wout + tw - 1) / tw; t.tiles_y = (a.Hout + th - 1) / th;
+    if (t.y_end == 0) { t.y_begin = 0; t.y_end = a.Hout; }
+    if (t.y_begin < 0 || t.y_end > a.Hout || t.y_begin >= t.y_end) return VST_E_ARG;
+    t.tiles_x = (a.Wout + tw - 1) / tw; t.tiles_y = (t.y_end - t.y_begin + th - 1) / th;
     t.tiles_total = t.tiles_x * t.tiles_y * B * ncot;
     const int grid = (t.tiles_total + 7) / 8 * 8;
     VST_TRACE_RESERVE(t, grid)
@@ -1177,7 +1182,7 @@
 }
 
 template <int CIN, int COUT, int STRIDE, bool IN_STATE, bool OUT_STATE>
-static int launch_conv(const ConvArgs& a, int B, int precision, hipStream_t st, bool out_h16 = false) {
+static int launch_conv(const ConvArgs& a, int B, int precision, hipStream_t st, bool out_h16 = false, bool counted = true) {
     if (precision == VST_PREC_FP32) {
         const size_t total = (size_t)B * a.Hout * a.Wout * COUT;
         size_t blocks = (total + 255) / 256;
@@ -1187,7 +1192,7 @@
         return VST_OK;
     }
     if (precision != VST_PREC_BF16X3 && !vst_is_f16(precision)) return VST_E_MODE;
-    vst_prof_scope prof(VST_KERNEL_ID(CIN, COUT, STRIDE), st);
+    vst_prof_scope prof(VST_KERNEL_ID(CIN, COUT, STRIDE), st, counted);
     if constexpr (CIN >= 64 && COUT >= 64 && STRIDE == 1) {
         if (vst_option(VST_OPT_STAGE3_LEAN)) return launch_pipe<CIN, COUT, IN_STATE, OUT_STATE, 4, 2>(a, B, st);
         if (vst_option(VST_OPT_STAGE3_WIDE)) return launch_pipe<CIN, COUT, IN_STATE, OUT_STATE, 4, 4>(a, B, st);
@@ -1223,9 +1228,9 @@
 }
 
 template <int MID, int CH>
-static int launch_pair(const ConvArgs& a, int B, int precision, hipStream_t st) {
+static int launch_pair(const ConvArgs& a, int B, int precision, hipStream_t st, bool counted = true) {
     const bool t2 = vst_is_f16(precision), h16 = precision == VST_PREC_F16X2H;
-    vst_prof_scope prof(VST_KERNEL_ID(MID, CH, 1), st);
+    vst_prof_scope prof(VST_KERNEL_ID(MID, CH, 1), st, counted);
     if constexpr (MID == 4) {
         if (a.rgb || a.rgb_u8) {
             constexpr int LDS = PairCfg<MID, CH, 3>::LDS_BYTES;
@@ -1243,7 +1248,7 @@
 template <int CH, int STRIDE>
 static int run_block(const vst_block_weights* w, int direction, int precision, float* dst, const float* src,
                      float* tmp, int B, int H, int W, hipStream_t st, float* rgb = nullptr, uint8_t* rgb_u8 = nullptr,
-                     int rgb_c = 0) {
+                     int rgb_c = 0, int y0 = 0, int y1 = 0, bool counted = true) {
     constexpr int LV = CH == 16 ? 0 : (CH == 64 ? 1 : 2);
     constexpr int MID = CH / 4;
     constexpr int IN_CH = STRIDE == 1 ? CH : CH / 4;
@@ -1274,7 +1279,12 @@
         }
     }
     const bool h16 = CH <= 64 && precision == VST_PREC_F16X2H;
-    int rc = launch_conv<IN_CH, MID, STRIDE, true, false>(a, B, precision, st, h16);
+    const bool band = y1 != 0;
+    if (band) {
+        if (CH > 64 || STRIDE != 1 || precision == VST_PREC_FP32 || y0 < 0 || y1 > Ho || y0 >= y1 || (y0 & 3)) return VST_E_ARG;
+        a.y_begin = y0 - 2 < 0 ? 0 : y0 - 2; a.y_end = y1 + 2 > Ho ? Ho : y1 + 2;
+    }
+    int rc = launch_conv<IN_CH, MID, STRIDE, true, false>(a, B, precision, st, h16, counted);
     if (rc) return rc;
     if constexpr (CH <= 64) {
         if (precision != VST_PREC_FP32) {
@@ -1283,7 +1293,8 @@
             a.packed1 = (const unsigned char*)w->conv[1].packed; a.bias1 = w->conv[1].bias;
             a.sign = direction > 0 ? 1.f : -1.f;
             a.rgb = rgb; a.rgb_u8 = rgb_u8; a.rgb_c = rgb_c;
-            return launch_pair<MID, CH>(a, B, precision, st);
+            if (band) { a.y_begin = y0; a.y_end = y1; }
+            return launch_pair<MID, CH>(a, B, precision, st, counted);
         }
     }
     a.in = h1; a.out = h2; a.packed = (const unsigned char*)w->conv[1].packed; a.bias = w->conv[1].bias;
@@ -1298,8 +1309,16 @@
 VST_DEFINE_TU_RANGE(vst_range_tu_conv)
 
 int vst_block0_to_image(const vst_block_weights* w0, int precision, float* dst, const float* src, float* tmp, int B, int H,
-                        int W, float* rgb, uint8_t* rgb_u8, int rgb_c, void* stream) {
-    return run_block<16, 1>(w0, -1, precision, dst, src, tmp, B, H, W, (hipStream_t)stream, rgb, rgb_u8, rgb_c);
+                        int W, float* rgb, uint8_t* rgb_u8, int rgb_c, void* stream, int y0, int y1, bool counted) {
+    return run_block<16, 1>(w0, -1, precision, dst, src, tmp, B, H, W, (hipStream_t)stream, rgb, rgb_u8, rgb_c, y0, y1, counted);
+}
+
+int vst_block_band(const vst_block_weights* w, int channel, int direction, int precision, float* dst, const float* src, float* tmp,
+                   int B, int H, int W, int y0, int y1, bool counted, void* stream) {
+    hipStream_t st = (hipStream_t)stream;
+    if (channel == 16) return run_block<16, 1>(w, direction, precision, dst, src, tmp, B, H, W, st, nullptr, nullptr, 0, y0, y1, counted);
+    if (channel == 64) return run_block<64, 1>(w, direction, precision, dst, src, tmp, B, H, W, st, nullptr, nullptr, 0, y0, y1, counted);
+    return VST_E_SHAPE;
 }
 
 extern "C" {
diff --git a/vstnet_amd/csrc/layout.hip b/vstnet_amd/csrc/layout.hip
--- a/vstnet_amd/csrc/layout.hip
+++ b/vstnet_amd/csrc/layout.hip
@@ -255,7 +255,7 @@
 
 extern "C" {
 
-int vst_version(void) { return 113; }
+int vst_version(void) { return 114; }
 int64_t vst_max_frame_pixels(void) { return VST_MAX_FRAME_PIXELS; }
 
 int vst_normalize_block(float* w1, float* b1, float* w4, float* b4, float* w7, int c_in1, int c_mid, int c_out, float* scales,
diff --git a/vstnet_amd/csrc/revnet.hip b/vstnet_amd/csrc/revnet.hip
--- a/vstnet_amd/csrc/revnet.hip
+++ b/vstnet_amd/csrc/revnet.hip
@@ -11,6 +11,62 @@
     size_t nb = ((size_t)192 << 20) / per_img;
     if (nb < 1) nb = 1;
     return nb > (size_t)B ? B : (int)nb;
+}
+
+#ifndef VST_BANDS_STAGES
+#define VST_BANDS_STAGES 3
+#endif
+#define VST_BAND_SEAM_DRIFT 4
+#define VST_BAND_MIN_ROWS 16
+#define VST_BAND_MAX_LAUNCHES 40
+
+static int band_schedule(int stage, int direction, int H, int W, int bands, int* out, int cap) {
+    if ((stage != 1 && stage != 2) || (direction != 1 && direction != -1) || bands < 1 || bands > 4 || !out || cap < 0)
+        return VST_E_ARG;
+    if (!vst_shape_ok(1, H, W)) return VST_E_SHAPE;
+    const int rows = H >> (stage - 1);
+    const int n = (stage == 1 && direction < 0) ? 10 : 9;
+    const int first = direction > 0 ? (stage == 1 ? 1 : 11) : (stage == 1 ? 9 : 19);
+    auto seam = [&](int i, int j) { return i == 0 ? 0 : (i == bands ? rows : ((int)((int64_t)i * rows / bands) & ~3) - VST_BAND_SEAM_DRIFT * j); };
+    bool fits = true;
+    for (int i = 0; i < bands; ++i)
+        for (int j = 0; j < n; ++j) fits = fits && seam(i + 1, j) - seam(i, j) >= VST_BAND_MIN_ROWS;
+    const int nb = fits ? bands : 1;
+    int m = 0;
+    for (int i = 0; i < nb; ++i)
+        for (int j = 0; j < n; ++j, ++m) {
+            if (m >= cap) continue;
+            out[3 * m + 0] = first + direction * j;
+            out[3 * m + 1] = nb == 1 ? 0 : seam(i, j);
+            out[3 * m + 2] = nb == 1 ? rows : seam(i + 1, j);
+        }
+    return m;
+}
+
+static int run_chain(const vst_net_weights* w, int stage, int direction, int precision, float* const s[2], float* tmp, int B, int H,
+                     int W, void* stream, bool to_image, float* rgb, uint8_t* rgb_u8, int rgb_c) {
+    int sched[3 * VST_BAND_MAX_LAUNCHES];
+    const int bands = (VST_BANDS_STAGES >> (stage - 1)) & 1 ? vst_option(VST_OPT_BANDS) : 1;
+    const int n = vst_band_schedule(stage, direction, H, W, bands, sched, VST_BAND_MAX_LAUNCHES);
+    if (n < 0) return n;
+    if (n > VST_BAND_MAX_LAUNCHES) return VST_E_ARG;
+    const int rows = H >> (stage - 1), ch = stage == 1 ? 16 : 64;
+    for (int e = 0; e < n; ++e) {
+        const int k = sched[3 * e], y0 = sched[3 * e + 1], y1 = sched[3 * e + 2];
+        const bool whole = y0 == 0 && y1 == rows;
+        float* const dst = s[k & 1];
+        const float* const src = s[1 - (k & 1)];
+        int rc;
+        if (k == 0 && to_image)
+            rc = vst_block0_to_image(&w->blocks[0], precision, dst, src, tmp, B, H, W, rgb, rgb_u8, rgb_c, stream, whole ? 0 : y0,
+                                     whole ? 0 : y1, y0 == 0);
+        else if (whole)
+            rc = vst_block_apply(&w->blocks[k], ch, 1, direction, precision, dst, src, tmp, B, H, W, stream);
+        else
+            rc = vst_block_band(&w->blocks[k], ch, direction, precision, dst, src, tmp, B, H, W, y0, y1, y0 == 0, stream);
+        if (rc) return rc;
+    }
+    return VST_OK;
 }
 
 static int forward_blocks(const vst_net_weights* w, const float* x, const uint8_t* x_u8, float* const s[2], float* tmp, int B,
@@ -23,6 +79,12 @@
     if (rc) return rc;
     const bool sp = vst_is_f16(precision);
     for (int k = fold0 ? 1 : 0; k < VST_NUM_BLOCKS; ++k) {
+        if (fold0 && (k == 1 || k == 11)) {
+            rc = run_chain(w, k == 1 ? 1 : 2, +1, precision, s, tmp, B, H, W, stream, false, nullptr, nullptr, 0);
+            if (rc) return rc;
+            k += 8;
+            continue;
+        }
         if (sp && k >= 21)
             rc = vst3_block256(&w->blocks[k], +1, precision, s[k & 1], s[1 - (k & 1)], tmp, k - 21, 1, B, H, W, stream);
         else
@@ -44,11 +106,19 @@
             if (!w->blocks[0].conv[i].packed || !w->blocks[0].conv[i].bias) return VST_E_ARG;
     }
     for (int k = VST_NUM_BLOCKS - 1; k >= 0; --k) {
+        if (precision != VST_PREC_FP32 && (k == 19 || k == 9)) {
+            rc = run_chain(w, k == 19 ? 2 : 1, -1, precision, s, tmp, B, H, W, stream, rgb0, x_u8 ? nullptr : x, x_u8, C_out);
+            if (rc) return rc;
+            if (k == 9) {
+                if (rgb0) return VST_OK;
+                break;
+            }
+            k = 11;
+            continue;
+        }
         if (sp && k >= 21)
             rc = vst3_block256(&w->blocks[k], -1, precision, s[k & 1], s[1 - (k & 1)], tmp, VST_NUM_BLOCKS - 1 - k, 1, B, H, W,
                                stream);
-        else if (k == 0 && rgb0)
-            return vst_block0_to_image(&w->blocks[0], precision, s[0], s[1], tmp, B, H, W, x_u8 ? nullptr : x, x_u8, C_out, stream);
         else
             rc = vst_block_apply(&w->blocks[k], kBlockChannel[k], kBlockStride[k], -1, precision, s[k & 1], s[1 - (k & 1)],
                                  tmp, B, H, W, stream);
@@ -171,6 +241,10 @@
 
 extern "C" {
 
+int vst_band_schedule(int stage, int direction, int H, int W, int bands, int* out, int cap) {
+    return band_schedule(stage, direction, H, W, bands, out, cap);
+}
+
 size_t vst_pass_workspace_bytes(int B, int H, int W) { return (size_t)B * H * W * (16 + 16 + 40) * sizeof(float); }
 
 int vst_pass_sub_batch(int B, int H, int W) {
diff --git a/vstnet_amd/csrc/runtime.hip b/vstnet_amd/csrc/runtime.hip
--- a/vstnet_amd/csrc/runtime.hip
+++ b/vstnet_amd/csrc/runtime.hip
@@ -2,20 +2,26 @@
 #include <stdlib.h>
 #include "common.h"
 
-static const struct { const char* env; int def; } kOptions[] = {
-    {nullptr, 0},
-    {"VST_LEAN", 0},
-    {nullptr, 0},
-    {"VST_WIDE", 1},
-    {"VST_FOLD16", 1},
-    {"VST_OUT_RGB", 1},
+#ifndef VST_BANDS_DEFAULT
+#define VST_BANDS_DEFAULT 1
+#endif
+static const struct { const char* env; int def, lo, hi; } kOptions[] = {
+    {nullptr, 0, 0, 0},
+    {"VST_LEAN", 0, 0, 1},
+    {nullptr, 0, 0, 0},
+    {"VST_WIDE", 1, 0, 1},
+    {"VST_FOLD16", 1, 0, 1},
+    {"VST_OUT_RGB", 1, 0, 1},
+    {nullptr, 0, 0, 0},
+    {"VST_BANDS", VST_BANDS_DEFAULT, 1, 4},
 };
 constexpr int kNumOptions = sizeof(kOptions) / sizeof(kOptions[0]);
 static std::atomic<int> g_options[kNumOptions];
 static const bool g_options_ready = [] {
     for (int i = 0; i < kNumOptions; ++i) {
         const char* e = kOptions[i].env ? getenv(kOptions[i].env) : nullptr;
-        g_options[i].store(e && (e[0] == '0' || e[0] == '1') ? e[0] - '0' : kOptions[i].def, std::memory_order_relaxed);
+        const bool ok = e && e[0] >= '0' + kOptions[i].lo && e[0] <= '0' + kOptions[i].hi && (e[1] == 0 || kOptions[i].hi == 1);
+        g_options[i].store(ok ? e[0] - '0' : kOptions[i].def, std::memory_order_relaxed);
     }
     return true;
 }();
@@ -28,16 +34,18 @@
 static std::atomic<int> g_prof_kernel{0};
 static int g_prof_count = 0, g_prof_cap = 0;
 static int g_prof_id[VST_PROFILE_MAX_RECORDS];
+static bool g_prof_counted[VST_PROFILE_MAX_RECORDS];
 static hipEvent_t g_prof_ev[2 * VST_PROFILE_MAX_RECORDS];
 static bool g_prof_ev_created = false;
 
-int vst_prof_open(int kernel_id, hipStream_t st) {
+int vst_prof_open(int kernel_id, hipStream_t st, bool counted) {
     const int sel = g_prof_kernel.load(std::memory_order_relaxed);
     if (sel != kernel_id && sel != VST_KERNEL_ALL) return -1;
     std::lock_guard<std::mutex> lk(g_prof_mu);
     if ((g_prof_kernel.load() != kernel_id && g_prof_kernel.load() != VST_KERNEL_ALL) || g_prof_count >= g_prof_cap) return -1;
     const int rec = g_prof_count++;
     g_prof_id[rec] = kernel_id;
+    g_prof_counted[rec] = counted;
     (void)hipEventRecord(g_prof_ev[2 * rec], st);
     return rec;
 }
@@ -51,7 +59,12 @@
 
 int vst_set_option(int option, int value) {
     if (!option_ok(option)) return VST_E_ARG;
-    g_options[option].store(value != 0, std::memory_order_relaxed);
+    if (kOptions[option].hi > 1) {
+        if (value < kOptions[option].lo || value > kOptions[option].hi) return VST_E_ARG;
+    } else {
+        value = value != 0;
+    }
+    g_options[option].store(value, std::memory_order_relaxed);
     return VST_OK;
 }
 
@@ -100,6 +113,7 @@
     std::lock_guard<std::mutex> lk(g_prof_mu);
     g_prof_kernel.store(0);
     double tot = 0.0;
+    int n_counted = 0;
     for (int i = 0; i < g_prof_count; ++i) {
         hipError_t e = hipEventSynchronize(g_prof_ev[2 * i + 1]);
         if (e != hipSuccess) return (int)e;
@@ -107,8 +121,9 @@
         e = hipEventElapsedTime(&ms, g_prof_ev[2 * i], g_prof_ev[2 * i + 1]);
         if (e != hipSuccess) return (int)e;
         tot += ms;
+        n_counted += g_prof_counted[i];
     }
-    *total_ms = tot; *launches = g_prof_count;
+    *total_ms = tot; *launches = n_counted;
     g_prof_count = 0; g_prof_cap = 0;
     return VST_OK;
 }
@@ -130,7 +145,7 @@
             if (n == cap) continue;
             ids[n] = g_prof_id[i]; ms[n] = 0.0; launches[n] = 0; ++n;
         }
-        ms[k] += t; launches[k] += 1;
+        ms[k] += t; launches[k] += g_prof_counted[i];
     }
     *n_ids = n;
     g_prof_count = 0; g_prof_cap = 0;
```

Measured after the change: 220.5. No clear change (-0.3%).
